# jiaxi98/cnf_ot

Hardware: AMD Instinct MI355X
Metric: MC samples/sec through flow fwd+log|detJ| at dim=2, batch=65536 (higher is better)
Workload: dtype f32; 1 GPU; configs[1]: OT free dim=2, batch=65536, sample_and_log_prob (RQS fwd + log|detJ|), L=2 H=16 M=2 K=5, params N(0,0.20^2) seed 42; ONE STEP = one evaluator-shaped pass of 10000 time-slices x 65536 samples (cnf_ot/utils.py:311-340), each slice its own condition t, one cnf_sample_logprob call per rank; batch=65536, dim=2, parallelism=slice-shard x1 (contiguous blocks of the step's slices; no collective)

## Files before the change

cnf_ot_amd/_capi.py:

```python
import ctypes
import os

_HERE = os.path.dirname(os.path.abspath(__file__))
LIB_PATH = os.path.join(_HERE, "lib", "libcnf_ot_amd.so")

CNF_OK = 0
CNF_ERR_INVALID = -22
CNF_ERR_UNSUPPORTED = -95
CNF_ERR_NOMEM = -12
CNF_ERR_HIP = -5


class CnfConfig(ctypes.Structure):
  _fields_ = [
    ("dim", ctypes.c_int32), ("num_layers", ctypes.c_int32),
    ("hidden_size", ctypes.c_int32), ("mlp_num_layers", ctypes.c_int32),
    ("num_bins", ctypes.c_int32),
    ("range_min", ctypes.c_float), ("range_max", ctypes.c_float),
    ("min_bin_size", ctypes.c_float), ("min_knot_slope", ctypes.c_float),
    ("periodized", ctypes.c_int32),
  ]


class CnfFieldGrid(ctypes.Structure):
# ... 57 lines not shown

KDE_MAX_BW = 4


class CnfKdeSpec(ctypes.Structure):
  _fields_ = [("n_bw", ctypes.c_int32), ("loo", ctypes.c_int32), ("bw", ctypes.c_float * KDE_MAX_BW)]


TERM_KINETIC, TERM_KINETIC_SCORE, TERM_FLOW_MATCHING, TERM_POTENTIAL, TERM_REVERSE_KL, TERM_NEG_LOGPROB = range(6)
TERM_DENSITY_L2, TERM_DENSITY_L2_DATA = 6, 7
POTENTIALS = {"quadratic": 0, "double_well": 1, "obstacle": 2}
DRIFTS = {"ou": 0, "gradient": 1, "smile": 1, "nongradient": 2, "lorenz": 3}

_P = ctypes.c_void_p
_I64 = ctypes.c_int64
_U64 = ctypes.c_uint64
_CFG = ctypes.POINTER(CnfConfig)
SYMBOLS = {
  "cnf_config_default": (None, [_CFG, ctypes.c_int32]),
  "cnf_param_count": (_I64, [_CFG]),
  "cnf_model_create": (ctypes.c_int, [_CFG, ctypes.POINTER(_P)]),
  "cnf_model_destroy": (None, [_P]),
  "cnf_model_set_params": (ctypes.c_int, [_P, _P, _P]),
  "cnf_model_reserve": (ctypes.c_int, [_P, _P, _I64]),
  "cnf_model_reserved": (_I64, [_P, _P]),
  "cnf_model_table_bytes": (_I64, [_P]),
  "cnf_model_has_tables": (ctypes.c_int, [_P]),
  "cnf_model_term_on_tables": (ctypes.c_int, [_P, _I64, _I64, ctypes.c_int]),
  "cnf_model_last_path": (ctypes.c_int, [_P]),
  "cnf_model_set_precise": (ctypes.c_int, [_P, ctypes.c_int]),
  "cnf_forward_logdet": (ctypes.c_int, [_P, _P, _P, _I64, _P, _P, _I64, _P]),
  "cnf_inverse_logdet": (ctypes.c_int, [_P, _P, _P, _I64, _P, _P, _I64, _P]),
  "cnf_log_prob": (ctypes.c_int, [_P, _P, _P, _I64, _P, _I64, _P]),
  "cnf_sample_logprob": (ctypes.c_int, [_P, _P, _P, _I64, _P, _P, _I64, _P]),
  "cnf_sample_logprob_seeded": (ctypes.c_int, [_P, _U64, _I64, _I64, _P, _I64, _P, _P, _I64, _P]),
  "cnf_forward_logdet_f64": (ctypes.c_int, [_P, _P, _P, _I64, _P, _P, _I64, _P]),
  "cnf_inverse_logdet_f64": (ctypes.c_int, [_P, _P, _P, _I64, _P, _P, _I64, _P]),
  "cnf_log_prob_f64": (ctypes.c_int, [_P, _P, _P, _I64, _P, _I64, _P]),
  "cnf_sample_logprob_f64": (ctypes.c_int, [_P, _P, _P, _I64, _P, _P, _I64, _P]),
  "cnf_fill_normal": (ctypes.c_int, [_U64, _U64, _I64, _P, _P]),
  "cnf_fill_normal_threefry": (ctypes.c_int, [ctypes.c_uint32, ctypes.c_uint32, _U64, _U64, _I64, _P, _P, _P]),
  "cnf_loss_terms": (ctypes.c_int, [_P, ctypes.POINTER(CnfLossSpec), _P, ctypes.c_int, _P, _I64, _I64, _P, _P]),
  "cnf_loss_terms_seeded": (ctypes.c_int, [_P, ctypes.POINTER(CnfLossSpec), _U64, _I64, _I64, _P, _I64, _I64, _P, _P]),
  "cnf_grad_supported": (ctypes.c_int, [_CFG]),
  "cnf_grad_enable": (ctypes.c_int, [_P, _I64]),
  "cnf_loss_terms_grad": (ctypes.c_int, [_P, ctypes.POINTER(CnfLossSpec), _P, ctypes.c_int, _P, _I64, _I64,
                                         ctypes.c_float, _P, _P, _P, _P]),
  "cnf_loss_terms_grad_multi": (ctypes.c_int, [_P, ctypes.c_int32, _P, _P, _P, _P, _P, _P, _P, _P, _P, _P, _P]),
  "cnf_input_vjp": (ctypes.c_int, [_P, ctypes.c_int, _P, _P, _I64, _P, _P, _P, _I64, _P]),
  "cnf_pass_vjp": (ctypes.c_int, [_P, ctypes.c_int, _P, _P, _I64, _P, _P, _P, _P, _P, _I64, _P]),
  "cnf_neg_logprob_vjp": (ctypes.c_int, [_P, _P, _P, _I64, ctypes.c_float, _P, _P, _P, _I64, _P]),
  "cnf_kinetic_potential_vjp": (ctypes.c_int, [_P, _P, _I64, _P, ctypes.c_int32, ctypes.c_float, ctypes.c_float, ctypes.c_int32,
                                               ctypes.c_float, ctypes.c_float, _P, _P, _P, _P, _P, _P]),
  "cnf_logprob_fd": (ctypes.c_int, [_P, _P, _P, _I64, ctypes.c_float, _P, _I64, _P]),
  "cnf_score": (ctypes.c_int, [_P, _P, ctypes.c_int32, _P, _I64, _I64, _P, _P, _P]),
  "cnf_logprob_fd_vjp": (ctypes.c_int, [_P, _P, _P, _I64, ctypes.c_float, _P, _P, _P, _P, _I64, _P]),
  "cnf_score_fd_vjp": (ctypes.c_int, [_P, _P, _P, _I64, ctypes.c_float, ctypes.c_float, ctypes.c_float, ctypes.c_int32,
                                      ctypes.c_float, ctypes.c_float, _P, _P, _P, _P, _I64, _P]),
  "cnf_score_residual": (ctypes.c_int, [_P, _P, _I64, _I64, ctypes.c_int32, ctypes.c_float, ctypes.c_float,
                                        ctypes.c_int32, ctypes.c_float, ctypes.c_float, _P, _P, _P, _P]),
  "cnf_score_residual_force": (ctypes.c_int, [_P, _P, _P, ctypes.c_float, _I64, _I64, ctypes.c_int32, ctypes.c_float,
                                              ctypes.c_float, ctypes.c_int32, ctypes.c_float, ctypes.c_float, _P, _P, _P, _P,
                                              _P]),
  "cnf_term_residual": (ctypes.c_int, [ctypes.c_int32, _P, _P, _I64, _I64, ctypes.c_int32, ctypes.c_int32, ctypes.c_float,
                                       ctypes.c_float, _P, _P, _P, _P]),
  "cnf_rkl_residual": (ctypes.c_int, [_P, _P, _I64, ctypes.c_int32, ctypes.c_float, ctypes.c_float, ctypes.c_float,
                                      ctypes.c_float, _P, _P, _P, _P]),
  "cnf_adam_step": (ctypes.c_int, [_P, _P, _P, _P, _I64, ctypes.c_float, ctypes.c_float, ctypes.c_float,
                                   ctypes.c_float, _I64, _P]),
  "cnf_step_begin": (ctypes.c_int, [_P, _P]),
  "cnf_fill_normal_dev": (ctypes.c_int, [_P, _U64, _I64, _P, _P]),
  "cnf_fill_uniform_dev": (ctypes.c_int, [_P, _U64, _I64, ctypes.c_float, _P, _P]),
  "cnf_mixture_source_dev": (ctypes.c_int, [_P, _U64, _I64, _P, _P, _P, _P]),
  "cnf_adam_step_dev": (ctypes.c_int, [_P, _P, _P, _P, _I64, ctypes.c_float, ctypes.c_float, ctypes.c_float,
                                       ctypes.c_float, _P, _P]),
  "cnf_weighted_sum": (ctypes.c_int, [_P, _P, _I64, _P, _P]),
  "cnf_hopf_cole_workspace": (ctypes.c_int, [ctypes.c_double, ctypes.c_double, ctypes.c_double, _I64, _I64,
                                              ctypes.POINTER(_I64)]),
  "cnf_hopf_cole_2d": (ctypes.c_int, [ctypes.c_int32, ctypes.c_float] + [ctypes.c_double] * 6
                       + [_P, _I64, _P, _I64, _P, _P, _P, _P, _P, _P, _P, _I64, _P]),
  "cnf_hopf_cole_path_workspace": (ctypes.c_int, [ctypes.c_double, ctypes.c_double, ctypes.c_double, _I64, _I64,
                                                   ctypes.POINTER(_I64)]),
  "cnf_hopf_cole_path_2d": (ctypes.c_int, [ctypes.c_int32, ctypes.c_float] + [ctypes.c_double] * 6
                            + [ctypes.POINTER(ctypes.c_double), _I64, _P, _I64, _P, _I64, _P, _P, _P, _P, _P, _P, _P,
                               _I64, _P]),
  "cnf_eulerian_fields": (ctypes.c_int, [_P, ctypes.POINTER(CnfFieldGrid), _P, _I64, _P, _I64, ctypes.c_float, ctypes.c_float,
                                        _P, _P, _P, _P, _P]),
  "cnf_eulerian_fields_f64": (ctypes.c_int, [_P, ctypes.POINTER(CnfFieldGrid), _P, _I64, _P, _I64, ctypes.c_double,
                                            ctypes.c_double, _P, _P, _P, _P, _P]),
  "cnf_trajectories": (ctypes.c_int, [_P, _P, _I64, ctypes.c_float, _P, _I64, ctypes.c_float, _P, _P, _P]),
  "cnf_trajectories_f64": (ctypes.c_int, [_P, _P, _I64, ctypes.c_double, _P, _I64, ctypes.c_double, _P, _P, _P]),
  "cnf_fp_particles_workspace": (ctypes.c_int, [_I64, ctypes.c_int32, ctypes.c_int32, ctypes.POINTER(_I64)]),
  "cnf_fp_particles": (ctypes.c_int, [ctypes.c_int32, ctypes.c_int32, ctypes.c_float, ctypes.c_double, ctypes.c_double,
                                      _I64, ctypes.c_double, _U64, _I64, _I64, _P, ctypes.POINTER(_I64), ctypes.c_int32,
                                      ctypes.POINTER(CnfFieldGrid), _P, _P, _P, _P, _I64, _P]),
  "cnf_point_stats": (ctypes.c_int, [_P, _I64, ctypes.c_int32, ctypes.c_int32, ctypes.POINTER(CnfFieldGrid), _P, _P, _P,
                                     _I64, _P]),
  "cnf_importance_workspace": (ctypes.c_int, [_I64, _I64, ctypes.c_int32, ctypes.POINTER(_I64)]),
  "cnf_importance_stats": (ctypes.c_int, [_P, ctypes.POINTER(CnfTargetSpec), _P, ctypes.c_int, _P, _I64, _I64, _P, _P, _I64,
                                          _P]),
  "cnf_importance_stats_seeded": (ctypes.c_int, [_P, ctypes.POINTER(CnfTargetSpec), _U64, _I64, _I64, _P, _I64, _I64, _P, _P,
                                                 _I64, _P]),
  "cnf_mmd_workspace": (ctypes.c_int, [ctypes.c_int32, _I64, _I64, ctypes.c_int32, ctypes.c_int32, ctypes.POINTER(_I64)]),
  "cnf_mmd_splits": (ctypes.c_int, [ctypes.c_int32, _I64, _I64, ctypes.c_int32]),
  "cnf_mmd2": (ctypes.c_int, [ctypes.POINTER(CnfMmdSpec), ctypes.c_int32, _P, _I64, _P, _I64, ctypes.c_int32, _P, _P, _P,
                              _I64, _P]),
  "cnf_sinkhorn_workspace": (ctypes.c_int, [ctypes.c_int32, _I64, _I64, ctypes.c_int32, ctypes.POINTER(_I64)]),
  "cnf_sinkhorn_splits": (ctypes.c_int, [ctypes.c_int32, _I64, _I64, ctypes.c_int32]),
  "cnf_sinkhorn": (ctypes.c_int, [ctypes.c_int32, _P, _I64, _P, _I64, ctypes.c_int32, ctypes.POINTER(ctypes.c_double),
                                  ctypes.c_int32, _P, _P, _P, _P, _P, _I64, _P]),
  "cnf_sliced_workspace": (ctypes.c_int, [ctypes.c_int32, _I64, _I64, ctypes.c_int32, ctypes.c_int32, ctypes.c_int32,
                                          ctypes.POINTER(_I64)]),
  "cnf_sliced_tile": (ctypes.c_int, []),
  "cnf_sliced_w2": (ctypes.c_int, [ctypes.c_int32, _P, _I64, _P, _I64, ctypes.c_int32, _P, ctypes.c_int32, ctypes.c_int32, _P,
                                   _P, _P, _I64, _P]),
  "cnf_knn_workspace": (ctypes.c_int, [ctypes.c_int32, _I64, _I64, ctypes.c_int32, ctypes.c_int32, ctypes.POINTER(_I64)]),
  "cnf_knn_splits": (ctypes.c_int, [ctypes.c_int32, _I64, _I64, ctypes.c_int32]),
  "cnf_knn": (ctypes.c_int, [ctypes.c_int32, _P, _I64, _P, _I64, ctypes.c_int32, ctypes.c_int32, _P, _P, _P, _P, _P, _P, _I64,
                             _P]),
  "cnf_interaction_workspace": (ctypes.c_int, [ctypes.c_int32, _I64, _I64, ctypes.c_int32, ctypes.c_int32,
                                               ctypes.POINTER(_I64)]),
  "cnf_interaction_splits": (ctypes.c_int, [ctypes.c_int32, _I64, _I64, ctypes.c_int32]),
  "cnf_interaction": (ctypes.c_int, [ctypes.POINTER(CnfInteractionSpec), ctypes.c_int32, _P, _I64, _P, _I64, ctypes.c_int32,
                                     _P, _P, _P, _P, _I64, _P]),
  "cnf_interaction_vjp_workspace": (ctypes.c_int, [ctypes.c_int32, _I64, ctypes.c_int32, ctypes.POINTER(_I64)]),
  "cnf_interaction_vjp": (ctypes.c_int, [ctypes.POINTER(CnfInteractionSpec), ctypes.c_int32, _P, _P, _I64, ctypes.c_int32, _P,
                                         _P, _I64, _P]),
  "cnf_stein_workspace": (ctypes.c_int, [ctypes.c_int32, _I64, ctypes.c_int32, ctypes.c_int32, ctypes.POINTER(_I64)]),
  "cnf_stein_splits": (ctypes.c_int, [ctypes.c_int32, _I64, ctypes.c_int32]),
  "cnf_stein": (ctypes.c_int, [ctypes.POINTER(CnfSteinSpec), ctypes.c_int32, _P, _P, _I64, ctypes.c_int32, _P, _P, _P, _P,
                               _P, _I64, _P]),
  "cnf_kde_workspace": (ctypes.c_int, [ctypes.c_int32, _I64, _I64, ctypes.c_int32, ctypes.c_int32, ctypes.c_int32,
                                       ctypes.POINTER(_I64)]),
  "cnf_kde_splits": (ctypes.c_int, [ctypes.c_int32, _I64, _I64, ctypes.c_int32]),
  "cnf_kde": (ctypes.c_int, [ctypes.POINTER(CnfKdeSpec), ctypes.c_int32, _P, _I64, _P, _I64, ctypes.c_int32, _P, _P, _P, _P,
                             _I64, _P]),
  "cnf_mv_particles_workspace": (ctypes.c_int, [ctypes.c_int32, _I64, ctypes.c_int32, ctypes.c_int32, ctypes.POINTER(_I64)]),
  "cnf_mv_particles": (ctypes.c_int, [ctypes.POINTER(CnfInteractionSpec), ctypes.c_double, ctypes.c_int32, ctypes.c_int32,
                                      ctypes.c_float, ctypes.c_double, ctypes.c_double, _I64, ctypes.c_double, _U64, _I64,
                                      ctypes.c_int32, _I64, _P, ctypes.POINTER(_I64), ctypes.c_int32,
                                      ctypes.POINTER(CnfFieldGrid), _P, _P, _P, _P, _P, _I64, _P]),
  "cnf_strerror": (ctypes.c_char_p, [ctypes.c_int]),
  "cnf_build_arch": (ctypes.c_char_p, []),
  "cnf_config_supported": (ctypes.c_int, [_CFG]),
}
_INTERNAL = {
  "cnf_model_set_fast_math": (ctypes.c_int, [_P, ctypes.c_int]),
  "cnf_model_set_samples_per_lane": (ctypes.c_int, [_P, ctypes.c_int]),
  "cnf_model_set_mfma": (ctypes.c_int, [_P, ctypes.c_int]),
  "cnf_model_set_pwl": (ctypes.c_int, [_P, ctypes.c_int]),
  "cnf_model_set_dpar": (ctypes.c_int, [_P, ctypes.c_int]),
  "cnf_model_set_pwl_builder": (ctypes.c_int, [_P, ctypes.c_int]),
  "cnf_model_last_pwl_builder": (ctypes.c_int, [_P]),
  "cnf_internal_build_tables_into": (ctypes.c_int, [_P, _P, _P, ctypes.c_float, _I64, _P]),
  "cnf_model_set_profiling": (ctypes.c_int, [_P, ctypes.c_int]),
  "cnf_model_read_profile": (ctypes.c_int, [_P, ctypes.POINTER(ctypes.c_double), ctypes.POINTER(ctypes.c_double),
                                            ctypes.POINTER(_I64), ctypes.POINTER(_I64)]),
}
PATH_NAMES = {0: "none", 1: "mlp1", 2: "mlp2", 3: "mfma", 4: "tables", 5: "loss_mlp", 6: "loss_tables", 7: "f64", 8: "detect", 9: "dpar", 10: "fields",
              11: "score", 12: "importance"}

_lib = None


class CnfError(RuntimeError):
  def __init__(self, code, where):
    self.code = code
    msg = lib().cnf_strerror(code).decode() if _lib is not None else str(code)
    super().__init__(f"{where}: {msg} ({code})")


def lib():
  global _lib
  if _lib is not None:
    return _lib
  if not os.path.exists(LIB_PATH):
    raise ImportError(
      f"{LIB_PATH} is missing: the cnf_ot_amd product path is hand-written HIP "
      "for gfx950 and has no CPU fallback. Build it with "
      "`python -m cnf_ot_amd.build` (needs hipcc).")
  handle = ctypes.CDLL(LIB_PATH)
  for table in (SYMBOLS, _INTERNAL):
    for name, (res, args) in table.items():
      fn = getattr(handle, name)
      fn.restype = res
      fn.argtypes = args
  _lib = handle
  return _lib


def check(code, where):
  if code != CNF_OK:
    raise CnfError(code, where)
```

cnf_ot_amd/build.py:

```python
import os
import shutil
import subprocess
import sys
from concurrent.futures import ThreadPoolExecutor

HERE = os.path.dirname(os.path.abspath(__file__))
SRC_DIR = os.path.join(HERE, "csrc")
LIB_DIR = os.path.join(HERE, "lib")
LIB_PATH = os.path.join(LIB_DIR, "libcnf_ot_amd.so")
OBJ_DIR = os.path.join(LIB_DIR, "obj")
SOURCES = ["cnf_flow.hip", "cnf_grad.hip", "cnf_grad_pwl.hip", "cnf_importance.hip", "cnf_mmd.hip", "cnf_knn.hip", "cnf_interaction.hip", "cnf_interaction_vjp.hip", "cnf_stein.hip", "cnf_kde.hip", "cnf_hopf_cole.hip", "cnf_fp_particles.hip",
           "cnf_mv_particles.hip", "cnf_sinkhorn.hip", "cnf_sliced.hip", "cnf_step.hip", "cnf_model.hip", "cnf_rng.hip"]
HEADERS = ["cnf_device.h", "cnf_terms.h", "cnf_common.h", "cnf_host.h", "cnf_flow_tile.h", "cnf_backward.h", "cnf_pwl.h",
           "cnf_pwl_build.h", "cnf_fp_stats.h", "cnf_pairs.h", "cnf_interaction_pairs.h", os.path.join("..", "..", "include", "cnf_ot_amd.h")]
VARIANT_PATH = os.path.join(LIB_DIR, "BUILD_VARIANT")
ARCH = "gfx950"


def _hipcc():
  for cand in (os.environ.get("HIPCC"), shutil.which("hipcc"), "/opt/rocm/bin/hipcc"):
    if cand and os.path.exists(cand):
      return cand
  raise RuntimeError("hipcc not found (need ROCm's hipcc to build the gfx950 kernels)")


def _variant() -> str:
  try:
    with open(VARIANT_PATH) as f:
      return f.read().strip()
  except OSError:
    return ""


def is_stale(minimal: bool = False) -> bool:
  if not os.path.exists(LIB_PATH):
    return True
  if not minimal and _variant() != "full":
    return True
  t = os.path.getmtime(LIB_PATH)
  deps = [os.path.join(SRC_DIR, f) for f in SOURCES + HEADERS]
  return any(os.path.getmtime(d) > t for d in deps if os.path.exists(d))


def _jobs() -> int:
  try:
    n = int(os.environ.get("MAX_JOBS", ""))
  except ValueError:
    n = 16
  return max(1, min(n, len(SOURCES), 16))


def build(force: bool = False, minimal: bool = False, verbose: bool = False) -> str:
  if not force and not is_stale(minimal):
    return LIB_PATH
  os.makedirs(OBJ_DIR, exist_ok=True)
  hipcc = _hipcc()
  flags = ["-O3", f"--offload-arch={ARCH}", "-std=c++17", "-fPIC", "-Wall", "-Wno-unused-function"]
  if minimal:
    flags.append("-DCNF_MINIMAL_CONFIGS")
  flags += os.environ.get("CNF_EXTRA_FLAGS", "").split()
  flags_path = os.path.join(OBJ_DIR, "FLAGS")
  try:
    with open(flags_path) as f:
      same_flags = f.read() == " ".join(flags)
  except OSError:
    same_flags = False
  newest_header = max(os.path.getmtime(os.path.join(SRC_DIR, h)) for h in HEADERS)

  def compile_one(name):
    src, obj = os.path.join(SRC_DIR, name), os.path.join(OBJ_DIR, os.path.splitext(name)[0] + ".o")
    if not force and same_flags and os.path.exists(obj) and os.path.getmtime(obj) > max(os.path.getmtime(src), newest_header):
      return obj
    cmd = [hipcc, *flags, "-c", src, "-o", obj]
    if verbose:
      print(" ".join(cmd), flush=True)
    res = subprocess.run(cmd, capture_output=True, text=True)
    if res.returncode != 0:
      raise RuntimeError(f"hipcc failed on {name}:\n" + res.stdout + res.stderr)
    return obj

  if os.path.exists(flags_path):
    os.remove(flags_path)
  with ThreadPoolExecutor(max_workers=_jobs()) as pool:
    objs = list(pool.map(compile_one, SOURCES))
  with open(flags_path, "w") as f:
    f.write(" ".join(flags))
  tmp = LIB_PATH + ".tmp"
  cmd = [hipcc, f"--offload-arch={ARCH}", "-fPIC", "-shared", *objs, "-o", tmp]
  if verbose:
    print(" ".join(cmd), flush=True)
  res = subprocess.run(cmd, capture_output=True, text=True)
  if res.returncode != 0:
    raise RuntimeError("hipcc failed to link:\n" + res.stdout + res.stderr)
  os.replace(tmp, LIB_PATH)
  with open(VARIANT_PATH, "w") as f:
    f.write("minimal\n" if minimal else "full\n")
  return LIB_PATH


if __name__ == "__main__":
  path = build(force="--force" in sys.argv, minimal="--minimal" in sys.argv, verbose=True)
  print("built", path)
```

cnf_ot_amd/csrc/cnf_common.h:

```cpp
#pragma once
#include <mutex>
#include <map>
#include <tuple>
#include <type_traits>
#include <unordered_map>
#include <vector>

#include "cnf_device.h"
#include "cnf_terms.h"
#include "../../include/cnf_ot_amd.h"

namespace cnf {

constexpr int TILE = 256;

struct ModelArgs {
  const float* prep;
  const float* wq;
  int64_t per_layer;
  int64_t per_layer_q;
  int32_t D, L, M;
  SplineConsts sc;
  SplineConstsT<double> scd;
  const double* tabd;
  const double* e2tab;
};

template <class R> __device__ __forceinline__ const SplineConstsT<R>& sc_of(const ModelArgs& a);
template <> __device__ __forceinline__ const SplineConstsT<float>& sc_of<float>(const ModelArgs& a) { return a.sc; }
template <> __device__ __forceinline__ const SplineConstsT<double>& sc_of<double>(const ModelArgs& a) { return a.scd; }
template <class R> __device__ __forceinline__ const R* table_of(const ModelArgs& a);
template <> __device__ __forceinline__ const float* table_of<float>(const ModelArgs& a) { return a.prep; }
template <> __device__ __forceinline__ const double* table_of<double>(const ModelArgs& a) { return a.tabd; }

}

struct CnfModel {
  CnfConfig cfg;
  cnf::SplineConsts sc;
  cnf::SplineConstsT<double> scd;
  int64_t tabd_off;
  int64_t e2_off;
  int precise;
  float* prep;
  int64_t n_params;
  int64_t per_layer;
  int device;
  int num_cus;
  int fast_math;
  int force_spl;
  int use_mfma;
  uint32_t div_magic;
  int64_t per_layer_q;
  int64_t mfma_off;
  int params_set;
  float* grad_slabs;
  int64_t grad_max_blocks;
  int use_pwl;
  int use_dpar;
  int pwl_builder;
  int last_pwl_builder;
  float* pwl_stats;
  struct PwlWorkspace { float* tables; int64_t sets; uint32_t epoch; std::vector<float*> retired; };
  std::mutex pwl_mu;
  std::unordered_map<void*, PwlWorkspace> pwl_ws;
  hipEvent_t prep_event;
  void* prep_stream;
  int last_path;
  struct ProfRec { hipEvent_t e0, e1, e2; int64_t samples; int path; };
  int profiling;
  std::vector<ProfRec> prof;
};

enum CnfPath {
  CNF_PATH_NONE = 0,
  CNF_PATH_MLP1 = 1,
  CNF_PATH_MLP2 = 2,
  CNF_PATH_MFMA = 3,
  CNF_PATH_TABLES = 4,
  CNF_PATH_LOSS_MLP = 5,
  CNF_PATH_LOSS_TABLES = 6,
  CNF_PATH_F64 = 7,
  CNF_PATH_DPAR = 9,
  CNF_PATH_DETECT = 8,
  CNF_PATH_FIELDS = 10,
  CNF_PATH_SCORE = 11,
  CNF_PATH_IMPORTANCE = 12,
};

static inline bool pwl_network(const CnfConfig& g) {
  return g.dim == 2 && g.hidden_size == 16 && g.num_bins == 5 && g.mlp_num_layers == 2 && !g.periodized;
}
static inline bool pwl_backward_network(const CnfConfig& g) { return pwl_network(g) && g.num_layers <= 4; }
static inline bool pwl_config_ok(const CnfModel* m) { return m->use_pwl && m->fast_math && pwl_network(m->cfg); }
static inline bool pwl_backward_ok(const CnfModel* m) {
  return pwl_config_ok(m) && pwl_backward_network(m->cfg) && m->pwl_stats != nullptr;
}
constexpr int64_t PWL_MIN_SLICE = 8192, PWL_MIN_POINTS = 262144;
static inline bool pwl_term_on_tables(const CnfModel* m, int64_t slice_len, int64_t n_points, bool with_grad) {
  if (with_grad ? !pwl_backward_ok(m) : !pwl_config_ok(m)) return false;
  return m->use_pwl != 1 || (slice_len >= PWL_MIN_SLICE && n_points >= PWL_MIN_POINTS);
}

#ifdef CNF_MINIMAL_CONFIGS
#define CNF_KERNEL_CONFIGS(X) X(16, 5)
#else
#define CNF_KERNEL_CONFIGS(X) \
  X(8, 5) X(16, 4) X(16, 5) X(16, 8) X(16, 10) X(32, 5) X(32, 8) X(64, 5)
#endif

template <class F>
static inline int with_shape(const CnfConfig& cfg, F&& f) {
#define X(HH, KK)                                      \
  if (cfg.hidden_size == HH && cfg.num_bins == KK)     \
    return f(std::integral_constant<int, HH>{}, std::integral_constant<int, KK>{});
  CNF_KERNEL_CONFIGS(X)
#undef X
  return CNF_ERR_UNSUPPORTED;
}
static inline bool shape_compiled(const CnfConfig& cfg) {
  return with_shape(cfg, [](auto, auto) { return CNF_OK; }) == CNF_OK;
}

template <class K>
static inline bool ensure_lds(K kernel, size_t bytes) {
  if (bytes > 160 * 1024) return false;
  if (bytes <= 64 * 1024) return true;
  static std::mutex mu;
  static std::map<std::pair<const void*, int>, bool> done;
  int dev = 0;
  if (hipGetDevice(&dev) != hipSuccess) return false;
  std::lock_guard<std::mutex> lock(mu);
  const auto key = std::make_pair((const void*)kernel, dev);
  auto it = done.find(key);
  if (it != done.end()) return it->second;
  const bool ok = hipFuncSetAttribute((const void*)kernel, hipFuncAttributeMaxDynamicSharedMemorySize, 160 * 1024) == hipSuccess;
  done[key] = ok;
  return ok;
}

struct ProfScope {
  CnfModel* m; hipStream_t s; CnfModel::ProfRec r; bool on;
  ProfScope(CnfModel* m_, hipStream_t s_, bool with_build, int64_t samples, int path) : m(m_), s(s_), on(false) {
    r.e0 = r.e1 = r.e2 = nullptr; r.samples = samples; r.path = path;
    if (!m->profiling || samples < 0 || m->prof.size() >= 4096) return;
    if (hipEventCreate(&r.e1) != hipSuccess || hipEventCreate(&r.e2) != hipSuccess) return;
    if (with_build) { if (hipEventCreate(&r.e0) != hipSuccess) return; (void)hipEventRecord(r.e0, s); }
    else (void)hipEventRecord(r.e1, s);
    on = true;
  }
  void built() { if (on && r.e0) (void)hipEventRecord(r.e1, s); }
  void done() { if (on) { (void)hipEventRecord(r.e2, s); m->prof.push_back(r); on = false; } }
};

template <class K, class A>
static int launch(CnfModel* m, K kernel, int64_t grid, int threads, size_t lds, hipStream_t stream, const A& a, int path,
                  bool gated = false, int64_t prof_samples = -1) {
  if (!gated) m->last_path = path;
  if (!ensure_lds(kernel, lds)) return CNF_ERR_UNSUPPORTED;
  ProfScope ps(m, stream, false, prof_samples, path);
  hipLaunchKernelGGL(kernel, dim3((unsigned)grid), dim3(threads), lds, stream, a);
  ps.done();
  return hipGetLastError() == hipSuccess ? CNF_OK : CNF_ERR_HIP;
}

template <class K, class... A>
static int launch_plain(K kernel, int64_t grid, int threads, size_t lds, hipStream_t stream, const A&... a) {
  hipLaunchKernelGGL(kernel, dim3((unsigned)grid), dim3(threads), lds, stream, a...);
  return hipGetLastError() == hipSuccess ? CNF_OK : CNF_ERR_HIP;
}

template <class K>
static inline int resident_blocks_per_cu(K kernel, int threads, size_t lds) {
  static std::mutex mu;
  static std::map<std::tuple<const void*, int, size_t, int>, int> cache;
  int dev = 0;
  if (hipGetDevice(&dev) != hipSuccess) return 1;
  std::lock_guard<std::mutex> lock(mu);
  const auto key = std::make_tuple((const void*)kernel, threads, lds, dev);
  auto it = cache.find(key);
  if (it != cache.end()) return it->second;
  int n = 0;
  if (hipOccupancyMaxActiveBlocksPerMultiprocessor(&n, (const void*)kernel, threads, lds) != hipSuccess || n < 1) n = 1;
  hipFuncAttributes fa;
  if (hipFuncGetAttributes(&fa, (const void*)kernel) == hipSuccess) {
    const size_t per_wg = ((lds + fa.sharedSizeBytes + 511) / 512) * 512;
    if (per_wg > 0) { const int by_lds = (int)((160 * 1024) / per_wg); if (by_lds >= 1 && by_lds < n) n = by_lds; }
    const int regs = ((fa.numRegs > 0 ? fa.numRegs : 1) + 7) / 8 * 8;
    int waves_per_simd = 512 / regs; if (waves_per_simd > 8) waves_per_simd = 8;
    const int by_regs = waves_per_simd * 4 / ((threads + 63) / 64);
    if (by_regs >= 1 && by_regs < n) n = by_regs;
  }
  cache[key] = n;
  return n;
}

// ... 60 lines not shown
```

cnf_ot_amd/csrc/cnf_device.h:

```cpp
#pragma once

#include <hip/hip_runtime.h>
#include <stdint.h>
#include <type_traits>

namespace cnf {

typedef float v2f __attribute__((ext_vector_type(2)));
typedef int v2i __attribute__((ext_vector_type(2)));

typedef const float __attribute__((address_space(4)))* uniform_ptr;

__device__ __forceinline__ uniform_ptr as_uniform(const float* p) { return (uniform_ptr)p; }

__device__ __forceinline__ uniform_ptr launder(uniform_ptr p) {
  asm volatile("" : "+s"(p));
  return p;
}

enum TabField {
  F_X0 = 0, F_Y0, F_BW, F_BH, F_IBW, F_IBH, F_S, F_ST, F_D0, F_D1, F_L2S,
  F_XK,
  F_YK,
  F_TAIL,
// ... 111 lines not shown
  static __device__ __forceinline__ v2f div(v2f a, v2f b) { return v2f{a.x / b.x, a.y / b.y}; }
  static __device__ __forceinline__ v2f sqrt(v2f x) { return v2f{sqrtf(x.x), sqrtf(x.y)}; }
};

constexpr float LOG2E = 1.44269502162933349609375f;
constexpr float LN2 = 0.693147182464599609375f;

template <> struct Math<true> {
  static __device__ __forceinline__ float exp(float x) { return __builtin_amdgcn_exp2f(x * LOG2E); }
  static __device__ __forceinline__ float log(float x) { return __builtin_amdgcn_logf(x) * LN2; }
  static __device__ __forceinline__ float rcp(float x) { return __builtin_amdgcn_rcpf(x); }
  static __device__ __forceinline__ float div(float a, float b) {
    const float r = __builtin_amdgcn_rcpf(b), q = a * r;
    return fmaf(fmaf(-b, q, a), r, q);
  }
  static __device__ __forceinline__ float sqrt(float x) { return __builtin_amdgcn_sqrtf(x); }
  static __device__ __forceinline__ v2f exp(v2f x) {
    const v2f t = x * LOG2E;
    return v2f{__builtin_amdgcn_exp2f(t.x), __builtin_amdgcn_exp2f(t.y)};
  }
  static __device__ __forceinline__ float exp2(float x) { return __builtin_amdgcn_exp2f(x); }
  static __device__ __forceinline__ v2f exp2(v2f x) { return v2f{__builtin_amdgcn_exp2f(x.x), __builtin_amdgcn_exp2f(x.y)}; }
  static __device__ __forceinline__ v2f log(v2f x) {
    return v2f{__builtin_amdgcn_logf(x.x), __builtin_amdgcn_logf(x.y)} * LN2;
  }
  static __device__ __forceinline__ v2f rcp(v2f x) {
    return v2f{__builtin_amdgcn_rcpf(x.x), __builtin_amdgcn_rcpf(x.y)};
  }
  static __device__ __forceinline__ v2f div(v2f a, v2f b) {
    const v2f r = rcp(b), q = a * r;
    return vfma(vfma(-b, q, a), r, q);
  }
  static __device__ __forceinline__ v2f sqrt(v2f x) {
    return v2f{__builtin_amdgcn_sqrtf(x.x), __builtin_amdgcn_sqrtf(x.y)};
  }
};

__device__ __forceinline__ v2f mul_clip01(v2f a, v2f b) {
  v2f z;
  asm("s_nop 0\n\tv_pk_mul_f32 %0, %1, %2 clamp" : "=v"(z) : "v"(a), "v"(b));
  return z;
}
__device__ __forceinline__ float mul_clip01(float a, float b) { return clip01(a * b); }
__device__ __forceinline__ double mul_clip01(double a, double b) { return clip01(a * b); }

template <bool FAST, class T, bool OFFSET_ADDED = false>
__device__ __forceinline__ T knot_slope(T t, const SplineConstsT<typename Lanes<T>::real> sc) {
  const T v = OFFSET_ADDED ? t : t + sc.sp_offset;
  const T av = vabs(v);
  const T e = Math<FAST>::exp(-av);
  typedef typename Lanes<T>::real R;
  if constexpr (std::is_same<T, double>::value) {
    return vrelu(v) + ::log1p(e) + sc.min_slope;
  } else {
    const T l_log = Math<FAST>::log(e + 1.0f);
    const T l_ser = vfma(e * -0.5f, e, e);
    const T l = vsel(vlt(e, (R)1e-4f), l_ser, l_log);
    return vfma(v + av, splat<T>(0.5f), l) + sc.min_slope;
  }
}

template <bool INV, bool FAST, class T, bool L2S_GIVEN = true, bool ARG = false, bool NEWTON = true, bool PRE = false>
__device__ __forceinline__ void rqs_bin_eval(T v, T x0, T y0, T bw, T bh, T ibw, T s, T st,
                                             T d0, T d1, T l2s, T& out, T& ld, T d0bh = T{}, T s2 = T{}) {
  using M = Math<FAST>;
  static_assert(!PRE || (INV && !NEWTON), "prepared products: the sampling direction's root");
  static_assert(NEWTON || INV, "the root without its Newton step: the inverse only");
  T z;
  [[maybe_unused]] T two_s;
  if (INV) {
    const T dy = vclamp(v - y0, bh);
    if constexpr (NEWTON) {
      const T c = -s * dy;
      const T b = vfma(-st, dy, d0 * bh);
      const T a = vfma(s, bh, -b);
      const T disc = vfma(b, b, a * c * -4.0f);
      z = clip01(M::div(c * -2.0f, b + M::sqrt(disc)));
    } else {
      two_s = PRE ? s2 : s * 2.0f;
      const T c2 = two_s * dy;
      const T b = vfma(-st, dy, PRE ? d0bh : d0 * bh);
      const T a = vfma(s, bh, -b);
      const T disc = vfma(b, b, a * (c2 + c2));
      z = mul_clip01(c2, M::rcp(b + M::sqrt(disc)));
    }
    out = vfma(bw, z, x0);
  } else {
    z = clip01((v - x0) * ibw);
  }
  const T sq_z = z * z;
  const T z1mz = z - sq_z;
  const T omz = 1.0f - z;
  const T den = vfma(st, z1mz, s);
  const T iden = M::rcp(den);
  if (!INV) out = vfma(bh * vfma(s, sq_z, d0 * z1mz), iden, y0);
  const T num2 = vfma(d1, sq_z, vfma(NEWTON ? s * 2.0f : two_s, z1mz, d0 * omz * omz));
  if constexpr (ARG) {
    static_assert(!L2S_GIVEN, "the argument form folds s^2 in");
    const T q = s * iden;
    ld = num2 * q * q;
  } else {
    T ldf;
    if (L2S_GIVEN) {
      ldf = l2s + M::log(num2 * iden * iden);
    } else {
      const T q = s * iden;
      ldf = M::log(num2 * q * q);
    }
    ld = INV ? -ldf : ldf;
  }
}

template <int K, class R> __device__ __forceinline__ int bin_of(const R* pos, R v) {
  int k = 0;
#pragma unroll
  for (int j = 1; j < K; ++j) k += (v >= pos[j]) ? 1 : 0;
  return k;
}
template <int K> __device__ __forceinline__ v2i bin_of_pairs(const float* kb, v2f v) {
  const v2f big = v2f{1.152921504606846976e18f, 1.152921504606846976e18f};
  v2f c = v2f{0.0f, 0.0f};
#pragma unroll
  for (int j = 1; j < K; ++j) {
    const v2f nk = *reinterpret_cast<const v2f*>(kb + 2 * j);
    v2f m;
    asm("v_pk_fma_f32 %0, %1, %2, %3 clamp" : "=v"(m) : "v"(v), "v"(big), "v"(nk));
    c = j == 1 ? m : c + m;
  }
  return v2i{(int)c.x, (int)c.y};
}
template <int K, class R> __device__ __forceinline__ R gather(const R* tab, int f, int k) {
  return tab[tab_off(f, K) + k];
}
template <int K> __device__ __forceinline__ v2f gather(const float* tab, int f, v2i k) {
  return v2f{tab[tab_off(f, K) + k.x], tab[tab_off(f, K) + k.y]};
}

template <class T> struct BinRow {
  const typename Lanes<T>::real* p;
  __device__ __forceinline__ BinRow(const typename Lanes<T>::real* tab, int k) : p(tab + k) {}
  template <int K> __device__ __forceinline__ T get(int f) const { return p[tab_off(f, K)]; }
};
template <> struct BinRow<v2f> {
  typedef const volatile float __attribute__((address_space(3))) * lds_ptr;
  lds_ptr px, py;
  __device__ __forceinline__ BinRow(const float* tab, v2i k) {
    lds_ptr t = (lds_ptr)(uintptr_t)(uint32_t)(uintptr_t)tab;
    px = t + k.x;
    py = t + k.y;
  }
  template <int K> __device__ __forceinline__ v2f get(int f) const { return v2f{px[tab_off(f, K)], py[tab_off(f, K)]}; }
};

template <int K, bool INV, bool FAST, class T, bool ARG = false, bool LEAN = false>
__device__ __forceinline__ void table_spline(const typename Lanes<T>::real* tab, T v,
                                             const SplineConstsT<typename Lanes<T>::real> sc, T& out, T& ld,
                                             bool tails = true) {
  typedef typename Lanes<T>::real R;
  typename Lanes<T>::index k;
  if constexpr (std::is_same<T, v2f>::value) k = bin_of_pairs<K>(tab + tab_off(INV ? F_YKB : F_XKB, K), v);
  else k = bin_of<K>(tab + tab_off(INV ? F_YK : F_XK, K), v);
  const BinRow<T> row(tab, k);
  const T bw = INV ? row.template get<K>(F_BW) : splat<T>(0.0f);
  const T ibw = INV ? splat<T>(0.0f) : row.template get<K>(F_IBW);
  if constexpr (ARG && LEAN && INV)
    rqs_bin_eval<INV, FAST, T, false, true, false, true>(v, row.template get<K>(F_X0), row.template get<K>(F_Y0), bw,
                                            row.template get<K>(F_BH), ibw,
                                            row.template get<K>(F_S), row.template get<K>(F_ST), row.template get<K>(F_D0),
                                            row.template get<K>(F_D1), splat<T>(0.0f), out, ld,
                                            row.template get<K>(F_D0BH), row.template get<K>(F_2S));
  else if constexpr (ARG)
    rqs_bin_eval<INV, FAST, T, false, true, !LEAN>(v, row.template get<K>(F_X0), row.template get<K>(F_Y0), bw,
                                            row.template get<K>(F_BH), ibw,
                                            row.template get<K>(F_S), row.template get<K>(F_ST), row.template get<K>(F_D0),
                                            row.template get<K>(F_D1), splat<T>(0.0f), out, ld);
  else
    rqs_bin_eval<INV, FAST, T, true, false, !LEAN>(v, row.template get<K>(F_X0), row.template get<K>(F_Y0), bw,
                               row.template get<K>(F_BH), ibw,
                               row.template get<K>(F_S), row.template get<K>(F_ST), row.template get<K>(F_D0),
                               row.template get<K>(F_D1), row.template get<K>(F_L2S), out, ld);
  if (LEAN ? tails : maybe_outside(v, sc.lo, sc.hi)) {
    const auto below = vle(v, sc.lo);
    const auto above = vge(v, sc.hi);
    const R* tl = tab + tab_off(F_TAIL, K);
    const T lo_out = INV ? vfma(v - sc.lo, splat<T>(tl[T_INV_DLO]), splat<T>(sc.lo))
                         : vfma(v - sc.lo, splat<T>(tl[T_DLO]), splat<T>(sc.lo));
    const T hi_out = INV ? vfma(v - sc.hi, splat<T>(tl[T_INV_DHI]), splat<T>(sc.hi))
                         : vfma(v - sc.hi, splat<T>(tl[T_DHI]), splat<T>(sc.hi));
    out = vsel(below, lo_out, out);
    ld = vsel(below, ARG ? splat<T>(tl[T_DLO]) : splat<T>(INV ? -tl[T_LOG_DLO] : tl[T_LOG_DLO]), ld);
    out = vsel(above, hi_out, out);
    ld = vsel(above, ARG ? splat<T>(tl[T_DHI]) : splat<T>(INV ? -tl[T_LOG_DHI] : tl[T_LOG_DHI]), ld);
  }
}

__device__ __forceinline__ v2f step_mask(v2f d, v2f big) {
  v2f m;
  asm("v_pk_mul_f32 %0, %1, %2 clamp" : "=v"(m) : "v"(d), "v"(big));
  return m;
}

template <int K, bool INV, bool FAST, bool SHIFT_FREE>
__device__ __forceinline__ void cond_spline_masked(const v2f (&th)[3 * K + 1], v2f v,
                                                   const SplineConsts sc, v2f& out, v2f& ld) {
  using M = Math<FAST>;
  typedef v2f T;
  T ew[K], eh[K];
  T aw, ah;
  if constexpr (SHIFT_FREE) {
#pragma unroll
    for (int k = 0; k < K; ++k) { ew[k] = M::exp2(th[k]); eh[k] = M::exp2(th[K + k]); }
    T sw = ew[0] + ew[1], sh = eh[0] + eh[1];
#pragma unroll
    for (int k = 2; k < K; ++k) { sw += ew[k]; sh += eh[k]; }
    const T r = M::rcp(sw * sh) * sc.span_eff;
    aw = r * sh; ah = r * sw;
  } else {
    T mw = th[0], mh = th[K];
#pragma unroll
    for (int k = 1; k < K; ++k) { mw = vmax(mw, th[k]); mh = vmax(mh, th[K + k]); }
#pragma unroll
    for (int k = 0; k < K; ++k) { ew[k] = M::exp2(th[k] - mw); eh[k] = M::exp2(th[K + k] - mh); }
    T sw = ew[0], sh = eh[0];
#pragma unroll
    for (int k = 1; k < K; ++k) { sw += ew[k]; sh += eh[k]; }
    aw = M::rcp(sw) * sc.span_eff; ah = M::rcp(sh) * sc.span_eff;
  }
  const T big = splat<T>(1.152921504606846976e18f);
  T px = splat<T>(sc.lo), py = splat<T>(sc.lo);
  T wp = vfma(ew[0], aw, splat<T>(sc.min_bin)), hp = vfma(eh[0], ah, splat<T>(sc.min_bin));
  T x0 = px, y0 = py;
  T mprev = splat<T>(1.0f), bw = splat<T>(0.0f), bh = splat<T>(0.0f), t0 = splat<T>(0.0f), t1 = splat<T>(0.0f);
#pragma unroll
  for (int k = 1; k < K; ++k) {
    px += wp;
    py += hp;
    const T m = step_mask(v - (INV ? py : px), big);
    const T o = mprev - m;
    bw = k == 1 ? o * wp : vfma(o, wp, bw);
    bh = k == 1 ? o * hp : vfma(o, hp, bh);
    t0 = k == 1 ? o * th[2 * K] : vfma(o, th[2 * K + k - 1], t0);
    t1 = k == 1 ? o * th[2 * K + 1] : vfma(o, th[2 * K + k], t1);
    x0 = vfma(m, wp, x0);
    y0 = vfma(m, hp, y0);
    if (k == K - 1) { wp = sc.hi - px; hp = sc.hi - py; }
    else { wp = vfma(ew[k], aw, splat<T>(sc.min_bin)); hp = vfma(eh[k], ah, splat<T>(sc.min_bin)); }
    mprev = m;
  }
  bw = vfma(mprev, wp, bw);
  bh = vfma(mprev, hp, bh);
  t0 = vfma(mprev, th[3 * K - 1], t0);
  t1 = vfma(mprev, th[3 * K], t1);
  T d0, d1;
  if constexpr (SHIFT_FREE) {
    const T l0 = v2f{__builtin_amdgcn_logf(M::exp2(t0).x + 1.0f), __builtin_amdgcn_logf(M::exp2(t0).y + 1.0f)};
    const T l1 = v2f{__builtin_amdgcn_logf(M::exp2(t1).x + 1.0f), __builtin_amdgcn_logf(M::exp2(t1).y + 1.0f)};
    d0 = vfma(l0, splat<T>(LN2), splat<T>(sc.min_slope));
    d1 = vfma(l1, splat<T>(LN2), splat<T>(sc.min_slope));
  } else {
    T n0 = t0 * LN2, n1 = t1 * LN2;
    asm volatile("" : "+v"(n0), "+v"(n1));
    d0 = knot_slope<FAST, T, true>(n0, sc);
    d1 = knot_slope<FAST, T, true>(n1, sc);
  }
  const T ibw = M::rcp(bw);
  const T s = bh * ibw;
  const T st = d1 + d0 - s * 2.0f;
  rqs_bin_eval<INV, FAST, T, false>(v, x0, y0, bw, bh, ibw, s, st, d0, d1, s, out, ld);
  if (maybe_outside(v, sc.lo, sc.hi)) {
    const auto below = vle(v, sc.lo);
    const auto above = vge(v, sc.hi);
    const T lo_out = INV ? M::div(v - sc.lo, d0) + sc.lo : vfma(v - sc.lo, d0, splat<T>(sc.lo));
    const T hi_out = INV ? M::div(v - sc.hi, d1) + sc.hi : vfma(v - sc.hi, d1, splat<T>(sc.hi));
    const T ld0 = M::log(d0), ld1 = M::log(d1);
    out = vsel(below, lo_out, out);
    ld = vsel(below, INV ? -ld0 : ld0, ld);
    out = vsel(above, hi_out, out);
    ld = vsel(above, INV ? -ld1 : ld1, ld);
  }
}

template <int K, bool INV, bool FAST, bool SHIFT_FREE, bool ARG = false, bool LEAN = false, class SlopeFetch>
__device__ __forceinline__ void cond_spline_rows(const v2f (&qa)[K], const v2f (&qb)[K], SlopeFetch&& slopes, v2f v,
                                                 const SplineConsts sc, v2f& out, v2f& ld, bool tails = true) {
  using M = Math<FAST>;
  typedef v2f T;
  auto la = [&](int j) { return qa[j >> 1][j & 1]; };
  auto lb = [&](int j) { return qb[j >> 1][j & 1]; };
  constexpr bool UNNORM = LEAN && SHIFT_FREE && INV;
  T ew[K], eh[K];
  T aw, ah;
  [[maybe_unused]] T ch[K + 1];
  if constexpr (SHIFT_FREE) {
#pragma unroll
    for (int k = 0; k < K; ++k) {
      ew[k] = v2f{__builtin_amdgcn_exp2f(la(k)), __builtin_amdgcn_exp2f(lb(k))};
      eh[k] = v2f{__builtin_amdgcn_exp2f(la(K + k)), __builtin_amdgcn_exp2f(lb(K + k))};
    }
    T sw = ew[0] + ew[1], sh = eh[0] + eh[1];
    if constexpr (UNNORM) { ch[1] = eh[0]; ch[2] = sh; }
#pragma unroll
    for (int k = 2; k < K; ++k) {
      sw += ew[k]; sh += eh[k];
      if constexpr (UNNORM) ch[k + 1] = sh;
    }
    const T r = M::rcp(sw * sh) * sc.span_eff;
    aw = r * sh; ah = r * sw;
  } else {
    float mwa = la(0), mwb = lb(0), mha = la(K), mhb = lb(K);
#pragma unroll
    for (int k = 1; k < K; ++k) {
      mwa = fmaxf(mwa, la(k)); mwb = fmaxf(mwb, lb(k));
      mha = fmaxf(mha, la(K + k)); mhb = fmaxf(mhb, lb(K + k));
    }
#pragma unroll
    for (int k = 0; k < K; ++k) {
      ew[k] = v2f{__builtin_amdgcn_exp2f(la(k) - mwa), __builtin_amdgcn_exp2f(lb(k) - mwb)};
      eh[k] = v2f{__builtin_amdgcn_exp2f(la(K + k) - mha), __builtin_amdgcn_exp2f(lb(K + k) - mhb)};
    }
    T sw = ew[0], sh = eh[0];
#pragma unroll
    for (int k = 1; k < K; ++k) { sw += ew[k]; sh += eh[k]; }
    aw = M::rcp(sw) * sc.span_eff; ah = M::rcp(sh) * sc.span_eff;
  }
  const T big = splat<T>(1.152921504606846976e18f);
  T x0, y0, bw, bh, kf;
  if constexpr (UNNORM) {
    const T t = ch[K] * (1.0f / sc.span_eff);
    T m[K];
#pragma unroll
    for (int k = 1; k < K; ++k) m[k] = step_mask(vfma(v - (sc.lo + (float)k * sc.min_bin), t, -ch[k]), big);
    T xs = m[1] * ew[0], ys = m[1] * eh[0];
    T ws = ew[0] - xs, hs = eh[0] - ys;
    kf = m[1];
#pragma unroll
    for (int k = 1; k < K; ++k) {
      const T o = k == K - 1 ? m[k] : m[k] - m[k + 1];
      ws = vfma(o, ew[k], ws);
      hs = vfma(o, eh[k], hs);
      if (k > 1) { xs = vfma(m[k], ew[k - 1], xs); ys = vfma(m[k], eh[k - 1], ys); kf += m[k]; }
    }
    const T base = vfma(kf, splat<T>(sc.min_bin), splat<T>(sc.lo));
    x0 = vfma(xs, aw, base);
    y0 = vfma(ys, ah, base);
    bw = vfma(ws, aw, splat<T>(sc.min_bin));
    bh = vfma(hs, ah, splat<T>(sc.min_bin));
// ... 607 lines not shown
```

cnf_ot_amd/csrc/cnf_flow.hip:

```cpp
#include "cnf_flow_tile.h"
#include "cnf_host.h"
#include "cnf_pwl_build.h"

#include <math.h>
#include <new>
#include <stdlib.h>
#include <string.h>

namespace cnf {

__global__ void circular_slopes_kernel(const float* __restrict__ params, float* __restrict__ prep, int K, int H,
                                       int D, int L, int M, int64_t per_layer) {
  const int P = 3 * K + 1;
  const int hdr = hdr_floats(K);
  const int l = blockIdx.x / (D - 1), d = 1 + blockIdx.x % (D - 1);
  int64_t o = (int64_t)l * per_layer;
  for (int dd = 1; dd < d; ++dd) o += cond_floats_p(dd, H, M, P, true);
  o += cond_floats_p(d, H, M, P, true) - ((int64_t)H * P + P);
  for (int r = threadIdx.x; r <= H; r += blockDim.x)
    prep[hdr + o + (int64_t)r * P + 3 * K] = params[P + o + (int64_t)r * P + 2 * K];
}

__global__ void prepare_kernel(const float* __restrict__ params, float* __restrict__ prep,
                               int K, int64_t n_params, double lo, double hi, double min_bin,
                               double min_slope, int D, int L, int M, int64_t per_layer,
                               int64_t per_layer_q, int64_t mfma_off, int64_t tabd_off, int H, int periodic) {
  const int P = 3 * K + 1;
  const int hdr = hdr_floats(K);
  constexpr int MAXK = 64;
  if (blockIdx.x != gridDim.x - 1) {
    const int nb = gridDim.x - 1;
    for (int64_t i = blockIdx.x * (int64_t)blockDim.x + threadIdx.x; i < n_params - P; i += (int64_t)nb * blockDim.x)
      prep[hdr + i] = params[P + i];
    if (mfma_off > 0) {
      const int nc = L * (D - 1);
      for (int ci = blockIdx.x; ci < nc; ci += nb) {
        const int l = ci / (D - 1), d = 1 + ci % (D - 1);
        int64_t so = P + l * per_layer, qo = mfma_off + l * per_layer_q;
        for (int dd = 1; dd < d; ++dd) { so += cond_floats(dd, 16, M, 16); qo += cond_floats_mfma(dd, M); }
        const float* src = params + so;
        float* dst = prep + qo;
        const int nf = (1 + d) + 1 + 2 * M;
        for (int idx = threadIdx.x; idx < nf * 64; idx += blockDim.x) {
          const int f = idx >> 6, lane = idx & 63, g = lane >> 4, i = lane & 15;
          float o[4];
          if (f <= d) {
            for (int t = 0; t < 4; ++t) o[t] = src[f * 16 + 4 * g + t];
          } else if (f == d + 1) {
            for (int t = 0; t < 4; ++t) o[t] = src[(1 + d) * 16 + 4 * g + t];
          } else {
            const int m = (f - (d + 2)) >> 1;
            const float* Wm = src + (1 + d) * 16 + 16 + m * (256 + 16);
            if (((f - (d + 2)) & 1) == 0) { for (int t = 0; t < 4; ++t) o[t] = Wm[(4 * g + t) * 16 + i]; }
            else { for (int t = 0; t < 4; ++t) o[t] = Wm[256 + 4 * g + t]; }
          }
          for (int t = 0; t < 4; ++t) dst[(f * 64 + lane) * 4 + t] = o[t];
        }
      }
    }
    return;
  }

  __shared__ double ex[2][MAXK], dl[MAXK + 1], mxs[2];
  if (threadIdx.x < 2) {
    const float* u = params + threadIdx.x * K;
    double mx = u[0];
    for (int k = 1; k < K; ++k) mx = fmax(mx, (double)u[k]);
    mxs[threadIdx.x] = mx;
  }
  __syncthreads();
  const double offset = log(exp(1.0 - min_slope) - 1.0);
  for (int idx = threadIdx.x; idx < 3 * K + 1; idx += blockDim.x) {
    if (idx < 2 * K) {
      const int part = idx / K, k = idx - part * K;
      ex[part][k] = exp((double)params[part * K + k] - mxs[part]);
    } else {
      const int k = idx - 2 * K;
      const double v = (double)params[2 * K + (periodic && k == K ? 0 : k)] + offset;
      dl[k] = fmax(v, 0.0) + log1p(exp(-fabs(v))) + min_slope;
    }
  }
  __syncthreads();
  __shared__ double xk[MAXK + 1], yk[MAXK + 1];
  double* td = reinterpret_cast<double*>(prep + tabd_off);
  for (int i = threadIdx.x; i < hdr; i += blockDim.x) { prep[i] = 0.0f; td[i] = 0.0; }
  const double total = (hi - lo) - K * min_bin;
  if (threadIdx.x < 2) {
    const int part = threadIdx.x;
    double* pos = part == 0 ? xk : yk;
    double sum = 0;
    for (int k = 0; k < K; ++k) sum += ex[part][k];
    double run = 0;
    pos[0] = lo;
    for (int k = 0; k < K - 1; ++k) {
      run += ex[part][k] / sum * total + min_bin;
      pos[k + 1] = lo + run;
    }
    pos[K] = hi;
  }
  __syncthreads();
  for (int k = threadIdx.x; k < K; k += blockDim.x) {
    const double bw = xk[k + 1] - xk[k], bh = yk[k + 1] - yk[k], s = bh / bw;
    td[tab_off(F_X0, K) + k] = xk[k];            td[tab_off(F_Y0, K) + k] = yk[k];
    td[tab_off(F_BW, K) + k] = bw;               td[tab_off(F_BH, K) + k] = bh;
    td[tab_off(F_IBW, K) + k] = 1.0 / bw;        td[tab_off(F_IBH, K) + k] = 1.0 / bh;
    td[tab_off(F_S, K) + k] = s;                 td[tab_off(F_ST, K) + k] = dl[k + 1] + dl[k] - 2.0 * s;
    td[tab_off(F_D0, K) + k] = dl[k];            td[tab_off(F_D1, K) + k] = dl[k + 1];
    td[tab_off(F_L2S, K) + k] = 2.0 * log(s);
    prep[tab_off(F_X0, K) + k] = (float)xk[k];
    prep[tab_off(F_Y0, K) + k] = (float)yk[k];
    prep[tab_off(F_BW, K) + k] = (float)bw;
    prep[tab_off(F_BH, K) + k] = (float)bh;
    prep[tab_off(F_IBW, K) + k] = (float)(1.0 / bw);
    prep[tab_off(F_IBH, K) + k] = (float)(1.0 / bh);
    prep[tab_off(F_S, K) + k] = (float)s;
    prep[tab_off(F_ST, K) + k] = (float)(dl[k + 1] + dl[k] - 2.0 * s);
    prep[tab_off(F_D0, K) + k] = (float)dl[k];
    prep[tab_off(F_D1, K) + k] = (float)dl[k + 1];
    prep[tab_off(F_L2S, K) + k] = (float)(2.0 * log(s));
    td[tab_off(F_D0BH, K) + k] = dl[k] * bh;     td[tab_off(F_2S, K) + k] = 2.0 * s;
    prep[tab_off(F_D0BH, K) + k] = (float)(dl[k] * bh);
    prep[tab_off(F_2S, K) + k] = 2.0f * (float)s;
  }
  for (int k = threadIdx.x; k <= K; k += blockDim.x) {
    const float big = 1.152921504606846976e18f;
    if (2 * k + 1 < 2 * tab_stride(K)) {
      prep[tab_off(F_XKB, K) + 2 * k] = prep[tab_off(F_XKB, K) + 2 * k + 1] = -(float)xk[k] * big;
      prep[tab_off(F_YKB, K) + 2 * k] = prep[tab_off(F_YKB, K) + 2 * k + 1] = -(float)yk[k] * big;
    }
    prep[tab_off(F_XK, K) + k] = (float)xk[k];
    prep[tab_off(F_YK, K) + k] = (float)yk[k];
    td[tab_off(F_XK, K) + k] = xk[k];
    td[tab_off(F_YK, K) + k] = yk[k];
  }
  if (threadIdx.x != 64) return;
  double* tld = td + tab_off(F_TAIL, K);
  tld[T_DLO] = dl[0];            tld[T_DHI] = dl[K];
  tld[T_LOG_DLO] = log(dl[0]);   tld[T_LOG_DHI] = log(dl[K]);
  tld[T_INV_DLO] = 1.0 / dl[0];  tld[T_INV_DHI] = 1.0 / dl[K];
  float* tl = prep + tab_off(F_TAIL, K);
  tl[T_DLO] = (float)dl[0];             tl[T_DHI] = (float)dl[K];
  tl[T_LOG_DLO] = (float)log(dl[0]);    tl[T_LOG_DHI] = (float)log(dl[K]);
  tl[T_INV_DLO] = (float)(1.0 / dl[0]); tl[T_INV_DHI] = (float)(1.0 / dl[K]);
}

template <int H, int K, bool TO_BASE, bool FAST, class T, bool MFMA = false, bool PRECISE = false, bool PERIODIC = false, int DFIX = 0>
__global__ __launch_bounds__(TILE, 2) void flow_kernel(const FlowArgsT<typename Lanes<T>::real> a) {
  typedef typename Lanes<T>::real R;
  extern __shared__ __attribute__((aligned(16))) float lds_raw[];
  R* lds = reinterpret_cast<R*>(lds_raw);
  constexpr int HDR = hdr_floats(K);
  constexpr int SPL = Lanes<T>::N;
  constexpr int TS = TILE * SPL;
  const int DD = DFIX ? DFIX : a.m.D;
  const uint32_t dmagic = DFIX == 2 ? 0x80000000u : (uint32_t)a.div_magic;
  R* tab = lds;
  R* U = lds + HDR;
  R* O = U + DD * TS;
  if (gate_closed(a)) return;
  for (int i = threadIdx.x; i < HDR; i += TILE) tab[i] = table_of<R>(a.m)[i];
  [[maybe_unused]] double* e2tab = nullptr;
  [[maybe_unused]] double* tabd = nullptr;
  [[maybe_unused]] R* LO = nullptr;
  if constexpr (PRECISE) {
    LO = O + DD * TS;
    e2tab = reinterpret_cast<double*>(LO + DD * TS);
    tabd = e2tab + EXP2_N;
    for (int i = threadIdx.x; i < EXP2_N; i += TILE) e2tab[i] = a.m.e2tab[i];
    for (int i = threadIdx.x; i < HDR; i += TILE) tabd[i] = a.m.tabd[i];
  }

  const int64_t n_tiles = (a.B + TS - 1) / TS;
  for (int64_t tile = blockIdx.x; tile < n_tiles; tile += gridDim.x) {
    const int64_t tile_start = tile * TS;
    const int64_t i = tile_start + SPL * threadIdx.x;
    __syncthreads();
    if (TO_BASE && !PRECISE && a.fd2) tile_load_fd<R>(a, U, DD, dmagic, TS, tile_start);
    else if (a.in) tile_load<R>(a.in, U, DD, dmagic, TS, tile_start, a.B);
    else tile_noise_flow(a, U, DD, dmagic, TS, tile_start, TILE);
    const T c = load_cond<T>(a, tile_start, i);
    __syncthreads();

    T base = splat<T>(0.0f);
    if (!TO_BASE && a.aux_mode == AUX_LOGPROB && a.aux) base = base_logprob<T>(lds_col<T>(U + SPL * threadIdx.x, TS), DD);
    BaseAcc<T> bacc;
    [[maybe_unused]] T poison = splat<T>(0.0f);
    if constexpr (TO_BASE) {
      for (int d = 0; d < DD; ++d) { const T v = lds_get<T>(U + SPL * threadIdx.x, d, TS); poison += v - v; }
    }
    const T acc = flow_pass<H, K, TO_BASE, FAST, T, MFMA, PRECISE, PERIODIC, DFIX>(a.m, tab, U, O, c, e2tab, tabd, LO, &bacc);
    if (a.aux) {
      T r = acc;
      if (a.aux_mode == AUX_LOGPROB) {
        if constexpr (PRECISE) r = bacc.log_prob(acc, DD);
        else r = TO_BASE ? base_logprob<T>(lds_col<T>(U + SPL * threadIdx.x, TS), DD) + acc : base - acc;
      }
      if constexpr (TO_BASE) r += poison;
      if (TO_BASE && !PRECISE && a.fd2) store_fd(a, i, r);
      else store_aux(a.aux, i, a.B, r);
    }
    if (a.out) {
      if constexpr (TO_BASE) {
        for (int d = 0; d < DD; ++d) lds_put(U + SPL * threadIdx.x, d, TS, lds_get<T>(U + SPL * threadIdx.x, d, TS) + poison);
      }
      __syncthreads();
      tile_store<R>(a.out, U, DD, dmagic, TS, tile_start, a.B);
    }
  }
}


template <int H, int K, bool FAST, class T>
__global__ __launch_bounds__(1024) void flow_dpar_kernel(const FlowArgs a) {
  extern __shared__ __attribute__((aligned(16))) float lds[];
  constexpr int HDR = hdr_floats(K), P = 3 * K + 1, SPL = Lanes<T>::N, TS = 64 * SPL;
  const int D = a.m.D, L = a.m.L, NT = blockDim.x, NW = NT >> 6;
  const int wave = __builtin_amdgcn_readfirstlane(threadIdx.x >> 6), lane = threadIdx.x & 63;
  float* tab = lds;
  float* U = lds + HDR;
  float* O = U + D * TS;
  float* LD = O + D * TS;
  if (gate_closed(a)) return;
  for (int i = threadIdx.x; i < HDR; i += NT) tab[i] = a.m.prep[i];
  const SplineConsts& sc = a.m.sc;
  uniform_ptr weights = as_uniform(a.m.prep + HDR);
  const int64_t cpart = cond_floats(0, H, a.m.M, P) - H;

  const int64_t n_tiles = (a.B + TS - 1) / TS;
  for (int64_t tile = blockIdx.x; tile < n_tiles; tile += gridDim.x) {
    const int64_t tile_start = tile * TS;
    const int64_t i = tile_start + SPL * lane;
    __syncthreads();
    if (a.in) tile_load_n<float>(a.in, U, D, a.div_magic, TS, tile_start, a.B, NT);
    else tile_noise_flow(a, U, D, a.div_magic, TS, tile_start, NT);
    const T c = load_cond<T>(a, tile_start, i);
    __syncthreads();
    T base = splat<T>(0.0f);
    if (wave == 0 && a.aux_mode == AUX_LOGPROB && a.aux) base = base_logprob<T>(lds_col<T>(U + SPL * lane, TS), D);
    T acc = splat<T>(0.0f);
    for (int l = 0; l < L; ++l) {
      const bool odd = l & 1;
      const int first_idx = odd ? D - 1 : 0, idx_step = odd ? -1 : 1;
      const float* cu = U + SPL * lane;
      float* co = O + SPL * lane;
      T o, ld;
      if (wave == 0) {
        table_spline<K, true, FAST, T>(tab, lds_get<T>(cu, first_idx, TS), sc, o, ld);
        lds_put(co, first_idx, TS, o);
        acc += ld;
      }
      for (int d = 1 + wave; d < D; d += NW) {
        const int64_t off = l * a.m.per_layer + (int64_t)H * ((d - 1) + (int64_t)d * (d - 1) / 2) + (d - 1) * cpart;
        T th[P];
        conditioner<H, P, T>(weights + off, d, a.m.M, c, cu, first_idx, idx_step, TS, th);
        const int idx = first_idx + d * idx_step;
        cond_spline<K, true, FAST, T>(th, lds_get<T>(cu, idx, TS), sc, o, ld);
        lds_put(co, idx, TS, o);
        acc += ld;
      }
      __syncthreads();
      float* t = U; U = O; O = t;
    }
    if (a.aux) lds_put(LD + wave * TS + SPL * lane, 0, TS, acc);
    __syncthreads();
    if (a.aux && wave == 0) {
      T tot = splat<T>(0.0f);
      for (int w = 0; w < NW; ++w) tot += lds_get<T>(LD + w * TS + SPL * lane, 0, TS);
      store_aux(a.aux, i, a.B, a.aux_mode == AUX_LOGPROB ? base - tot : tot);
    }
    if (a.out) tile_store_n<float>(a.out, U, D, a.div_magic, TS, tile_start, a.B, NT);
  }
}

struct PwlArgs {
  ModelArgs m;
  const float* in;
  float* out;
  float* aux;
  const float* tables;
  int64_t B, slice_len;
  int32_t n_slices, tiles_per_slice, aux_mode;
  const uint32_t* gate;
  uint32_t gate_epoch;
  int32_t gate_want;
  uint64_t seed;
  int64_t first_sample, slice_stride;
  int32_t in_shared;
};

__global__ void cond_uniform_kernel(const float* __restrict__ c, int64_t B, uint32_t* flag, uint32_t epoch) {
  const uint32_t c0 = __float_as_uint(c[0]);
  bool diff = false;
  for (int64_t i = blockIdx.x * (int64_t)blockDim.x + threadIdx.x; i < B; i += (int64_t)gridDim.x * blockDim.x)
    diff |= __float_as_uint(c[i]) != c0;
  if (__syncthreads_or(diff) && threadIdx.x == 0) *flag = epoch;
}

constexpr int PWL_WAIT_VM0 = 0x0F70;

template <int K, bool TO_BASE, bool FAST, bool PRECISE = false, int LROWS = PWL_LROWS, int LFIX = 0, bool SEEDED = false>
__global__ __launch_bounds__(PWL_MAX_THREADS) void flow_pwl_kernel(const PwlArgs a) {
  const int PWL_THREADS = blockDim.x, PWL_TS = 2 * PWL_THREADS;
  extern __shared__ __attribute__((aligned(16))) float lds_raw[];
  constexpr int HDR = (hdr_floats(K) + 3) & ~3;
  float* tab = lds_raw;
  float* tbl = lds_raw + HDR;
  const int tid = threadIdx.x;
  const int L = LFIX ? LFIX : a.m.L;
  if (gate_closed(a)) return;
  for (int i = tid; i < hdr_floats(K); i += PWL_THREADS) tab[i] = table_of<float>(a.m)[i];
  const SplineConsts sc = sc_scalars(sc_of<float>(a.m));
  [[maybe_unused]] double* e2tab = nullptr;
  [[maybe_unused]] double* tabd = nullptr;
  if constexpr (PRECISE) {
    e2tab = reinterpret_cast<double*>(tbl + L * pwl_ltbl(LROWS));
    tabd = e2tab + EXP2_N;
    for (int i = tid; i < EXP2_N; i += PWL_THREADS) e2tab[i] = a.m.e2tab[i];
    for (int i = tid; i < hdr_floats(K); i += PWL_THREADS) tabd[i] = a.m.tabd[i];
  }

  const int total = a.n_slices * a.tiles_per_slice;
  const int per_block = (total + gridDim.x - 1) / gridDim.x;
  const int t0 = blockIdx.x * per_block;
  const int t1 = t0 + per_block < total ? t0 + per_block : total;
  int cur = -1;
  const bool big = a.slice_len >= ((int64_t)1 << 30);
  struct Tile { int slice; int ti; int valid; int left; int64_t g0; int64_t st0; int64_t gin; };
  auto tile_at = [&](int slice, int ti) {
    Tile t;
    t.slice = slice;
    t.ti = ti;
    const int64_t s0 = (int64_t)t.slice * a.slice_len;
    const int64_t len = a.B - s0 < a.slice_len ? a.B - s0 : a.slice_len;
    const int64_t jt = (int64_t)ti * PWL_TS;
    const int64_t left = len - jt;
    t.valid = left >= PWL_TS ? PWL_TS : (left > 0 ? (int)left : 0);
    t.left = big ? 0 : (int)(left < -(int64_t)PWL_TS ? -(int64_t)PWL_TS : left);
    t.g0 = s0 + jt;
    t.gin = a.in_shared ? jt : t.g0;
    t.st0 = a.first_sample + (int64_t)t.slice * a.slice_stride + jt;
    return t;
  };
  auto tile_of = [&](int tile) { const int sl = tile / a.tiles_per_slice; return tile_at(sl, tile - sl * a.tiles_per_slice); };
  auto tile_next = [&](const Tile& t) {
    if (t.ti + 1 >= a.tiles_per_slice) return tile_at(t.slice + 1, 0);
    if (big) return tile_at(t.slice, t.ti + 1);
    Tile n = t;
    n.ti = t.ti + 1;
    n.left = t.left - PWL_TS;
    n.valid = n.left >= PWL_TS ? PWL_TS : (n.left > 0 ? n.left : 0);
    n.g0 = t.g0 + PWL_TS; n.gin = t.gin + PWL_TS; n.st0 = t.st0 + PWL_TS;
    return n;
  };
  const uint32_t lane2 = 2u * (uint32_t)tid;
  const bool lp = a.aux_mode == AUX_LOGPROB;
  const int omode = (a.aux ? 1 : 0) | (a.out ? 2 : 0) | (lp ? 4 : 0);
  auto tile_points = [&](const Tile& t) {
    f4 x = {0.f, 0.f, 0.f, 0.f};
    if (SEEDED && !a.in) {
      const uint64_t e0 = (uint64_t)(t.st0 + lane2) * 2u;
      if ((int)lane2 < t.valid) {
        if ((e0 & 3) == 0) {
          float z[4];
          philox_normals4(a.seed, e0 >> 2, z);
#pragma unroll
          for (int q = 0; q < 4; ++q) x[q] = z[q];
        } else {
#pragma unroll
          for (int q = 0; q < 4; ++q) x[q] = normal_at(a.seed, e0 + q);
        }
        if ((int)lane2 + 1 >= t.valid) { x[2] = 0.f; x[3] = 0.f; }
      }
      return x;
    }
    const float* p = a.in + 2 * t.gin;
    if (t.valid == PWL_TS) return *reinterpret_cast<const f4*>(p + 2u * lane2);
    if ((int)lane2 + 1 < t.valid) x = *reinterpret_cast<const f4*>(p + 2u * lane2);
    else if ((int)lane2 < t.valid) { x[0] = p[2u * lane2]; x[1] = p[2u * lane2 + 1]; }
    __builtin_amdgcn_s_waitcnt(PWL_WAIT_VM0);
    return x;
  };
  [[maybe_unused]] f4 xn = {0.f, 0.f, 0.f, 0.f};
  Tile tn{};
  if (t0 < t1) { tn = tile_of(t0); xn = tile_points(tn); }
  f4 x = xn;
  __builtin_amdgcn_s_waitcnt(PWL_WAIT_VM0);
  for (int tile = t0; tile < t1; ++tile) {
    const Tile tl = tn;
    const int slice = tl.slice;
    if (slice != cur) {
      __syncthreads();
      pwl_stage<LROWS>(tbl, a.tables + (int64_t)slice * L * PWL_TBL, L, tid, PWL_THREADS);
      cur = slice;
      __syncthreads();
    }
    const bool full = tl.valid == PWL_TS;
    if (tile + 1 < t1) { tn = tile_next(tl); xn = tile_points(tn); }
    __builtin_amdgcn_sched_barrier(0);
    v2f u0 = {x[0], x[2]}, u1 = {x[1], x[3]};
    [[maybe_unused]] v2f poison = splat<v2f>(0.0f);
    if constexpr (TO_BASE) poison = (u0 - u0) + (u1 - u1);

    v2f base = splat<v2f>(0.0f);
    if (!TO_BASE && lp && a.aux) base = (u0 * u0 + u1 * u1) * -0.5f - (float)(2 * HALF_LOG_2PI);
    if (!TO_BASE) asm volatile("" : "+v"(base));
    BaseAcc<v2f> bacc;
    const v2f acc = flow2_tables<K, TO_BASE, FAST, PRECISE, true, LROWS, LFIX, true>(tab, tbl, a.tables + (int64_t)slice * L * PWL_TBL, L, sc,
                                                            u0, u1, &a.m.scd, e2tab, tabd, &bacc);
    asm volatile("" : "+v"(xn));
    __builtin_amdgcn_sched_barrier(0);
    auto emit = [&](bool has_aux, bool is_lp, bool has_out, bool whole) {
      const bool v0 = (int)lane2 < tl.valid, v1 = (int)lane2 + 1 < tl.valid;
      if (has_aux) {
        v2f r = acc;
        if constexpr (PRECISE) { if (is_lp) r = bacc.log_prob(acc, 2); }
        else if (is_lp)
          r = TO_BASE ? (u0 * u0 + u1 * u1) * -0.5f - (float)(2 * HALF_LOG_2PI) + acc : base - acc;
        if constexpr (TO_BASE) r += poison;
        float* q = a.aux + tl.g0;
        if (whole || v1) *reinterpret_cast<v2f*>(q + lane2) = r;
        else if (v0) q[lane2] = r.x;
      }
      if (has_out) {
        float* q = a.out + 2 * tl.g0;
        if constexpr (TO_BASE) { u0 += poison; u1 += poison; }
        if (whole || v1) *reinterpret_cast<f4*>(q + 2u * lane2) = f4{u0.x, u1.x, u0.y, u1.y};
        else if (v0) { q[2u * lane2] = u0.x; q[2u * lane2 + 1] = u1.x; }
      }
    };
    if (full && omode == 7) emit(true, true, true, true);
    else emit(a.aux != nullptr, lp, a.out != nullptr, full);
    x = xn;
  }
}

struct LossArgs {
  ModelArgs m;
  CnfLossSpec spec;
  const float* pts;
  const float* t;
  double* sums;
  int64_t B;
  int64_t n_slices;
  int64_t pts_slice_stride;
  uint32_t div_magic;
  uint64_t seed;
  int64_t first_sample;
  DensityMix mix;
};

template <class T>
__device__ __forceinline__ void copy_cols(float* dst, const float* src, int D, int TS) {
  for (int d = 0; d < D; ++d) lds_put(dst, d, TS, lds_get<T>(src, d, TS));
}

__device__ __forceinline__ float mask_tail(float v, int64_t i, int64_t B) { return i < B ? v : 0.0f; }
__device__ __forceinline__ float mask_tail(v2f v, int64_t i, int64_t B) {
  return (i < B ? v.x : 0.0f) + (i + 1 < B ? v.y : 0.0f);
}

template <int H, int K, bool FAST, class T>
__global__ __launch_bounds__(TILE, 2) void loss_kernel(const LossArgs a) {
  extern __shared__ __attribute__((aligned(16))) float lds[];
  constexpr int HDR = hdr_floats(K);
  constexpr int SPL = Lanes<T>::N;
  constexpr int TS = TILE * SPL;
  using M = Math<FAST>;
  const int D = a.m.D;
  float* tab = lds;
  float* Nn = lds + HDR;
  float* U = Nn + D * TS;
  float* O = U + D * TS;
  float* V = O + D * TS;
  float* R = V + D * TS;
  for (int i = threadIdx.x; i < HDR; i += TILE) tab[i] = a.m.prep[i];
  const int col = SPL * threadIdx.x;
  const int kind = a.spec.kind;

  const int64_t tiles_per_slice = (a.B + TS - 1) / TS;
  const int64_t n_tiles = tiles_per_slice * a.n_slices;
  SliceSum ssum;
  for (int64_t tile = blockIdx.x; tile < n_tiles; tile += gridDim.x) {
    const int64_t slice = tile / tiles_per_slice;
    const int64_t tile_start = (tile - slice * tiles_per_slice) * TS;
    const int64_t i = tile_start + col;
    __syncthreads();
    if (a.pts)
      tile_load<float>(a.pts + slice * a.pts_slice_stride * D, Nn, D, a.div_magic, TS, tile_start, a.B);
    else
      tile_noise(a.seed, (uint64_t)(a.first_sample + slice * a.pts_slice_stride + tile_start) * (uint64_t)D, Nn, D,
                 a.div_magic, TS, a.B - tile_start);
    const float t = a.t[slice];
    __syncthreads();

    T acc = splat<T>(0.0f);
    const float dt = a.spec.dt;
    const bool kin = kind <= CNF_TERM_FLOW_MATCHING;
    const bool data = kind == CNF_TERM_NEG_LOGPROB || kind == CNF_TERM_DENSITY_L2_DATA;
    const int n_fwd = data ? 0 : (kind == CNF_TERM_KINETIC ? 2 : (kin ? 3 : 1));
    T fldj = splat<T>(0.0f);
    for (int p = 0; p < n_fwd; ++p) {
      const float c = !kin ? t : (p == 0 ? t - 0.5f * dt : (p == 1 ? t + 0.5f * dt : t));
      copy_cols<T>(U + col, Nn + col, D, TS);
      fldj = flow_pass<H, K, false, FAST, T>(a.m, tab, U, O, splat<T>(c));
      if (kin) {
        if (p == 0) copy_cols<T>(V + col, U + col, D, TS);
        else if (p == 1) {
          const float inv_dt = 1.0f / dt;
          for (int d = 0; d < D; ++d)
            lds_put(V + col, d, TS, (lds_get<T>(U + col, d, TS) - lds_get<T>(V + col, d, TS)) * inv_dt);
        } else copy_cols<T>(R + col, U + col, D, TS);
      }
    }
    if (kind == CNF_TERM_KINETIC) {
      acc = sq_norm<T>(lds_col<T>(V + col, TS), D);
    } else if (kind == CNF_TERM_POTENTIAL) {
      acc = potential<FAST, T>(lds_col<T>(U + col, TS), D, a.spec.subtype, a.spec.a).v;
    } else if (kind == CNF_TERM_REVERSE_KL) {
      const T lp = base_logprob<T>(lds_col<T>(Nn + col, TS), D) - fldj;
      acc = lp - rkl_mixture<FAST, T>(lds_col<T>(U + col, TS), D, t, a.spec.T, a.spec.beta).logmix;
    } else if (kind == CNF_TERM_DENSITY_L2) {
      const T lp = base_logprob<T>(lds_col<T>(Nn + col, TS), D) - fldj;
      acc = density_l2_residual<FAST, T>(lp, density_mixture<FAST, T>(lds_col<T>(U + col, TS), D, t, a.mix));
    }
    const bool neg = data;
    const int n_tb = neg ? 1 : ((kind == CNF_TERM_KINETIC_SCORE || kind == CNF_TERM_FLOW_MATCHING) ? 2 * D : 0);
    const float dx = a.spec.dx;
    T lp0 = splat<T>(0.0f);
    for (int e = 0; e < n_tb; ++e) {
      const int d = e >> 1, sgn = e & 1;
      copy_cols<T>(U + col, (neg ? Nn : R) + col, D, TS);
      if (!neg) lds_put(U + col, d, TS, lds_get<T>(R + col, d, TS) + (sgn == 0 ? 0.5f * dx : -0.5f * dx));
      if (kind == CNF_TERM_DENSITY_L2_DATA)
        lds_put(V + col, 0, TS, density_mixture<FAST, T>(lds_col<T>(Nn + col, TS), D, t, a.mix));
      const T ildj = flow_pass<H, K, true, FAST, T>(a.m, tab, U, O, splat<T>(t));
      const T lp = base_logprob<T>(lds_col<T>(U + col, TS), D) + ildj;
      if (kind == CNF_TERM_DENSITY_L2_DATA) acc = density_l2_residual<FAST, T>(lp, lds_get<T>(V + col, 0, TS));
      else if (neg) acc = -lp;
      else if (sgn == 0) lp0 = lp;
      else {
        const T dr = drift_field<T>(lds_col<T>(R + col, TS), d, kind == CNF_TERM_FLOW_MATCHING ? a.spec.subtype : -1, a.spec.a);
        const T u = score_residual(lds_get<T>(V + col, d, TS), (lp0 - lp) * (1.0f / dx), a.spec.coef, dr);
        acc = vfma(u, u, acc);
      }
    }
    float part = mask_tail(acc, i, a.B);
#pragma unroll
    for (int off = 32; off > 0; off >>= 1) part += __shfl_xor(part, off, 64);
    ssum.add(a.sums, slice, part);
  }
  ssum.flush(a.sums);
}


template <class R> struct FieldArgsT {
  ModelArgs m;
  const R* pts;
  const R* t;
  const R* fixed;
  const R* sec;
  R* rho;
// ... 116 lines not shown
          field_copy<T>(U + col, P + col, D);
          lds_put(U + col, d, TS, lds_get<T>(P + col, d, TS) + (sgn == 0 ? half_dx : -half_dx));
          const T ps = field_poison<T>(U + col, D);
          const T ildj = flow_pass<H, K, true, FAST, T>(a.m, tab, U, O, ts);
          const T lp = base_logprob<T>(lds_col<T>(U + col, TS), D) + ildj;
          if (sgn == 0) lp0 = lp;
          else lds_put(V + col, d, TS, (lp0 - lp) * inv_dx + ps);
        }
        __syncthreads();
        tile_store<R>(a.score + s * a.N * D, V, D, a.div_magic, TS, tile_start, a.N);
        __syncthreads();
      }
    }
  }
}


struct LossPwlArgs {
  ModelArgs m;
  CnfLossSpec spec;
  const float* pts;
  const float* t;
  double* sums;
  const float* tables;
  int64_t B, n_slices, pts_slice_stride;
  uint64_t seed;
  int64_t first_sample;
  int32_t n_sets, tiles_per_slice;
  DensityMix mix;
};

template <int K, bool FAST>
__global__ __launch_bounds__(PWL_MAX_THREADS) void loss_pwl_kernel(const LossPwlArgs a) {
  using M = Math<FAST>;
  typedef v2f T;
  const int NT = blockDim.x, TS = 2 * NT;
  extern __shared__ __attribute__((aligned(16))) float lds_raw[];
  constexpr int HDR = (hdr_floats(K) + 3) & ~3;
  const int tid = threadIdx.x;
  const int L = a.m.L;
  float* tab = lds_raw;
  float* tbl = lds_raw + HDR;
  float* R = tbl + a.n_sets * L * PWL_LTBL;
  for (int i = tid; i < hdr_floats(K); i += NT) tab[i] = table_of<float>(a.m)[i];
  const SplineConsts sc = sc_scalars(sc_of<float>(a.m));
  const int kind = a.spec.kind;
  const bool kin = kind <= CNF_TERM_FLOW_MATCHING;
  const float dt = a.spec.dt, dx = a.spec.dx;
  const int64_t set_stride = a.n_slices * L * (int64_t)PWL_TBL;
  const int col = 2 * tid;

  const int total = (int)a.n_slices * a.tiles_per_slice;
  const int per_block = (total + gridDim.x - 1) / gridDim.x;
  const int t0 = blockIdx.x * per_block;
  const int t1 = t0 + per_block < total ? t0 + per_block : total;
  int cur = -1;
  SliceSum ssum;
  for (int tile = t0; tile < t1; ++tile) {
    const int slice = tile / a.tiles_per_slice;
    __syncthreads();
    if (slice != cur) {
      for (int s = 0; s < a.n_sets; ++s)
        pwl_stage(tbl + s * L * PWL_LTBL, a.tables + s * set_stride + (int64_t)slice * L * PWL_TBL, L, tid, NT);
      cur = slice;
      __syncthreads();
    }
    const float* gslice = a.tables + (int64_t)slice * L * PWL_TBL;
    const int64_t j = (int64_t)(tile - slice * a.tiles_per_slice) * TS + col;
    const bool v0 = j < a.B, v1 = j + 1 < a.B;
    const float t = a.t[slice];
    f4 x = {0.f, 0.f, 0.f, 0.f};
    const int64_t g = slice * a.pts_slice_stride + j;
    if (a.pts) {
      const float* src = a.pts + 2 * g;
      if (v1 && (reinterpret_cast<uintptr_t>(src) & 15) == 0) x = *reinterpret_cast<const f4*>(src);
      else { if (v0) { x[0] = src[0]; x[1] = src[1]; } if (v1) { x[2] = src[2]; x[3] = src[3]; } }
    } else {
      const uint64_t e0 = (uint64_t)(a.first_sample + g) * 2u;
      if ((e0 & 3) == 0) {
        float z[4];
        philox_normals4(a.seed, e0 >> 2, z);
#pragma unroll
        for (int q = 0; q < 4; ++q) x[q] = z[q];
      } else {
#pragma unroll
        for (int q = 0; q < 4; ++q) x[q] = normal_at(a.seed, e0 + q);
      }
      if (!v0) { x[0] = 0.f; x[1] = 0.f; }
      if (!v1) { x[2] = 0.f; x[3] = 0.f; }
    }
    const T n0 = {x[0], x[2]}, n1 = {x[1], x[3]};
    auto n = [&](int q) { return q == 0 ? n0 : n1; };

    T acc = splat<T>(0.0f);
    const bool data = kind == CNF_TERM_NEG_LOGPROB || kind == CNF_TERM_DENSITY_L2_DATA;
    const int n_fwd = data ? 0 : (kind == CNF_TERM_KINETIC ? 2 : (kin ? 3 : 1));
    T fldj = splat<T>(0.0f);
    T y0 = n0, y1 = n1, va = splat<T>(0.0f), vb = splat<T>(0.0f);
    auto y = [&](int q) { return q == 0 ? y0 : y1; };
    for (int p = 0; p < n_fwd; ++p) {
      y0 = n0; y1 = n1;
      fldj = flow2_tables<K, false, FAST, false, true>(tab, tbl + p * L * PWL_LTBL, gslice + p * set_stride, L, sc, y0, y1);
      if (kin) {
        if (p == 0) { va = y0; vb = y1; }
        else if (p == 1) { const float inv_dt = 1.0f / dt; va = (y0 - va) * inv_dt; vb = (y1 - vb) * inv_dt; }
      }
    }
    const int tset = kin ? 2 : 0;
    if (kind == CNF_TERM_KINETIC) {
      acc = vfma(va, va, vb * vb);
    } else if (kind == CNF_TERM_POTENTIAL) {
      acc = potential<FAST, T>(y, 2, a.spec.subtype, a.spec.a).v;
    } else if (kind == CNF_TERM_REVERSE_KL) {
      acc = base_logprob<T>(n, 2) - fldj - rkl_mixture<FAST, T>(y, 2, t, a.spec.T, a.spec.beta).logmix;
    } else if (kind == CNF_TERM_DENSITY_L2) {
      acc = density_l2_residual<FAST, T>(base_logprob<T>(n, 2) - fldj,
                                         density_mixture<FAST, T>(y, 2, t, a.mix));
    }
    const bool neg = data;
    const int n_tb = neg ? 1 : ((kind == CNF_TERM_KINETIC_SCORE || kind == CNF_TERM_FLOW_MATCHING) ? 4 : 0);
    if (kind == CNF_TERM_FLOW_MATCHING) { lds_put(R + col, 0, TS, y0); lds_put(R + col, 1, TS, y1); }
    T lp0 = splat<T>(0.0f);
    for (int e = 0; e < n_tb; ++e) {
      const int d = e >> 1, sgn = e & 1;
      T u0 = neg ? n0 : y0, u1 = neg ? n1 : y1;
      if (!neg) {
        const float h = sgn == 0 ? 0.5f * dx : -0.5f * dx;
        if (d == 0) u0 = u0 + h; else u1 = u1 + h;
      }
      if (kind == CNF_TERM_DENSITY_L2_DATA) lds_put(R + col, 0, TS, density_mixture<FAST, T>(n, 2, t, a.mix));
      const T ildj = flow2_tables<K, true, FAST, false, true>(tab, tbl + tset * L * PWL_LTBL, gslice + tset * set_stride, L, sc, u0, u1);
      const T lp = base_logprob<T>([&](int q) { return q == 0 ? u0 : u1; }, 2) + ildj;
      if (kind == CNF_TERM_DENSITY_L2_DATA) acc = density_l2_residual<FAST, T>(lp, lds_get<T>(R + col, 0, TS));
      else if (neg) acc = -lp;
      else if (sgn == 0) lp0 = lp;
      else {
        const T dr = drift_field<T>(lds_col<T>(R + col, TS), d, kind == CNF_TERM_FLOW_MATCHING ? a.spec.subtype : -1, a.spec.a);
        const T u = score_residual(d == 0 ? va : vb, (lp0 - lp) * (1.0f / dx), a.spec.coef, dr);
        acc = vfma(u, u, acc);
      }
    }
    float part = (v0 ? acc.x : 0.0f) + (v1 ? acc.y : 0.0f);
#pragma unroll
    for (int off = 32; off > 0; off >>= 1) part += __shfl_xor(part, off, 64);
    ssum.add(a.sums, slice, part);
  }
  ssum.flush(a.sums);
}

}

using namespace cnf;

extern "C" int cnf_model_set_params(CnfModel* m, const float* params, void* stream) {
  if (!m || !params) return CNF_ERR_INVALID;
  const int K = m->cfg.num_bins;
  const int64_t n_w = m->n_params - (3 * K + 1);
  int blocks = (int)((n_w + 255) / 256);
  if (blocks < 1) blocks = 1;
  if (blocks > 256) blocks = 256;
  blocks += 1;
  hipLaunchKernelGGL(prepare_kernel, dim3(blocks), dim3(256), 0, (hipStream_t)stream, params, m->prep, K,
                     m->n_params, (double)m->cfg.range_min, (double)m->cfg.range_max,
                     (double)m->cfg.min_bin_size, (double)m->cfg.min_knot_slope, m->cfg.dim,
                     m->cfg.num_layers, m->cfg.mlp_num_layers, m->per_layer, m->per_layer_q, m->mfma_off,
                     m->tabd_off, m->cfg.hidden_size, m->cfg.periodized);
  if (m->cfg.periodized && m->cfg.dim > 1)
    hipLaunchKernelGGL(circular_slopes_kernel, dim3((unsigned)(m->cfg.num_layers * (m->cfg.dim - 1))), dim3(64), 0,
                       (hipStream_t)stream, params, m->prep, K, m->cfg.hidden_size, m->cfg.dim, m->cfg.num_layers,
                       m->cfg.mlp_num_layers, m->per_layer);
  if (hipGetLastError() != hipSuccess) return CNF_ERR_HIP;
  hipStreamCaptureStatus cap = hipStreamCaptureStatusNone;
  if (hipStreamIsCapturing((hipStream_t)stream, &cap) != hipSuccess) cap = hipStreamCaptureStatusNone;
  if (cap == hipStreamCaptureStatusNone && hipEventRecord(m->prep_event, (hipStream_t)stream) != hipSuccess) return CNF_ERR_HIP;
  m->prep_stream = stream;
  m->params_set = 1;
  return CNF_OK;
}


constexpr int CNF_MFMA_SMALL_WAVES = 4;

static int samples_per_lane(const CnfModel* m, int64_t B) {
  if (m->force_spl == 1 || m->force_spl == 2) return m->force_spl;
  if (m->use_mfma == 2 && m->mfma_off > 0 && m->cfg.hidden_size == 16 && m->cfg.num_bins == 5 &&
      B <= (int64_t)m->num_cus * 4 * 64 * CNF_MFMA_SMALL_WAVES) return 1;
  return (m->fast_math && B >= (int64_t)m->num_cus * 4 * 64 * 2) ? 2 : 1;
}

typedef void (*FlowKernel)(const FlowArgs);

static int launch_flow_dpar(CnfModel* m, const FlowArgs& a, hipStream_t stream) {
  const int D = m->cfg.dim;
  if (D < 3 || !m->fast_math || m->use_mfma == 1 || !m->use_dpar || m->cfg.periodized) return CNF_ERR_UNSUPPORTED;
  if (m->use_dpar == 1 && a.B > (int64_t)m->num_cus * 512) return CNF_ERR_UNSUPPORTED;
  int nw = D - 1;
  if (nw > 16) nw = 16;
  const int spl = (m->force_spl == 1 || m->force_spl == 2) ? m->force_spl : (a.B >= (int64_t)m->num_cus * 128 ? 2 : 1);
  const int64_t ts = 64 * spl;
  const size_t lds = (size_t)(hdr_floats(m->cfg.num_bins) + (2 * D + nw) * ts) * sizeof(float);
  if (lds > 64 * 1024) return CNF_ERR_UNSUPPORTED;
  int64_t grid = (a.B + ts - 1) / ts;
  const int64_t cap = (int64_t)m->num_cus * 8;
  if (grid > cap) grid = cap;
  return with_shape(m->cfg, [&](auto h, auto k) -> int {
    constexpr int H = decltype(h)::value, K = decltype(k)::value;
    const FlowKernel kern = spl == 2 ? flow_dpar_kernel<H, K, true, v2f> : flow_dpar_kernel<H, K, true, float>;
    return launch(m, kern, grid, 64 * nw, lds, stream, a, CNF_PATH_DPAR, a.gate != nullptr, a.B);
  });
}

static size_t precise_lds_bytes(int K) { return sizeof(double) * (size_t)(cnf::EXP2_N + hdr_floats(K)); }

template <int H, int K, bool TO_BASE, bool PRECISE = false>
static FlowKernel flow_kernel_of(bool precise, bool fast, int spl) {
  if constexpr (TO_BASE && !PRECISE)
    if (precise) return flow_kernel_of<H, K, true, true>(true, fast, spl);
  if (!fast) return flow_kernel<H, K, TO_BASE, false, float, false, PRECISE>;
  return spl == 2 ? flow_kernel<H, K, TO_BASE, true, v2f, false, PRECISE>
                  : flow_kernel<H, K, TO_BASE, true, float, false, PRECISE>;
}
template <bool TO_BASE, bool PRECISE = false>
static FlowKernel flow_mfma_kernel_of(bool precise, int spl, bool d2) {
  if constexpr (TO_BASE && !PRECISE)
    if (precise) return flow_mfma_kernel_of<true, true>(true, spl, d2);
  if (spl == 2) return flow_kernel<16, 5, TO_BASE, true, v2f, true, PRECISE>;
  return d2 ? flow_kernel<16, 5, TO_BASE, true, float, true, PRECISE, false, 2>
            : flow_kernel<16, 5, TO_BASE, true, float, true, PRECISE>;
}

template <bool TO_BASE>
static int launch_flow(CnfModel* m, const FlowArgs& a, int spl, hipStream_t stream) {
  const int64_t ts = (int64_t)TILE * spl;
  const int64_t n_tiles = (a.B + ts - 1) / ts;
  int64_t grid = n_tiles;
  const int64_t cap = (int64_t)m->num_cus * 8;
  if (grid > cap) grid = cap;
  const bool gated = a.gate != nullptr;
  if (m->cfg.periodized) {
    if (!m->fast_math) return CNF_ERR_UNSUPPORTED;
    const int64_t tiles1 = (a.B + TILE - 1) / TILE;
    const int64_t grid1 = tiles1 < cap ? tiles1 : cap;
    const size_t lds1 = (size_t)(hdr_floats(m->cfg.num_bins) + 2 * a.m.D * TILE) * sizeof(float);
    return with_shape(m->cfg, [&](auto h, auto k) -> int {
      constexpr int H = decltype(h)::value, K = decltype(k)::value;
      return launch(m, flow_kernel<H, K, TO_BASE, true, float, false, false, true>, grid1, TILE, lds1, stream, a,
                    CNF_PATH_MLP1, gated);
    });
  }
  const bool precise = TO_BASE && m->precise;
  const size_t lds = (size_t)(hdr_floats(m->cfg.num_bins) + 2 * a.m.D * ts) * sizeof(float) +
                     (precise ? precise_lds_bytes(m->cfg.num_bins) + sizeof(float) * a.m.D * ts : 0);
  const bool small = a.B <= (int64_t)m->num_cus * 4 * 64 * CNF_MFMA_SMALL_WAVES;
  if (m->fast_math && (m->use_mfma == 1 || (m->use_mfma == 2 && small)) && m->mfma_off > 0 &&
      m->cfg.hidden_size == 16 && m->cfg.num_bins == 5)
    return launch(m, flow_mfma_kernel_of<TO_BASE>(precise, spl, m->cfg.dim == 2 && spl == 1), grid, TILE, lds, stream, a,
                  CNF_PATH_MFMA, gated, a.B);
  return with_shape(m->cfg, [&](auto h, auto k) -> int {
    constexpr int H = decltype(h)::value, K = decltype(k)::value;
    return launch(m, flow_kernel_of<H, K, TO_BASE>(precise, m->fast_math != 0, spl), grid, TILE, lds, stream, a,
                  spl == 2 ? CNF_PATH_MLP2 : CNF_PATH_MLP1, gated, a.B);
  });
}

struct SlicePlan { int64_t tps, chunk; float* tables; };

static int slice_plan(CnfModel* m, hipStream_t stream, int64_t slice_len, int64_t n_slices, int64_t tile,
                      int sets_per_slice, SlicePlan* p) {
  const int64_t PWL_MAX_SLICES = 2048;
  p->tps = (slice_len + tile - 1) / tile;
  const int64_t total = n_slices * p->tps;
  if (total > (1 << 30)) return CNF_ERR_UNSUPPORTED;
  if (m->use_pwl == 1 && (total < 2 * (int64_t)m->num_cus || slice_len < 4 * tile)) return CNF_ERR_UNSUPPORTED;
  p->chunk = n_slices < PWL_MAX_SLICES ? n_slices : PWL_MAX_SLICES;
  int64_t sets = 0;
  pwl_workspace(m, stream, &p->tables, &sets);
  if (sets / sets_per_slice < p->chunk) p->chunk = sets / sets_per_slice;
  if (p->chunk < 1) return CNF_ERR_UNSUPPORTED;
  if (m->use_pwl == 1 && p->chunk < n_slices && p->chunk * p->tps < (int64_t)m->num_cus) return CNF_ERR_UNSUPPORTED;
  return CNF_OK;
}

constexpr int64_t PWL_LEAN_MIN_TABLES = 2048;
static void build_tables(CnfModel* m, hipStream_t stream, const float* c, float offset, int64_t ns, float* tables) {
  const int L = m->cfg.num_layers;
  const float* w = m->prep + cnf::hdr_floats(5);
  const bool lean = m->pwl_builder == 0 ? ns * L >= PWL_LEAN_MIN_TABLES : m->pwl_builder != 1;
  m->last_pwl_builder = lean ? 2 : 1;
  const dim3 grid((unsigned)(ns * L));
  if (!lean)
    hipLaunchKernelGGL(cnf::pwl_build_kernel, grid, dim3(512), 0, stream, w, m->per_layer, c, offset, L,
                       m->scd.sp_offset, tables);
  else
    hipLaunchKernelGGL(cnf::pwl_build_lean_kernel<64>, grid, dim3(64), 0, stream, w, m->per_layer, c, offset, L,
                       m->scd.sp_offset, tables);
}

typedef void (*PwlKernel)(const cnf::PwlArgs);

template <bool TO_BASE, bool PRECISE, bool SEEDED>
static PwlKernel flow_pwl_kernel_of(bool full, bool l2) {
  constexpr int ALL = cnf::PWL_NPIECE, WIN = cnf::PWL_LROWS;
  if (l2) return cnf::flow_pwl_kernel<5, TO_BASE, true, PRECISE, ALL, 2, SEEDED>;
  return full ? cnf::flow_pwl_kernel<5, TO_BASE, true, PRECISE, ALL, 0, SEEDED>
              : cnf::flow_pwl_kernel<5, TO_BASE, true, PRECISE, WIN, 0, SEEDED>;
}
static PwlKernel flow_pwl_kernel_of(bool to_base, bool precise, bool seeded, bool full, bool l2) {
  if (precise) return flow_pwl_kernel_of<true, true, false>(full, l2);
  if (to_base) return flow_pwl_kernel_of<true, false, false>(full, l2);
  return seeded ? flow_pwl_kernel_of<false, false, true>(full, l2) : flow_pwl_kernel_of<false, false, false>(full, l2);
}

struct NoiseSrc { uint64_t seed; int64_t first_sample, slice_stride; };

static int run_flow_pwl(CnfModel* m, bool to_base, const float* in, const float* c, int64_t c_block,
                        float* out, float* aux, int aux_mode, int64_t B, hipStream_t stream,
                        bool detect = false, const uint32_t** gate = nullptr, uint32_t* gate_epoch = nullptr,
                        const NoiseSrc* noise = nullptr, const float* built = nullptr, bool in_shared = false) {
  if (!pwl_config_ok(m)) return CNF_ERR_UNSUPPORTED;
  const int L = m->cfg.num_layers;
  const bool precise = to_base && m->precise;
  auto lds_for = [&](int lrows) {
    return (size_t)(((cnf::hdr_floats(5) + 3) & ~3) + L * cnf::pwl_ltbl(lrows)) * sizeof(float) +
           (precise ? precise_lds_bytes(5) : 0);
  };
  const bool full = lds_for(cnf::PWL_NPIECE) <= 160 * 1024;
  size_t lds = lds_for(full ? cnf::PWL_NPIECE : cnf::PWL_LROWS);
  if (lds > 160 * 1024) return CNF_ERR_UNSUPPORTED;
  const int64_t slice_len = c_block < B ? c_block : B;
  const int64_t n_slices = (B + slice_len - 1) / slice_len;
  if (n_slices > 1 && (slice_len & 1)) return CNF_ERR_UNSUPPORTED;
  if ((reinterpret_cast<uintptr_t>(in) & 15) || (reinterpret_cast<uintptr_t>(out) & 15) ||
      (reinterpret_cast<uintptr_t>(aux) & 7))
    return CNF_ERR_UNSUPPORTED;
  const int pwl_threads = cnf::PWL_MAX_THREADS;
  const size_t pwl_min_lds = 82 * 1024;
  SlicePlan plan;
  if (slice_plan(m, stream, slice_len, n_slices, 2 * pwl_threads, 1, &plan) != CNF_OK) return CNF_ERR_UNSUPPORTED;
  const int64_t tps = plan.tps, chunk = plan.chunk;
  float* tables = plan.tables;
  if (built && (chunk < n_slices || built != tables)) return CNF_ERR_UNSUPPORTED;
  if (pwl_min_lds > lds) lds = pwl_min_lds;
  const PwlKernel kern = flow_pwl_kernel_of(to_base, precise, noise != nullptr, full, full && L == 2);
  if (!ensure_lds(kern, lds)) return CNF_ERR_UNSUPPORTED;
  uint32_t* flag = nullptr;
  uint32_t epoch = 0;
  if (detect) {
    int64_t sets = 0;
    pwl_workspace(m, stream, &tables, &sets, &flag, &epoch);
    int64_t g = (B + 4095) / 4096;
    if (g > 4 * (int64_t)m->num_cus) g = 4 * (int64_t)m->num_cus;
    hipLaunchKernelGGL(cnf::cond_uniform_kernel, dim3((unsigned)g), dim3(256), 0, stream, c, B, flag, epoch);
    *gate = flag; *gate_epoch = epoch;
  }
  m->last_path = detect ? CNF_PATH_DETECT : CNF_PATH_TABLES;
  for (int64_t s0 = 0; s0 < n_slices; s0 += chunk) {
    const int64_t ns = n_slices - s0 < chunk ? n_slices - s0 : chunk;
    const int64_t first = s0 * slice_len;
    ProfScope ps(m, stream, true, (B - first) < ns * slice_len ? (B - first) : ns * slice_len, CNF_PATH_TABLES);
    if (!built) build_tables(m, stream, c + s0, 0.0f, ns, tables);
    ps.built();
    cnf::PwlArgs a;
    a.m = model_args(m);
    a.in_shared = in_shared ? 1 : 0;
    a.in = in ? in + (in_shared ? 0 : first * 2) : nullptr; a.out = out ? out + first * 2 : nullptr; a.aux = aux ? aux + first : nullptr;
    a.seed = noise ? noise->seed : 0; a.slice_stride = noise ? noise->slice_stride : 0;
    a.first_sample = noise ? noise->first_sample + s0 * noise->slice_stride : 0;
    a.tables = tables;
    a.B = (B - first) < ns * slice_len ? (B - first) : ns * slice_len;
    a.slice_len = slice_len;
    a.n_slices = (int32_t)ns; a.tiles_per_slice = (int32_t)tps; a.aux_mode = aux_mode;
    a.gate = flag; a.gate_epoch = epoch; a.gate_want = 0;
    const int64_t tiles = ns * tps;
    const int64_t want = (int64_t)m->num_cus;
    const int64_t grid = tiles < want ? tiles : want;
    hipLaunchKernelGGL(kern, dim3((unsigned)grid), dim3(pwl_threads), lds, stream, a);
    ps.done();
  }
  return hipGetLastError() == hipSuccess ? CNF_OK : CNF_ERR_HIP;
}

int cnf_internal_flow_shared(CnfModel* m, hipStream_t stream, const float* in, const float* c, int64_t slice_len,
                             int64_t n_slices, const float* tables, float* out) {
  return run_flow_pwl(m, false, in, c, slice_len, out, nullptr, 0, n_slices * slice_len, stream, false, nullptr, nullptr,
                      nullptr, tables, true);
}

int cnf_internal_build_tables(CnfModel* m, hipStream_t stream, const float* c, int64_t n, float** tables) {
  if (!pwl_config_ok(m) || n < 1) return CNF_ERR_UNSUPPORTED;
  int64_t sets = 0;
  pwl_workspace(m, stream, tables, &sets);
  if (sets < n) return CNF_ERR_UNSUPPORTED;
  build_tables(m, stream, c, 0.0f, n, *tables);
  return hipGetLastError() == hipSuccess ? CNF_OK : CNF_ERR_HIP;
}

extern "C" int cnf_internal_build_tables_into(CnfModel* m, void* stream, const float* c, float c_offset, int64_t n,
                                              float* out) {
  if (!m || !c || !out || n < 1 || n * m->cfg.num_layers > (1 << 30)) return CNF_ERR_INVALID;
  if (!m->params_set) return CNF_ERR_INVALID;
  if (!pwl_network(m->cfg) || (reinterpret_cast<uintptr_t>(out) & 15)) return CNF_ERR_UNSUPPORTED;
  if (wait_for_params(m, (hipStream_t)stream) != CNF_OK) return CNF_ERR_HIP;
  build_tables(m, (hipStream_t)stream, c, c_offset, n, out);
  return hipGetLastError() == hipSuccess ? CNF_OK : CNF_ERR_HIP;
}

template <class R>
static FlowArgsT<R> flow_args(const CnfModel* m, const R* in, const R* c, int64_t c_block, R* out, R* aux, int aux_mode,
                              int64_t B, int64_t tile_samples) {
  FlowArgsT<R> a;
  a.m = model_args(m);
  a.in = in; a.c = c; a.out = out; a.aux = aux;
  a.B = B; a.c_block = c_block; a.aux_mode = aux_mode; a.div_magic = m->div_magic;
  if (c_block >= B) a.c_mode = C_SINGLE;
  else if (c_block == 1) a.c_mode = C_PER_SAMPLE;
  else if (c_block % tile_samples == 0) a.c_mode = C_TILE_UNIFORM;
  else a.c_mode = C_GENERIC;
  a.gate = nullptr; a.gate_epoch = 0; a.gate_want = 0;
  a.fd2 = 0; a.fd_h = 0; a.fd_inv_dx = 0;
  a.seed = 0; a.first_sample = 0; a.slice_stride = 0;
  return a;
}

static int run_flow(CnfModel* m, bool to_base, const float* in, const float* c, int64_t c_block,
                    float* out, float* aux, int aux_mode, int64_t B, void* stream, const NoiseSrc* noise = nullptr) {
  if (!m || (!in && !noise) || (in && noise) || !c || B < 0 || c_block < 1) return CNF_ERR_INVALID;
  if (noise && (to_base || noise->first_sample < 0 || noise->slice_stride < 0)) return CNF_ERR_INVALID;
  if (noise && c_block == 1 && B > 1 && noise->slice_stride != 1) return CNF_ERR_INVALID;
  if (!out && !aux) return CNF_ERR_INVALID;
  if (!m->params_set) return CNF_ERR_INVALID;
  if (B == 0) return CNF_OK;
  if (wait_for_params(m, (hipStream_t)stream) != CNF_OK) return CNF_ERR_HIP;
  const uint32_t* gate = nullptr;
  uint32_t gate_epoch = 0;
  if (c_block == 1 && B > 1) {
    const int r = run_flow_pwl(m, to_base, in, c, B, out, aux, aux_mode, B, (hipStream_t)stream, true, &gate, &gate_epoch, noise);
    if (r != CNF_OK && r != CNF_ERR_UNSUPPORTED) return r;
  } else {
    const int r = run_flow_pwl(m, to_base, in, c, c_block, out, aux, aux_mode, B, (hipStream_t)stream, false, nullptr, nullptr, noise);
    if (r != CNF_ERR_UNSUPPORTED) return r;
  }
  int spl = m->fast_math ? samples_per_lane(m, B) : 1;
  if (spl == 2 && (size_t)(hdr_floats(m->cfg.num_bins) + 3 * m->cfg.dim * TILE * 2) * sizeof(float) +
                      precise_lds_bytes(m->cfg.num_bins) > 160 * 1024) spl = 1;
  FlowArgs a = flow_args<float>(m, in, c, c_block, out, aux, aux_mode, B, TILE * spl);
  a.gate = gate; a.gate_epoch = gate_epoch; a.gate_want = 1;
  if (noise) { a.seed = noise->seed; a.first_sample = noise->first_sample; a.slice_stride = noise->slice_stride; }
  if (!to_base) {
    const int r = launch_flow_dpar(m, a, (hipStream_t)stream);
    if (r != CNF_ERR_UNSUPPORTED) return r;
  }
  return to_base ? launch_flow<true>(m, a, spl, (hipStream_t)stream)
                 : launch_flow<false>(m, a, spl, (hipStream_t)stream);
}

extern "C" int cnf_forward_logdet(CnfModel* m, const float* x, const float* c, int64_t c_block,
                                  float* y, float* logdet, int64_t B, void* stream) {
  return run_flow(m, false, x, c, c_block, y, logdet, AUX_LOGDET, B, stream);
}

extern "C" int cnf_inverse_logdet(CnfModel* m, const float* y, const float* c, int64_t c_block,
                                  float* x, float* logdet, int64_t B, void* stream) {
  return run_flow(m, true, y, c, c_block, x, logdet, AUX_LOGDET, B, stream);
}

extern "C" int cnf_log_prob(CnfModel* m, const float* value, const float* c, int64_t c_block,
                            float* logp, int64_t B, void* stream) {
  if (!logp) return CNF_ERR_INVALID;
  return run_flow(m, true, value, c, c_block, nullptr, logp, AUX_LOGPROB, B, stream);
}

extern "C" int cnf_sample_logprob(CnfModel* m, const float* noise, const float* c, int64_t c_block,
                                  float* y, float* logp, int64_t B, void* stream) {
  if (!y) return CNF_ERR_INVALID;
  return run_flow(m, false, noise, c, c_block, y, logp, AUX_LOGPROB, B, stream);
}

extern "C" int cnf_sample_logprob_seeded(CnfModel* m, uint64_t seed, int64_t first_sample, int64_t slice_stride,
                                         const float* c, int64_t c_block, float* y, float* logp, int64_t B,
                                         void* stream) {
  if (!y) return CNF_ERR_INVALID;
  const NoiseSrc noise{seed, first_sample, slice_stride};
  return run_flow(m, false, nullptr, c, c_block, y, logp, AUX_LOGPROB, B, stream, &noise);
}

extern "C" int cnf_logprob_fd(CnfModel* m, const float* pts, const float* c, int64_t c_block, float dx,
                              float* score, int64_t B, void* stream) {
  if (!m || !pts || !c || !score || B < 0 || c_block < 1 || !(dx > 0.f)) return CNF_ERR_INVALID;
  if (!m->params_set) return CNF_ERR_INVALID;
  if (B == 0) return CNF_OK;
  const int D = m->cfg.dim;
  if (B * 2 * D >= ((int64_t)1 << 40)) return CNF_ERR_INVALID;
  if (wait_for_params(m, (hipStream_t)stream) != CNF_OK) return CNF_ERR_HIP;
  const int64_t n_eval = B * 2 * D;
  int spl = m->fast_math ? samples_per_lane(m, n_eval) : 1;
  if (spl == 2 && (size_t)(hdr_floats(m->cfg.num_bins) + 2 * D * TILE * 2) * sizeof(float) > 160 * 1024) spl = 1;
  FlowArgs a = flow_args<float>(m, pts, c, c_block, nullptr, score, AUX_LOGPROB, n_eval, TILE * spl);
  a.fd2 = 2 * D; a.fd_h = 0.5f * dx; a.fd_inv_dx = 1.0f / dx;
  a.c_mode = c_block >= B ? C_SINGLE : C_GENERIC;
  const int precise = m->precise;
  m->precise = 0;
  const int r = launch_flow<true>(m, a, spl, (hipStream_t)stream);
  m->precise = precise;
  return r;
}


static int loss_terms_pwl(CnfModel* m, const CnfLossSpec* spec, const float* pts, int64_t slice_stride,
                          uint64_t seed, int64_t first_sample, const float* t, int64_t n_slices, int64_t B,
                          double* sums, hipStream_t stream) {
  if (!pwl_config_ok(m)) return CNF_ERR_UNSUPPORTED;
  const int L = m->cfg.num_layers;
  const int kind = spec->kind;
  const bool kin = kind <= CNF_TERM_FLOW_MATCHING;
  const int n_sets = kind == CNF_TERM_KINETIC ? 2 : (kin ? 3 : 1);
  const int threads = cnf::PWL_MAX_THREADS;
  const int64_t ts = 2 * threads;
  const size_t lds = (size_t)(((cnf::hdr_floats(5) + 3) & ~3) + n_sets * L * cnf::PWL_LTBL + 2 * ts) * sizeof(float);
  if (lds > 160 * 1024) return CNF_ERR_UNSUPPORTED;
  SlicePlan plan;
  if (slice_plan(m, stream, B, n_slices, ts, n_sets, &plan) != CNF_OK) return CNF_ERR_UNSUPPORTED;
// ... 219 lines not shown
```

cnf_ot_amd/csrc/cnf_flow_tile.h:

```cpp
#pragma once
#include "cnf_common.h"
#include "cnf_pwl.h"

namespace cnf {

enum CMode { C_SINGLE = 0, C_PER_SAMPLE = 1, C_TILE_UNIFORM = 2, C_GENERIC = 3 };
enum AuxMode { AUX_LOGDET = 0, AUX_LOGPROB = 1 };


template <class R> struct FlowArgsT {
  ModelArgs m;
  const R* in;
  const R* c;
  R* out;
  R* aux;
  int64_t B;
  int64_t c_block;
  int32_t c_mode, aux_mode;
  int32_t div_magic;
  const uint32_t* gate;
  uint32_t gate_epoch;
  int32_t gate_want;
  int32_t fd2;
  R fd_h, fd_inv_dx;
  uint64_t seed;
  int64_t first_sample, slice_stride;
};
typedef FlowArgsT<float> FlowArgs;
typedef FlowArgsT<double> FlowArgsD;

template <class A> __device__ __forceinline__ bool gate_closed(const A& a) {
  return a.gate && ((*a.gate == a.gate_epoch) ? 1 : 0) != a.gate_want;
}

template <class R>
__device__ __forceinline__ void tile_load(const R* __restrict__ g, R* U, int D, uint32_t magic, int TS,
                                          int64_t tile_start, int64_t B) {
  const int64_t base = tile_start * D;
  const int n_el = (int)(B - tile_start < TS ? B - tile_start : TS) * D;
  for (int e = threadIdx.x; e < TS * D; e += TILE) {
    const int s = magic ? (int)__umulhi((uint32_t)e, magic) : e, d = e - s * D;
    U[d * TS + s] = e < n_el ? g[base + e] : (R)0;
  }
}

__device__ __forceinline__ void tile_noise(uint64_t seed, uint64_t first_element, float* U, int D, uint32_t magic,
                                           int TS, int64_t n_valid_samples, int nthreads = TILE) {
  const int n_el = (int)(n_valid_samples < TS ? n_valid_samples : TS) * D;
  const uint64_t blk0 = first_element >> 2;
  const int n_blk = (int)(((first_element + (uint64_t)(TS * D) - 1) >> 2) - blk0) + 1;
  for (int q = threadIdx.x; q < n_blk; q += nthreads) {
    const uint64_t blk = blk0 + (uint64_t)q;
    float z[4];
    philox_normals4(seed, blk, z);
#pragma unroll
    for (int r = 0; r < 4; ++r) {
      const int64_t e = (int64_t)((blk << 2) + r) - (int64_t)first_element;
      if (e >= 0 && e < TS * D) {
        const int s = magic ? (int)__umulhi((uint32_t)e, magic) : (int)e, d = (int)e - s * D;
        U[d * TS + s] = e < n_el ? z[r] : 0.0f;
      }
    }
  }
}

__device__ __forceinline__ float normal_at(uint64_t seed, uint64_t e) {
  float z[4];
  philox_normals4(seed, e >> 2, z);
  return z[e & 3];
}

__device__ __forceinline__ void tile_noise_flow(const FlowArgsT<float>& a, float* U, int D, uint32_t magic, int TS,
                                                int64_t tile_start, int nthreads) {
  const int64_t left = a.B - tile_start;
  const int64_t last = tile_start + (left < TS ? left : TS) - 1;
  const bool one = a.c_block >= a.B;
  const int64_t s0 = one ? 0 : tile_start / a.c_block, s1 = one ? 0 : last / a.c_block;
  if (s0 == s1 || a.slice_stride == a.c_block) {
    const int64_t st = a.first_sample + s0 * a.slice_stride + (tile_start - s0 * a.c_block);
    tile_noise(a.seed, (uint64_t)st * (uint64_t)D, U, D, magic, TS, left, nthreads);
    return;
  }
  const int n_el = (int)(left < TS ? left : TS) * D;
  for (int e = threadIdx.x; e < TS * D; e += nthreads) {
    const int s = magic ? (int)__umulhi((uint32_t)e, magic) : e, d = e - s * D;
    float v = 0.0f;
    if (e < n_el) {
      const int64_t i = tile_start + s, sl = i / a.c_block;
      const int64_t st = a.first_sample + sl * a.slice_stride + (i - sl * a.c_block);
      v = normal_at(a.seed, (uint64_t)st * (uint64_t)D + (uint64_t)d);
    }
    U[d * TS + s] = v;
  }
}
__device__ __forceinline__ void tile_noise_flow(const FlowArgsT<double>&, double*, int, uint32_t, int, int64_t, int) {}

template <class R>
__device__ __forceinline__ void tile_store(R* __restrict__ g, const R* U, int D, uint32_t magic, int TS,
                                           int64_t tile_start, int64_t B) {
  const int64_t base = tile_start * D;
  const int n_el = (int)(B - tile_start < TS ? B - tile_start : TS) * D;
  for (int e = threadIdx.x; e < TS * D; e += TILE) {
    const int s = magic ? (int)__umulhi((uint32_t)e, magic) : e, d = e - s * D;
    if (e < n_el) g[base + e] = U[d * TS + s];
  }
}

template <class R>
__device__ __forceinline__ R load_cond1(const FlowArgsT<R>& a, int64_t tile_start, int64_t i) {
  if (a.fd2) {
    if (a.c_mode == C_SINGLE) return a.c[0];
    return i < a.B ? a.c[(i / a.fd2) / a.c_block] : (R)0;
  }
  switch (a.c_mode) {
    case C_SINGLE: return a.c[0];
    case C_PER_SAMPLE: return i < a.B ? a.c[i] : (R)0;
    case C_TILE_UNIFORM: return a.c[tile_start / a.c_block];
    default: return i < a.B ? a.c[i / a.c_block] : (R)0;
  }
}
template <class T> __device__ __forceinline__ T load_cond(const FlowArgsT<typename Lanes<T>::real>& a, int64_t tile_start, int64_t i);
template <> __device__ __forceinline__ float load_cond<float>(const FlowArgs& a, int64_t ts, int64_t i) {
  return load_cond1(a, ts, i);
}
template <> __device__ __forceinline__ double load_cond<double>(const FlowArgsD& a, int64_t ts, int64_t i) {
  return load_cond1(a, ts, i);
}
template <> __device__ __forceinline__ v2f load_cond<v2f>(const FlowArgs& a, int64_t ts, int64_t i) {
  if (a.c_mode == C_SINGLE || a.c_mode == C_TILE_UNIFORM) return splat<v2f>(load_cond1(a, ts, i));
  return v2f{load_cond1(a, ts, i), load_cond1(a, ts, i + 1)};
}

template <class R>
__device__ __forceinline__ void tile_load_fd(const FlowArgsT<R>& a, R* U, int D, uint32_t magic, int TS, int64_t tile_start) {
  const int n_el = (int)(a.B - tile_start < TS ? a.B - tile_start : TS) * D;
  for (int e = threadIdx.x; e < TS * D; e += TILE) {
    const int s = magic ? (int)__umulhi((uint32_t)e, magic) : e, d = e - s * D;
    R v = (R)0;
    if (e < n_el) {
      const int64_t j = tile_start + s, i = j / a.fd2;
      const int k = (int)(j - i * a.fd2);
      v = a.in[i * D + d];
      if ((k >> 1) == d) v += (k & 1) ? -a.fd_h : a.fd_h;
    }
    U[d * TS + s] = v;
  }
}
__device__ __forceinline__ void store_fd(const FlowArgs& a, int64_t j, v2f lp) {
  if (j + 1 < a.B) a.aux[j >> 1] = (lp.x - lp.y) * a.fd_inv_dx;
}
__device__ __forceinline__ void store_fd(const FlowArgs& a, int64_t j, float lp) {
  const float other = __shfl_xor(lp, 1, 64);
  if (!(j & 1) && j + 1 < a.B) a.aux[j >> 1] = (lp - other) * a.fd_inv_dx;
}
__device__ __forceinline__ void store_fd(const FlowArgsD&, int64_t, double) {}

__device__ __forceinline__ float hsum(float v) { return v; }
__device__ __forceinline__ v2f hsum(v2f v) { return v; }

template <int H, int K, bool TO_BASE, bool FAST, class T, bool MFMA = false, bool PRECISE = false, bool PERIODIC = false, int DFIX = 0>
__device__ __forceinline__ T flow_pass(const ModelArgs& a, const typename Lanes<T>::real* tab,
                                       typename Lanes<T>::real*& U, typename Lanes<T>::real*& O, T c,
                                       const double* e2tab = nullptr, const double* tabd = nullptr,
                                       typename Lanes<T>::real* LO = nullptr, BaseAcc<T>* bacc = nullptr) {
  typedef typename Lanes<T>::real R;
  static_assert(!PRECISE || (TO_BASE && !std::is_same<T, double>::value), "precise path: data -> base, fp32 kernels");
  const SplineConstsT<R>& sc = sc_of<R>(a);
  static_assert(!MFMA || (H == 16 && K == 5), "the MFMA conditioner is built for H = 16, P = 16");
  static_assert(!PERIODIC || (!MFMA && !PRECISE), "periodized: the scalar-weight conditioner, plain positions");
  constexpr int P = 3 * K + 1;
  constexpr bool INV = !TO_BASE;
  constexpr int SPL = Lanes<T>::N;
  constexpr int TS = TILE * SPL;
  uniform_ptr weights = as_uniform(a.prep + hdr_floats(K));
  const int D = DFIX ? DFIX : a.D;
  T acc = splat<T>(0.0f);
  for (int step = 0; step < a.L; ++step) {
    const int l = TO_BASE ? a.L - 1 - step : step;
    const bool odd = l & 1;
    const int first_idx = odd ? D - 1 : 0, idx_step = odd ? -1 : 1;
    R* cu = U + SPL * threadIdx.x;
    R* co = O + SPL * threadIdx.x;
    T o, ld, olo;
    const bool last = step == a.L - 1;
    [[maybe_unused]] R* clo = nullptr;
    if constexpr (PRECISE) {
      clo = LO + SPL * threadIdx.x;
      const T vlo = step == 0 ? splat<T>(0.0f) : lds_get<T>(clo, first_idx, TS);
      table_spline_precise<K, FAST>(tab, tabd, lds_get<T>(cu, first_idx, TS), vlo, sc, o, ld, olo);
      lds_put(clo, first_idx, TS, olo);
      if (last) bacc->add(o, olo);
    } else {
      table_spline<K, INV, FAST, T>(tab, lds_get<T>(cu, first_idx, TS), sc, o, ld);
    }
    lds_put(co, first_idx, TS, o);
    acc += ld;
    uniform_ptr w = weights + l * a.per_layer;
    const float* wq = a.wq + l * a.per_layer_q;
    for (int d = 1; d < D; ++d) {
      const int i = first_idx + d * idx_step;
      T th[P];
      if constexpr (MFMA && !std::is_same<T, double>::value) {
        conditioner_mfma<T>(reinterpret_cast<const f4*>(wq), d, a.M, c, TO_BASE ? co : cu, first_idx, idx_step, TS, th,
                            D >= 3 ? w : nullptr);
        wq += cond_floats_mfma(d, a.M);
        w += cond_floats(d, H, a.M, P);
      } else {
        conditioner<H, P, T, PERIODIC>(w, d, a.M, c, TO_BASE ? co : cu, first_idx, idx_step, TS, th);
        w += cond_floats_p(d, H, a.M, P, PERIODIC);
      }
      if constexpr (PRECISE) {
        const T vlo = step == 0 ? splat<T>(0.0f) : lds_get<T>(clo, i, TS);
        cond_spline_precise<K, FAST, false>(th, lds_get<T>(cu, i, TS), vlo, sc, a.scd, e2tab, o, ld, olo);
        lds_put(clo, i, TS, olo);
        if (last) bacc->add(o, olo);
      } else {
        cond_spline<K, INV, FAST, T>(th, lds_get<T>(cu, i, TS), sc, o, ld);
      }
      lds_put(co, i, TS, o);
      acc += ld;
    }
    R* t = U; U = O; O = t;
  }
  return acc;
}

__device__ __forceinline__ void store_aux(float* aux, int64_t i, int64_t B, float r) {
  if (i < B) aux[i] = r;
}
__device__ __forceinline__ void store_aux(double* aux, int64_t i, int64_t B, double r) {
  if (i < B) aux[i] = r;
}
__device__ __forceinline__ void store_aux(float* aux, int64_t i, int64_t B, v2f r) {
  if (i + 1 < B && ((reinterpret_cast<uintptr_t>(aux + i) & 7) == 0)) *reinterpret_cast<v2f*>(aux + i) = r;
  else { if (i < B) aux[i] = r.x; if (i + 1 < B) aux[i + 1] = r.y; }
}

template <class R>
__device__ __forceinline__ void tile_load_n(const R* __restrict__ g, R* U, int D, uint32_t magic, int TS,
                                            int64_t tile_start, int64_t B, int nthreads) {
  const int64_t base = tile_start * D;
  const int n_el = (int)(B - tile_start < TS ? B - tile_start : TS) * D;
  for (int e = threadIdx.x; e < TS * D; e += nthreads) {
    const int s = magic ? (int)__umulhi((uint32_t)e, magic) : e, d = e - s * D;
    U[d * TS + s] = e < n_el ? g[base + e] : (R)0;
  }
}
template <class R>
__device__ __forceinline__ void tile_store_n(R* __restrict__ g, const R* U, int D, uint32_t magic, int TS,
                                             int64_t tile_start, int64_t B, int nthreads) {
  const int64_t base = tile_start * D;
  const int n_el = (int)(B - tile_start < TS ? B - tile_start : TS) * D;
  for (int e = threadIdx.x; e < n_el; e += nthreads) {
    const int s = magic ? (int)__umulhi((uint32_t)e, magic) : e, d = e - s * D;
    g[base + e] = U[d * TS + s];
  }
}

constexpr int PWL_MAX_THREADS = 1024;

template <int K, bool TO_BASE, bool FAST, bool PRECISE = false, bool SHIFT_FREE_OK = false, int LROWS = PWL_LROWS, int LFIX = 0,
          bool LEAN_OK = false>
__device__ __forceinline__ v2f flow2_tables(const float* tab, const float* tbl, const float* __restrict__ gtbl,
                                            int L, const SplineConsts sc, v2f& u0, v2f& u1,
                                            const PreciseConsts* pc = nullptr, const double* e2tab = nullptr,
                                            const double* tabd = nullptr, BaseAcc<v2f>* bacc = nullptr) {
  constexpr bool INV = !TO_BASE;
  constexpr bool LEAN = LEAN_OK && INV && FAST;
  static_assert(!PRECISE || TO_BASE, "precise path: data -> base");
  v2f acc = splat<v2f>(0.0f);
  [[maybe_unused]] v2f lo0 = splat<v2f>(0.0f), lo1 = lo0;
  if (LFIX) L = LFIX;
#pragma unroll
  for (int step = 0; step < (LFIX ? LFIX : L); ++step) {
    const int l = TO_BASE ? L - 1 - step : step;
    const bool odd = l & 1;
    const v2f uf = odd ? u1 : u0, uo = odd ? u0 : u1;
    v2f of, oo, ld, olo_f, olo_o;
    bool general;
    const float* tl = tbl + l * pwl_ltbl(LROWS);
    const float* gl = gtbl + (int64_t)l * PWL_TBL;
    if constexpr (PRECISE) {
      table_spline_precise<K, FAST>(tab, tabd, uf, odd ? lo1 : lo0, sc, of, ld, olo_f);
      if (step == L - 1) bacc->add(of, olo_f);
      acc += ld;
      v2f th[PWL_P];
      pwl_eval<LROWS>(tl, gl, of, th, general);
      cond_spline_precise<K, FAST, true>(th, uo, odd ? lo0 : lo1, sc, *pc, e2tab, oo, ld, olo_o);
      if (step == L - 1) bacc->add(oo, olo_o);
      lo0 = odd ? olo_o : olo_f;
      lo1 = odd ? olo_f : olo_o;
    } else {
      PwlRows rr;
      v2f qa[K], qb[K];
      if (!TO_BASE) {
        pwl_find<LROWS>(tl, uf, rr, general);
        rr.dua = pwl_logit_pairs<LROWS>(rr.ra, gl, rr.pa, uf.x, qa);
        rr.dub = pwl_logit_pairs<LROWS>(rr.rb, gl, rr.pb, uf.y, qb);
      }
      constexpr bool LOGPROD = LEAN;
      bool tails = true;
      if constexpr (LEAN) tails = __builtin_amdgcn_ballot_w64(maybe_outside(uf, uo, sc.lo, sc.hi)) != 0;
      v2f larg = splat<v2f>(1.0f);
      if constexpr (LOGPROD) {
        table_spline<K, INV, FAST, v2f, true, LEAN>(tab, uf, sc, of, larg, tails);
      } else {
        table_spline<K, INV, FAST, v2f, false, LEAN>(tab, uf, sc, of, ld, tails);
        acc += ld;
      }
      if (TO_BASE) {
        pwl_find<LROWS>(tl, of, rr, general);
        rr.dua = pwl_logit_pairs<LROWS>(rr.ra, gl, rr.pa, of.x, qa);
        rr.dub = pwl_logit_pairs<LROWS>(rr.rb, gl, rr.pb, of.y, qb);
      }
      auto slopes = [&](int ka, int kb, v2f& ta, v2f& tb) {
        ta = pwl_slope_pair<LROWS>(rr.ra, gl, rr.pa, ka, rr.dua);
        tb = pwl_slope_pair<LROWS>(rr.rb, gl, rr.pb, kb, rr.dub);
      };
      if (!SHIFT_FREE_OK || __builtin_amdgcn_ballot_w64(general) != 0)
      {
        cond_spline_rows<K, INV, FAST, false, false, LEAN>(qa, qb, slopes, uo, sc, oo, ld, tails);
        if constexpr (LOGPROD) { const v2f lg = Math<FAST>::log(larg); ld += INV ? -lg : lg; }
      } else {
        cond_spline_rows<K, INV, FAST, true, LOGPROD, LEAN>(qa, qb, slopes, uo, sc, oo, ld, tails);
        if constexpr (LOGPROD) { const v2f lg = Math<FAST>::log(larg * ld); ld = INV ? -lg : lg; }
      }
    }
    acc += ld;
    u0 = odd ? oo : of;
    u1 = odd ? of : oo;
  }
  return acc;
}

}
```

cnf_ot_amd/csrc/cnf_host.h:

```cpp
#pragma once
#include "cnf_common.h"

void pwl_workspace(CnfModel* m, hipStream_t stream, float** tables, int64_t* sets, uint32_t** flag = nullptr,
                   uint32_t* epoch = nullptr);

int grad_finish(const CnfModel* m, int64_t n_slabs, const float* params, float* grad, uint32_t* amax, hipStream_t stream);

size_t pwl_stats_bytes(int L);
int pass_vjp_pwl(CnfModel* m, int to_base, const float* pts, const float* c, int64_t c_block, const float* ybar,
                 const float* ldbar, float* xbar, float* grad, const float* params, int64_t B, hipStream_t stream,
                 float seed_coef = 0.0f, double* seed_sums = nullptr, const float* built = nullptr);

int term_residual_launch(int32_t kind, const float* r, const float* aux, int64_t n, int64_t count, int32_t D,
                         int32_t subtype, float p0, float loss_coef, double* sums, float* rbar, float* auxbar,
                         uint32_t* amax, hipStream_t stream);

int cnf_internal_build_tables(CnfModel* m, hipStream_t stream, const float* c, int64_t n, float** tables);
int cnf_internal_flow_shared(CnfModel* m, hipStream_t stream, const float* in, const float* c, int64_t slice_len,
                             int64_t n_slices, const float* tables, float* out);






struct IaPairLayout {
  int32_t P;
  int64_t force_off;
  double cv, cf;
};
int interaction_pairs(const CnfInteractionSpec* spec, int32_t S, const float* x, int64_t N, const float* q, int64_t Q,
                      int32_t D, bool force, void* workspace, int64_t workspace_bytes, hipStream_t stream,
                      IaPairLayout* lay);
```

cnf_ot_amd/csrc/cnf_model.hip:

```cpp
#include "cnf_host.h"
#include "cnf_pwl.h"

#include <math.h>
#include <new>
#include <stdlib.h>
#include <string.h>

using namespace cnf;

static int config_valid(const CnfConfig* c) {
  if (!c) return 0;
  if (c->dim < 1 || c->dim > 64) return 0;
  if (c->num_layers < 1 || c->num_layers > 64) return 0;
  if (c->hidden_size < 1 || c->mlp_num_layers < 1 || c->mlp_num_layers > 16) return 0;
  if (c->num_bins < 1 || c->num_bins > 64) return 0;
  if (!(c->range_min < c->range_max)) return 0;
  if (!(c->min_bin_size > 0.f) || !(c->min_knot_slope > 0.f) || !(c->min_knot_slope < 1.f)) return 0;
  if (c->num_bins * c->min_bin_size > c->range_max - c->range_min) return 0;
  if (c->periodized != 0 && c->periodized != 1) return 0;
  return 1;
}

extern "C" int cnf_config_supported(const CnfConfig* c) {
  return config_valid(c) && shape_compiled(*c) ? 1 : 0;
}

extern "C" void cnf_config_default(CnfConfig* c, int32_t dim) {
  if (!c) return;
  c->dim = dim; c->num_layers = 2; c->hidden_size = 16; c->mlp_num_layers = 2; c->num_bins = 5;
  c->range_min = -10.f; c->range_max = 10.f; c->min_bin_size = 1e-4f; c->min_knot_slope = 1e-4f;
  c->periodized = 0;
}

extern "C" int64_t cnf_param_count(const CnfConfig* c) {
  if (!config_valid(c)) return CNF_ERR_INVALID;
  const int P = 3 * c->num_bins + 1;
  int64_t n = P;
  for (int d = 1; d < c->dim; ++d)
    n += (int64_t)c->num_layers * cond_floats_p(d, c->hidden_size, c->mlp_num_layers, P, c->periodized != 0);
  return n;
}

extern "C" const char* cnf_strerror(int code) {
  switch (code) {
    case CNF_OK: return "ok";
    case CNF_ERR_INVALID: return "invalid argument";
    case CNF_ERR_UNSUPPORTED: return "no kernel compiled for this (hidden_size, num_bins)";
    case CNF_ERR_NOMEM: return "out of memory";
    case CNF_ERR_HIP: return "HIP runtime error";
    default: return "unknown error";
  }
}

extern "C" const char* cnf_build_arch(void) { return "gfx950"; }

extern "C" int cnf_model_create(const CnfConfig* cfg, CnfModel** out) {
  if (!out) return CNF_ERR_INVALID;
  *out = nullptr;
  if (!config_valid(cfg)) return CNF_ERR_INVALID;
  if (!cnf_config_supported(cfg)) return CNF_ERR_UNSUPPORTED;
  CnfModel* m = new (std::nothrow) CnfModel();
  if (!m) return CNF_ERR_NOMEM;
  m->cfg = *cfg;
  const int K = cfg->num_bins, P = 3 * K + 1;
  m->n_params = cnf_param_count(cfg);
  m->per_layer = 0;
  for (int d = 1; d < cfg->dim; ++d)
    m->per_layer += cond_floats_p(d, cfg->hidden_size, cfg->mlp_num_layers, P, cfg->periodized != 0);
  m->sc.lo = cfg->range_min; m->sc.hi = cfg->range_max;
  m->sc.min_bin = cfg->min_bin_size; m->sc.min_slope = cfg->min_knot_slope;
  m->sc.span_eff = (float)(((double)cfg->range_max - (double)cfg->range_min) - (double)K * (double)cfg->min_bin_size);
  m->sc.sp_offset = (float)log(exp(1.0 - (double)cfg->min_knot_slope) - 1.0);
  m->fast_math = 1;
  if (hipGetDevice(&m->device) != hipSuccess) { delete m; return CNF_ERR_HIP; }
  hipDeviceProp_t prop;
  if (hipGetDeviceProperties(&prop, m->device) != hipSuccess) { delete m; return CNF_ERR_HIP; }
  m->num_cus = prop.multiProcessorCount;
  m->use_mfma = 2;
  m->use_pwl = 1;
  m->use_dpar = 1;
  m->div_magic = cfg->dim == 1 ? 0u : (uint32_t)((((uint64_t)1 << 32) + (uint64_t)cfg->dim - 1) / (uint64_t)cfg->dim);
  m->per_layer_q = 0; m->mfma_off = 0;
  size_t q_floats = 0;
  if (cfg->hidden_size == 16 && P == 16 && cfg->dim > 1 && !cfg->periodized) {
    for (int d = 1; d < cfg->dim; ++d) m->per_layer_q += cond_floats_mfma(d, cfg->mlp_num_layers);
    m->mfma_off = (hdr_floats(K) + (m->n_params - P) + 3) & ~(int64_t)3;
    q_floats = (size_t)m->per_layer_q * cfg->num_layers;
  }
  m->tabd_off = (hdr_floats(K) + (m->n_params - P) + 4 + (int64_t)q_floats + 1) & ~(int64_t)1;
  m->e2_off = m->tabd_off + 2 * hdr_floats(K);
  m->precise = 1;
  const size_t bytes = (size_t)(m->e2_off + 2 * cnf::EXP2_N) * sizeof(float) + 64;
  m->scd.lo = (double)cfg->range_min; m->scd.hi = (double)cfg->range_max;
  m->scd.min_bin = (double)cfg->min_bin_size; m->scd.min_slope = (double)cfg->min_knot_slope;
  m->scd.span_eff = (m->scd.hi - m->scd.lo) - (double)K * m->scd.min_bin;
  m->scd.sp_offset = log(exp(1.0 - m->scd.min_slope) - 1.0);
  if (hipMalloc((void**)&m->prep, bytes) != hipSuccess) { delete m; return CNF_ERR_NOMEM; }
  {
    double e2[cnf::EXP2_N];
    for (int i = 0; i < cnf::EXP2_N; ++i) e2[i] = exp2(-(double)i / (double)cnf::EXP2_STEPS);
    if (hipMemcpy(m->prep + m->e2_off, e2, sizeof(e2), hipMemcpyHostToDevice) != hipSuccess) {
      (void)hipFree(m->prep); delete m; return CNF_ERR_HIP;
    }
  }
  if (hipEventCreateWithFlags(&m->prep_event, hipEventDisableTiming) != hipSuccess) {
    (void)hipFree(m->prep); delete m; return CNF_ERR_HIP;
  }
  *out = m;
  return CNF_OK;
}

static void prof_clear(CnfModel* m) {
  for (auto& r : m->prof) {
    if (r.e0) (void)hipEventDestroy(r.e0);
    if (r.e1) (void)hipEventDestroy(r.e1);
    if (r.e2) (void)hipEventDestroy(r.e2);
  }
  m->prof.clear();
}

extern "C" void cnf_model_destroy(CnfModel* m) {
  if (!m) return;
  if (m->prep) (void)hipFree(m->prep);
  if (m->grad_slabs) (void)hipFree(m->grad_slabs);
  if (m->pwl_stats) (void)hipFree(m->pwl_stats);
  for (auto& kv : m->pwl_ws) {
    if (kv.second.tables) (void)hipFree(kv.second.tables);
    for (float* p : kv.second.retired) (void)hipFree(p);
  }
  if (m->prep_event) (void)hipEventDestroy(m->prep_event);
  prof_clear(m);
  delete m;
}

extern "C" int cnf_model_last_path(const CnfModel* m) { return m ? m->last_path : CNF_ERR_INVALID; }

extern "C" int cnf_model_set_profiling(CnfModel* m, int on) {
  if (!m) return CNF_ERR_INVALID;
  m->profiling = on ? 1 : 0;
  if (!on) prof_clear(m);
  return CNF_OK;
}

extern "C" int cnf_model_read_profile(CnfModel* m, double* flow_ms, double* build_ms, int64_t* launches,
                                      int64_t* samples) {
  if (!m) return CNF_ERR_INVALID;
  double f = 0.0, b = 0.0;
  int64_t n = 0, smp = 0;
  for (auto& r : m->prof) {
    if (hipEventSynchronize(r.e2) != hipSuccess) return CNF_ERR_HIP;
    float ms = 0.f;
    if (r.e0) { if (hipEventElapsedTime(&ms, r.e0, r.e1) != hipSuccess) return CNF_ERR_HIP; b += ms; }
    if (hipEventElapsedTime(&ms, r.e1, r.e2) != hipSuccess) return CNF_ERR_HIP;
    f += ms; ++n; smp += r.samples;
  }
  prof_clear(m);
  if (flow_ms) *flow_ms = f;
  if (build_ms) *build_ms = b;
  if (launches) *launches = n;
  if (samples) *samples = smp;
  return CNF_OK;
}

extern "C" int cnf_model_set_fast_math(CnfModel* m, int on) {
  if (!m) return CNF_ERR_INVALID;
  m->fast_math = on ? 1 : 0;
  return CNF_OK;
}

extern "C" int cnf_model_set_mfma(CnfModel* m, int mode) {
  if (!m || mode < 0 || mode > 2) return CNF_ERR_INVALID;
  m->use_mfma = mode;
  return CNF_OK;
}

extern "C" int cnf_model_set_pwl(CnfModel* m, int mode) {
  if (!m || mode < 0 || mode > 2) return CNF_ERR_INVALID;
  m->use_pwl = mode;
  return CNF_OK;
}

extern "C" int cnf_model_set_pwl_builder(CnfModel* m, int mode) {
  if (!m || mode < 0 || mode > 2) return CNF_ERR_INVALID;
  m->pwl_builder = mode;
  return CNF_OK;
}

extern "C" int cnf_model_last_pwl_builder(const CnfModel* m) { return m ? m->last_pwl_builder : CNF_ERR_INVALID; }

extern "C" int cnf_model_set_precise(CnfModel* m, int on) {
  if (!m) return CNF_ERR_INVALID;
  m->precise = on ? 1 : 0;
  return CNF_OK;
}

extern "C" int cnf_model_set_dpar(CnfModel* m, int mode) {
  if (!m || mode < 0 || mode > 2) return CNF_ERR_INVALID;
  m->use_dpar = mode;
  return CNF_OK;
}

extern "C" int cnf_model_set_samples_per_lane(CnfModel* m, int spl) {
  if (!m || spl < 0 || spl > 2) return CNF_ERR_INVALID;
  m->force_spl = spl;
  return CNF_OK;
}


void pwl_workspace(CnfModel* m, hipStream_t stream, float** tables, int64_t* sets, uint32_t** flag, uint32_t* epoch) {
  std::lock_guard<std::mutex> lock(m->pwl_mu);
  auto it = m->pwl_ws.find((void*)stream);
  if (it == m->pwl_ws.end()) { *tables = nullptr; *sets = 0; return; }
  *tables = it->second.tables; *sets = it->second.sets;
  if (flag) { *flag = reinterpret_cast<uint32_t*>(it->second.tables + it->second.sets * m->cfg.num_layers * (int64_t)cnf::PWL_TBL);
              *epoch = ++it->second.epoch; }
}

extern "C" int64_t cnf_model_table_bytes(const CnfModel* m) {
  return m ? (int64_t)sizeof(float) * m->cfg.num_layers * cnf::PWL_TBL : 0;
}

extern "C" int cnf_model_reserve(CnfModel* m, void* stream, int64_t n_sets) {
  if (!m || n_sets < 0) return CNF_ERR_INVALID;
  std::lock_guard<std::mutex> lock(m->pwl_mu);
  CnfModel::PwlWorkspace& ws = m->pwl_ws[stream];
  if (ws.sets >= n_sets && n_sets > 0) return CNF_OK;
  if (ws.tables && n_sets > 0) {
    ws.retired.push_back(ws.tables);
    ws.tables = nullptr; ws.sets = 0;
  }
  if (n_sets == 0) {
    if (hipStreamSynchronize((hipStream_t)stream) != hipSuccess) return CNF_ERR_HIP;
    if (ws.tables) (void)hipFree(ws.tables);
    for (float* p : ws.retired) (void)hipFree(p);
    m->pwl_ws.erase(stream);
    return CNF_OK;
  }
  if (hipMalloc((void**)&ws.tables, (size_t)cnf_model_table_bytes(m) * (size_t)n_sets + 64) != hipSuccess) {
    ws.tables = nullptr; ws.sets = 0;
    return CNF_ERR_NOMEM;
  }
  if (hipMemset(reinterpret_cast<char*>(ws.tables) + (size_t)cnf_model_table_bytes(m) * (size_t)n_sets, 0, 64) != hipSuccess) {
    (void)hipFree(ws.tables); ws.tables = nullptr; ws.sets = 0;
    return CNF_ERR_HIP;
  }
  ws.sets = n_sets; ws.epoch = 0;
  return CNF_OK;
}

extern "C" int64_t cnf_model_reserved(CnfModel* m, void* stream) {
  if (!m) return CNF_ERR_INVALID;
  float* t; int64_t sets;
  pwl_workspace(m, (hipStream_t)stream, &t, &sets);
  return sets;
}

static_assert(cnf::PWL_H == 16, "pwl_network (cnf_common.h) states the tables' network");

extern "C" int cnf_model_has_tables(const CnfModel* m) { return m && pwl_network(m->cfg) ? 1 : 0; }

extern "C" int cnf_model_term_on_tables(const CnfModel* m, int64_t slice_len, int64_t n_points, int with_grad) {
  return m && pwl_term_on_tables(m, slice_len, n_points, with_grad != 0) ? 1 : 0;
}
```

cnf_ot_amd/flows.py:

```python
import math
from collections import namedtuple
from typing import Optional, Sequence, Tuple, Union

import numpy as np
import torch

from . import _capi
from .params import FlowConfig, Params, flatten

Flow = namedtuple("Flow", [
  "log_prob", "sample", "sample_and_log_prob", "forward", "inverse",
  "forward_jac", "inverse_jac", "gauge_potential",
])

_MASK64 = (1 << 64) - 1

_WRITE_EPOCH = {}


def mark_updated(flat: torch.Tensor) -> None:
  _WRITE_EPOCH[flat.data_ptr()] = _WRITE_EPOCH.get(flat.data_ptr(), 0) + 1


def _c_config(cfg: FlowConfig) -> _capi.CnfConfig:
# ... 23 lines not shown

  def __exit__(self, *exc):
    if self.ctx is not None:
      self.ctx.__exit__(*exc)
      self.ctx = None
    return False


def seed_to_u64(seed) -> Tuple[int, int]:
  offset = 0
  if isinstance(seed, tuple) and len(seed) == 2 and not torch.is_tensor(seed[0]):
    seed, offset = seed
  if torch.is_tensor(seed) or isinstance(seed, np.ndarray):
    words = [int(v) for v in np.asarray(seed.cpu() if torch.is_tensor(seed) else seed).reshape(-1)]
    if len(words) == 1:
      seed = words[0]
    elif len(words) == 2:
      seed = ((words[0] & 0xFFFFFFFF) << 32) | (words[1] & 0xFFFFFFFF)
    else:
      raise ValueError("seed array must have 1 or 2 words")
  return int(seed) & _MASK64, int(offset)


_MULTI_TYPES = {}


class DeviceRng:

  SLOTS = 32

  def __init__(self, device):
    self.device = torch.device(device)
    self.state = torch.zeros(2, dtype=torch.int64, device=self.device)
    self._pin = torch.zeros(self.SLOTS, dtype=torch.int64).pin_memory()
    self._done = [None] * self.SLOTS
    self._n = 0

  def set_key(self, rng) -> "DeviceRng":
    seed, off = seed_to_u64(rng)
    seed = (seed + 0x9E3779B97F4A7C15 * off) & _MASK64
    k = self._n % self.SLOTS
    self._n += 1
    if self._done[k] is not None:
      self._done[k].synchronize()
    else:
      self._done[k] = torch.cuda.Event()
    self._pin[k] = seed - (1 << 64) if seed >= (1 << 63) else seed
    self.state[1:2].copy_(self._pin[k:k + 1], non_blocking=True)
    self._done[k].record(torch.cuda.current_stream(self.device))
    return self

  @property
  def ptr(self) -> int:
    return self.state.data_ptr()


class FlowEngine:

  def __init__(self, cfg: FlowConfig, device: Union[str, torch.device, int] = "cuda"):
    self.lib = _capi.lib()
    self.cfg = cfg
    self.device = torch.device(device)
    if self.device.type != "cuda":
      raise ValueError("cnf_ot_amd runs on MI355X only: pass a cuda (ROCm) device")
    if self.device.index is None:
      self.device = torch.device("cuda", torch.cuda.current_device())
    ccfg = _c_config(cfg)
    handle = _capi.ctypes.c_void_p()
    with _OnDevice(self.device):
      _capi.check(self.lib.cnf_model_create(_capi.ctypes.byref(ccfg), _capi.ctypes.byref(handle)),
                  "cnf_model_create")
    self._h = handle
    self._flat = None
    self._flat_key = None
    self._reserved = {}
    self._pwl_mode = 1
    self._precise = True
    self._tables_ok = bool(self.lib.cnf_model_has_tables(self._h))
    self._grad_enabled = False

  def __del__(self):
    h = getattr(self, "_h", None)
    if h:
      try:
        self.lib.cnf_model_destroy(h)
      except Exception:
        pass
      self._h = None

  def load(self, params, assume_unchanged: bool = False) -> "FlowEngine":
    flat = flatten(self.cfg, params, self.device)
    key = (flat.data_ptr(), flat._version, _WRITE_EPOCH.get(flat.data_ptr(), 0))
    if assume_unchanged and self._flat is not None and key == self._flat_key:
      return self
    with _OnDevice(self.device):
      _capi.check(self.lib.cnf_model_set_params(self._h, flat.data_ptr(), _stream_ptr(self.device)),
                  "cnf_model_set_params")
    self._flat = flat
    self._flat_key = key
    return self

  def reserve(self, n_slices: int, sets_per_slice: int = 1) -> int:
    if not self._tables_ok:
      return 0
    stream = _stream_ptr(self.device)
    have = self._reserved.get(stream, 0)
    want = min(int(n_slices), 2048) * int(sets_per_slice)
    if want <= have or torch.cuda.is_current_stream_capturing():
      return have
    want = max(16, 1 << (want - 1).bit_length())
    with _OnDevice(self.device):
      _capi.check(self.lib.cnf_model_reserve(self._h, stream, want), "cnf_model_reserve")
    self._reserved[stream] = want
    return want

  def term_on_tables(self, slice_len: int, n_points: int, with_grad: bool) -> bool:
    return bool(self.lib.cnf_model_term_on_tables(self._h, int(slice_len), int(n_points), 1 if with_grad else 0))

  def grad_ready(self, grad: torch.Tensor) -> None:
    if self._flat is None:
      raise RuntimeError("load(params) before asking for gradients")
    if not self._grad_enabled:
      with _OnDevice(self.device):
        _capi.check(self.lib.cnf_grad_enable(self._h, 0), "cnf_grad_enable")
      self._grad_enabled = True
    self._check_out(grad, (self.cfg.param_count(),), "grad")

  def last_path(self) -> str:
    return _capi.PATH_NAMES.get(self.lib.cnf_model_last_path(self._h), "?")

  def set_profiling(self, on: bool) -> None:
    _capi.check(self.lib.cnf_model_set_profiling(self._h, 1 if on else 0), "cnf_model_set_profiling")

  def read_profile(self):
    f, b = _capi.ctypes.c_double(), _capi.ctypes.c_double()
    n, smp = _capi.ctypes.c_int64(), _capi.ctypes.c_int64()
    _capi.check(self.lib.cnf_model_read_profile(self._h, _capi.ctypes.byref(f), _capi.ctypes.byref(b),
                                                _capi.ctypes.byref(n), _capi.ctypes.byref(smp)),
                "cnf_model_read_profile")
    return f.value, b.value, n.value, smp.value

  def set_fast_math(self, on: bool) -> None:
    _capi.check(self.lib.cnf_model_set_fast_math(self._h, 1 if on else 0), "cnf_model_set_fast_math")

  def set_mfma(self, mode) -> None:
    _capi.check(self.lib.cnf_model_set_mfma(self._h, int(mode)), "cnf_model_set_mfma")

  def set_pwl(self, mode: int) -> None:
    _capi.check(self.lib.cnf_model_set_pwl(self._h, int(mode)), "cnf_model_set_pwl")
    self._pwl_mode = int(mode)

  def set_pwl_builder(self, mode: int) -> None:
    _capi.check(self.lib.cnf_model_set_pwl_builder(self._h, int(mode)), "cnf_model_set_pwl_builder")

  def last_pwl_builder(self) -> int:
    return self.lib.cnf_model_last_pwl_builder(self._h)

  def build_tables(self, c: torch.Tensor, c_offset: float = 0.0, out: torch.Tensor = None) -> torch.Tensor:
    c = c.to(self.device, torch.float32).contiguous().reshape(-1)
    per = self.lib.cnf_model_table_bytes(self._h) // (4 * self.cfg.num_layers)
    shape = (c.numel(), self.cfg.num_layers, per)
    if out is None:
      out = torch.empty(shape, dtype=torch.float32, device=self.device)
    if tuple(out.shape) != shape or out.dtype != torch.float32 or out.device != self.device or not out.is_contiguous():
      raise ValueError(f"out must be a contiguous float32 tensor of shape {shape} on {self.device}")
    _capi.check(self.lib.cnf_internal_build_tables_into(self._h, _stream_ptr(self.device), c.data_ptr(), float(c_offset),
                                                        c.numel(), out.data_ptr()), "cnf_internal_build_tables_into")
    return out

  def set_dpar(self, mode: int) -> None:
    _capi.check(self.lib.cnf_model_set_dpar(self._h, int(mode)), "cnf_model_set_dpar")

  def set_precise(self, on: bool) -> None:
    _capi.check(self.lib.cnf_model_set_precise(self._h, 1 if on else 0), "cnf_model_set_precise")
    self._precise = bool(on)

  def set_samples_per_lane(self, spl: int) -> None:
    _capi.check(self.lib.cnf_model_set_samples_per_lane(self._h, int(spl)), "cnf_model_set_samples_per_lane")

  def _points(self, t, what, keep_f64=False) -> torch.Tensor:
    if torch.is_tensor(t) and t.device == self.device and t.dim() == 2 and t.shape[1] == self.cfg.dim and \
        t.is_contiguous() and (t.dtype == torch.float32 or (keep_f64 and t.dtype == torch.float64)):
      return t
    if not torch.is_tensor(t):
      t = torch.as_tensor(np.asarray(t))
    if t.dim() != 2 or t.shape[1] != self.cfg.dim:
      raise ValueError(f"{what}: expected shape [B, {self.cfg.dim}], got {tuple(t.shape)}")
    dtype = torch.float64 if (keep_f64 and t.dtype == torch.float64) else torch.float32
    return t.to(device=self.device, dtype=dtype).contiguous()

  def cond(self, cond, B: int, dtype=torch.float32) -> Tuple[torch.Tensor, int]:
    if torch.is_tensor(cond) and cond.device == self.device and cond.dtype == dtype and cond.is_contiguous():
      c = cond if cond.dim() == 1 else cond.reshape(-1)
    else:
      if not torch.is_tensor(cond):
        cond = torch.as_tensor(np.asarray(cond, dtype=np.float64))
      c = cond.to(device=self.device, dtype=dtype).reshape(-1).contiguous()
    n = c.numel()
    if n == 0:
      raise ValueError("cond is empty")
    if n == 1:
      return c, max(B, 1)
    if n == B:
      return c, 1
    if B % n == 0:
      return c, B // n
    raise ValueError(f"cond with {n} values does not tile a batch of {B}")

  def _check_out(self, t, shape, what, dtype=torch.float32):
    if (t.dtype != dtype or t.device != self.device or not t.is_contiguous()
        or tuple(t.shape) != tuple(shape)):
      raise ValueError(f"{what}: need a contiguous {dtype} {tuple(shape)} tensor on {self.device}")
    return t

  def _run(self, fn, name, pts, cond, want_pts, want_aux, out=None, aux=None):
    B = pts.shape[0]
    if pts.dtype == torch.float64:
      fn, name = getattr(self.lib, name + "_f64"), name + "_f64"
    c, c_block = self.cond(cond, B, pts.dtype)
    if self._pwl_mode and B > 0 and pts.dtype == torch.float32:
      self.reserve(-(-B // c_block) if c_block > 1 else 1)
    if out is not None:
      self._check_out(out, pts.shape, name + " out", pts.dtype)
    elif want_pts:
      out = torch.empty_like(pts)
    if aux is not None:
      self._check_out(aux, (B,), name + " aux", pts.dtype)
    elif want_aux:
      aux = torch.empty(B, dtype=pts.dtype, device=self.device)
    if B > 0:
      with _OnDevice(self.device):
        _capi.check(fn(self._h, pts.data_ptr(), c.data_ptr(), c_block,
                       out.data_ptr() if out is not None else None,
                       aux.data_ptr() if aux is not None else None, B,
                       _stream_ptr(self.device)), name)
    return out, aux

  def forward_logdet(self, x, cond, want_logdet=True):
    x = self._points(x, "forward", keep_f64=True)
    return self._run(self.lib.cnf_forward_logdet, "cnf_forward_logdet", x, cond, True, want_logdet)

  def inverse_logdet(self, y, cond, want_logdet=True):
    y = self._points(y, "inverse", keep_f64=True)
    return self._run(self.lib.cnf_inverse_logdet, "cnf_inverse_logdet", y, cond, True, want_logdet)

  def log_prob(self, value, cond) -> torch.Tensor:
    value = self._points(value, "log_prob", keep_f64=True)
    B = value.shape[0]
    f64 = value.dtype == torch.float64
    c, c_block = self.cond(cond, B, value.dtype)
    if self._pwl_mode and B > 0 and not f64:
      self.reserve(-(-B // c_block) if c_block > 1 else 1)
    lp = torch.empty(B, dtype=value.dtype, device=self.device)
    if B > 0:
      fn = self.lib.cnf_log_prob_f64 if f64 else self.lib.cnf_log_prob
      with _OnDevice(self.device):
        _capi.check(fn(self._h, value.data_ptr(), c.data_ptr(), c_block, lp.data_ptr(), B,
                       _stream_ptr(self.device)), "cnf_log_prob")
    return lp

  def sample_logprob(self, noise, cond, want_logp=True, out=None, logp_out=None):
    noise = self._points(noise, "sample", keep_f64=True)
    return self._run(self.lib.cnf_sample_logprob, "cnf_sample_logprob", noise, cond, True, want_logp,
                     out=out, aux=logp_out)

  def sample_logprob_seeded(self, seed, n_samples: int, cond, want_logp=True, first_sample: int = 0,
                            slice_stride: Optional[int] = None, out=None, logp_out=None):
    seed, off = seed_to_u64(seed)
    B = int(n_samples)
    c, c_block = self.cond(cond, B)
    if slice_stride is None:
      slice_stride = min(c_block, B) if c_block > 1 else 1
    if self._pwl_mode and B > 0:
      self.reserve(-(-B // c_block) if c_block > 1 else 1)
    D = self.cfg.dim
    if out is not None:
      self._check_out(out, (B, D), "sample_logprob_seeded out")
    else:
      out = torch.empty(B, D, dtype=torch.float32, device=self.device)
    if logp_out is not None:
      self._check_out(logp_out, (B,), "sample_logprob_seeded logp")
    elif want_logp:
      logp_out = torch.empty(B, dtype=torch.float32, device=self.device)
    if B > 0:
      with _OnDevice(self.device):
        _capi.check(self.lib.cnf_sample_logprob_seeded(self._h, seed, off + int(first_sample), int(slice_stride),
                                                       c.data_ptr(), c_block, out.data_ptr(),
                                                       logp_out.data_ptr() if logp_out is not None else None, B,
                                                       _stream_ptr(self.device)), "cnf_sample_logprob_seeded")
    return out, logp_out

  def slice_conds(self, t) -> torch.Tensor:
    if torch.is_tensor(t):
      if t.device == self.device and t.dtype == torch.float32 and t.is_contiguous():
        return t if t.dim() == 1 else t.reshape(-1)
      return t.to(device=self.device, dtype=torch.float32).reshape(-1).contiguous()
    a = np.ascontiguousarray(np.asarray(t, dtype=np.float32).reshape(-1))
    key = a.tobytes()
    cache = self.__dict__.setdefault("_cond_cache", {})
    d = cache.get(key)
    if d is None:
      if len(cache) >= 32:
        cache.clear()
      d = cache[key] = torch.from_numpy(a.copy()).to(self.device)
    return d

# ... 667 lines not shown
```

include/cnf_ot_amd_debug.h:

```cpp
#ifndef CNF_OT_AMD_DEBUG_H
#define CNF_OT_AMD_DEBUG_H

#include "cnf_ot_amd.h"

#ifdef __cplusplus
extern "C" {
#endif

int cnf_model_set_fast_math(CnfModel *m, int on);

int cnf_model_set_samples_per_lane(CnfModel *m, int spl);

int cnf_model_set_mfma(CnfModel *m, int mode);

int cnf_model_set_pwl(CnfModel *m, int mode);

int cnf_model_set_pwl_builder(CnfModel *m, int mode);
int cnf_model_last_pwl_builder(const CnfModel *m);

int cnf_internal_build_tables_into(CnfModel *m, void *stream, const float *c, float c_offset, int64_t n, float *out);

int cnf_model_set_dpar(CnfModel *m, int mode);

int cnf_model_set_profiling(CnfModel *m, int on);
int cnf_model_read_profile(CnfModel *m, double *flow_ms, double *build_ms,
                           int64_t *launches, int64_t *samples);

#ifdef __cplusplus
}
#endif
#endif
```

Baseline: 96.77 billion samples/s.

## Replace first-layer inverse spline with certified degree-5 piecewise polynomial table

Adds a kernel that, once per parameter set, fits degree-5 Chebyshev-node polynomials for the first (condition-independent) layer's inverse spline output and log-derivative over a 1024-cell grid split at the knots. It checks each piece against probe points and only marks the table certified if every error stays within budget. The flow kernel stages this table into LDS and, when certified, evaluates the first layer with a cell lookup plus Horner steps instead of bin search and closed-form sqrt/log. This targets per-sample transcendental and search cost in the first layer, at the price of extra LDS use, a one-time build kernel, and approximation error kept near f32 precision.

```diff
diff --git a/cnf_ot_amd/_capi.py b/cnf_ot_amd/_capi.py
--- a/cnf_ot_amd/_capi.py
+++ b/cnf_ot_amd/_capi.py
@@ -233,6 +233,9 @@
   "cnf_model_set_dpar": (ctypes.c_int, [_P, ctypes.c_int]),
   "cnf_model_set_pwl_builder": (ctypes.c_int, [_P, ctypes.c_int]),
   "cnf_model_last_pwl_builder": (ctypes.c_int, [_P]),
+  "cnf_model_set_first_table": (ctypes.c_int, [_P, ctypes.c_int]),
+  "cnf_internal_first_table_floats": (_I64, []),
+  "cnf_internal_first_table": (ctypes.c_int, [_P, _P, _P]),
   "cnf_internal_build_tables_into": (ctypes.c_int, [_P, _P, _P, ctypes.c_float, _I64, _P]),
   "cnf_model_set_profiling": (ctypes.c_int, [_P, ctypes.c_int]),
   "cnf_model_read_profile": (ctypes.c_int, [_P, ctypes.POINTER(ctypes.c_double), ctypes.POINTER(ctypes.c_double),
diff --git a/cnf_ot_amd/build.py b/cnf_ot_amd/build.py
--- a/cnf_ot_amd/build.py
+++ b/cnf_ot_amd/build.py
@@ -12,7 +12,7 @@
 SOURCES = ["cnf_flow.hip", "cnf_grad.hip", "cnf_grad_pwl.hip", "cnf_importance.hip", "cnf_mmd.hip", "cnf_knn.hip", "cnf_interaction.hip", "cnf_interaction_vjp.hip", "cnf_stein.hip", "cnf_kde.hip", "cnf_hopf_cole.hip", "cnf_fp_particles.hip",
            "cnf_mv_particles.hip", "cnf_sinkhorn.hip", "cnf_sliced.hip", "cnf_step.hip", "cnf_model.hip", "cnf_rng.hip"]
 HEADERS = ["cnf_device.h", "cnf_terms.h", "cnf_common.h", "cnf_host.h", "cnf_flow_tile.h", "cnf_backward.h", "cnf_pwl.h",
-           "cnf_pwl_build.h", "cnf_fp_stats.h", "cnf_pairs.h", "cnf_interaction_pairs.h", os.path.join("..", "..", "include", "cnf_ot_amd.h")]
+           "cnf_pwl_build.h", "cnf_first_table.h", "cnf_fp_stats.h", "cnf_pairs.h", "cnf_interaction_pairs.h", os.path.join("..", "..", "include", "cnf_ot_amd.h")]
 VARIANT_PATH = os.path.join(LIB_DIR, "BUILD_VARIANT")
 ARCH = "gfx950"
 
diff --git a/cnf_ot_amd/csrc/cnf_common.h b/cnf_ot_amd/csrc/cnf_common.h
--- a/cnf_ot_amd/csrc/cnf_common.h
+++ b/cnf_ot_amd/csrc/cnf_common.h
@@ -42,6 +42,10 @@
   int64_t tabd_off;
   int64_t e2_off;
   int precise;
+  int64_t ft_off;
+  int ft_built;
+  int ft_wanted;
+  int first_table_mode;
   float* prep;
   int64_t n_params;
   int64_t per_layer;
diff --git a/cnf_ot_amd/csrc/cnf_device.h b/cnf_ot_amd/csrc/cnf_device.h
--- a/cnf_ot_amd/csrc/cnf_device.h
+++ b/cnf_ot_amd/csrc/cnf_device.h
@@ -287,11 +287,27 @@
   template <int K> __device__ __forceinline__ v2f get(int f) const { return v2f{px[tab_off(f, K)], py[tab_off(f, K)]}; }
 };
 
+template <int K, bool INV, bool ARG, class T>
+__device__ __forceinline__ void table_spline_tails(const typename Lanes<T>::real* tab, T v,
+                                                   const SplineConstsT<typename Lanes<T>::real> sc, T& out, T& ld) {
+  typedef typename Lanes<T>::real R;
+  const auto below = vle(v, sc.lo);
+  const auto above = vge(v, sc.hi);
+  const R* tl = tab + tab_off(F_TAIL, K);
+  const T lo_out = INV ? vfma(v - sc.lo, splat<T>(tl[T_INV_DLO]), splat<T>(sc.lo))
+                       : vfma(v - sc.lo, splat<T>(tl[T_DLO]), splat<T>(sc.lo));
+  const T hi_out = INV ? vfma(v - sc.hi, splat<T>(tl[T_INV_DHI]), splat<T>(sc.hi))
+                       : vfma(v - sc.hi, splat<T>(tl[T_DHI]), splat<T>(sc.hi));
+  out = vsel(below, lo_out, out);
+  ld = vsel(below, ARG ? splat<T>(tl[T_DLO]) : splat<T>(INV ? -tl[T_LOG_DLO] : tl[T_LOG_DLO]), ld);
+  out = vsel(above, hi_out, out);
+  ld = vsel(above, ARG ? splat<T>(tl[T_DHI]) : splat<T>(INV ? -tl[T_LOG_DHI] : tl[T_LOG_DHI]), ld);
+}
+
 template <int K, bool INV, bool FAST, class T, bool ARG = false, bool LEAN = false>
 __device__ __forceinline__ void table_spline(const typename Lanes<T>::real* tab, T v,
                                              const SplineConstsT<typename Lanes<T>::real> sc, T& out, T& ld,
                                              bool tails = true) {
-  typedef typename Lanes<T>::real R;
   typename Lanes<T>::index k;
   if constexpr (std::is_same<T, v2f>::value) k = bin_of_pairs<K>(tab + tab_off(INV ? F_YKB : F_XKB, K), v);
   else k = bin_of<K>(tab + tab_off(INV ? F_YK : F_XK, K), v);
@@ -314,19 +330,8 @@
                                row.template get<K>(F_BH), ibw,
                                row.template get<K>(F_S), row.template get<K>(F_ST), row.template get<K>(F_D0),
                                row.template get<K>(F_D1), row.template get<K>(F_L2S), out, ld);
-  if (LEAN ? tails : maybe_outside(v, sc.lo, sc.hi)) {
-    const auto below = vle(v, sc.lo);
-    const auto above = vge(v, sc.hi);
-    const R* tl = tab + tab_off(F_TAIL, K);
-    const T lo_out = INV ? vfma(v - sc.lo, splat<T>(tl[T_INV_DLO]), splat<T>(sc.lo))
-                         : vfma(v - sc.lo, splat<T>(tl[T_DLO]), splat<T>(sc.lo));
-    const T hi_out = INV ? vfma(v - sc.hi, splat<T>(tl[T_INV_DHI]), splat<T>(sc.hi))
-                         : vfma(v - sc.hi, splat<T>(tl[T_DHI]), splat<T>(sc.hi));
-    out = vsel(below, lo_out, out);
-    ld = vsel(below, ARG ? splat<T>(tl[T_DLO]) : splat<T>(INV ? -tl[T_LOG_DLO] : tl[T_LOG_DLO]), ld);
-    out = vsel(above, hi_out, out);
-    ld = vsel(above, ARG ? splat<T>(tl[T_DHI]) : splat<T>(INV ? -tl[T_LOG_DHI] : tl[T_LOG_DHI]), ld);
-  }
+  if (LEAN ? tails : maybe_outside(v, sc.lo, sc.hi))
+    table_spline_tails<K, INV, ARG, T>(tab, v, sc, out, ld);
 }
 
 __device__ __forceinline__ v2f step_mask(v2f d, v2f big) {
diff --git a/cnf_ot_amd/csrc/cnf_first_table.h b/cnf_ot_amd/csrc/cnf_first_table.h
--- /dev/null
+++ b/cnf_ot_amd/csrc/cnf_first_table.h
@@ -0,0 +1,218 @@
+#pragma once
+#include "cnf_device.h"
+
+namespace cnf {
+
+constexpr int FT_K = 5;
+constexpr int FT_CELLS = 1024;
+constexpr int FT_DEG = 5;
+constexpr int FT_ROW = 2 * (FT_DEG + 1);
+constexpr int FT_ROWS = FT_CELLS + FT_K - 1;
+constexpr int FT_PROBES = 17;
+constexpr double FT_BUDGET = 2.4e-7;
+__host__ __device__ inline double ft_edge_guard(double lo, double hi) {
+  const double m = fabs(lo) > fabs(hi) ? fabs(lo) : fabs(hi);
+  return 1.1920928955078125e-7 * (2.0 * m + (hi - lo));
+}
+constexpr int FT_WORDS = 4;
+enum { FT_W_CERT = 0, FT_W_FAILS = 1, FT_W_DONE = 2 };
+constexpr uint32_t FT_CERTIFIED = 0x31305446u;
+constexpr int FT_GRID_FLOATS = 4 * FT_CELLS;
+constexpr int FT_LDS_FLOATS = FT_GRID_FLOATS + FT_ROWS * FT_ROW;
+constexpr int FT_FLOATS = FT_WORDS + FT_LDS_FLOATS;
+static_assert(FT_ROW % 4 == 0 && FT_WORDS % 4 == 0, "grid entries and rows are read with 16-byte loads");
+
+constexpr int FT_PPB = 8;
+constexpr int FT_BLOCKS = (FT_ROWS + FT_PPB - 1) / FT_PPB;
+static_assert(FT_BLOCKS * FT_PPB >= FT_CELLS, "block b also writes the grid entries of cells 8 b .. 8 b + 7");
+
+__device__ __forceinline__ void ft_closed(const double* xk, const double* yk, const double* d, int k, double v,
+                                          double& out, double& ld) {
+  const double x0 = xk[k], y0 = yk[k];
+  const double bw = xk[k + 1] - x0, bh = yk[k + 1] - y0, s = bh / bw;
+  const double d0 = d[k], d1 = d[k + 1], st = d1 + d0 - 2.0 * s;
+  const double dy = v - y0, c2 = 2.0 * s * dy;
+  const double b = d0 * bh - st * dy, a = s * bh - b;
+  const double z = c2 / (b + sqrt(b * b + a * (c2 + c2))), omz = 1.0 - z;
+  const double num2 = d1 * z * z + 2.0 * s * z * omz + d0 * omz * omz;
+  const double den = s + st * z * omz;
+  out = x0 + bw * z;
+  ld = -log(s * s * num2 / (den * den));
+}
+
+template <int K>
+__global__ __launch_bounds__(32 * FT_PPB) void first_table_kernel(const double* __restrict__ tabd, float* __restrict__ ft,
+                                                                 double lo, double hi) {
+  static_assert(K == FT_K, "FT_ROWS counts the K - 1 knot splits");
+  constexpr int N = FT_DEG + 1;
+  __shared__ double xk[K + 1], yk[K + 1], dk[K + 1];
+  __shared__ double fo[FT_PPB][N], fl[FT_PPB][N];
+  __shared__ float cf[FT_PPB][FT_ROW];
+  if (threadIdx.x <= K) {
+    xk[threadIdx.x] = tabd[tab_off(F_XK, K) + threadIdx.x];
+    yk[threadIdx.x] = tabd[tab_off(F_YK, K) + threadIdx.x];
+    dk[threadIdx.x] = threadIdx.x < K ? tabd[tab_off(F_D0, K) + threadIdx.x] : tabd[tab_off(F_D1, K) + K - 1];
+  }
+  __syncthreads();
+  const double cw = (hi - lo) / FT_CELLS, guard = ft_edge_guard(lo, hi);
+  int kc[K - 1];
+  bool fail = false;
+#pragma unroll
+  for (int j = 0; j < K - 1; ++j) {
+    const double q = floor((yk[j + 1] - lo) / cw);
+    const int c = q >= 0.0 && q < (double)FT_CELLS ? (int)q : 0;
+    fail |= !(q >= 0.0 && q < (double)FT_CELLS);
+    kc[j] = c;
+    if (j > 0 && kc[j - 1] == c) fail = true;
+    const double e0 = lo + c * cw, e1 = c + 1 < FT_CELLS ? lo + (c + 1) * cw : hi;
+    if (!(yk[j + 1] - e0 >= guard) || !(e1 - yk[j + 1] >= guard)) fail = true;
+  }
+  const int lp = threadIdx.x >> 5, ln = threadIdx.x & 31;
+  const int p = blockIdx.x * FT_PPB + lp;
+  float* grid = ft + FT_WORDS;
+  float* rows = grid + FT_GRID_FLOATS;
+
+  int m = 0, half = 0, knot = 0;
+#pragma unroll
+  for (int j = 0; j < K - 1; ++j) {
+    const int q = kc[j] + j;
+    if (q + 1 <= p) ++m;
+    if (p == q + 1) { half = 2; knot = j + 1; }
+    else if (p == q && half == 0) { half = 1; knot = j + 1; }
+  }
+  int c = p - m;
+  c = c < 0 ? 0 : (c > FT_CELLS - 1 ? FT_CELLS - 1 : c);
+  double a = lo + c * cw, b = c + 1 < FT_CELLS ? lo + (c + 1) * cw : hi;
+  int bin = 0;
+#pragma unroll
+  for (int j = 0; j < K - 1; ++j) bin += kc[j] < c ? 1 : 0;
+  double refd = 0.5 * (a + b);
+  if (half == 1) { b = yk[knot]; refd = yk[knot]; bin = knot - 1; }
+  if (half == 2) { a = yk[knot]; refd = yk[knot]; bin = knot; }
+  if (bin > K - 1) bin = K - 1;
+  const float ref32 = (float)refd;
+  const double ref = (double)ref32;
+  const double mid = 0.5 * (a + b), rad = 0.5 * (b - a);
+
+  const double nodes[N] = {-1.0, -0.8090169943749475, -0.30901699437494745, 0.30901699437494745, 0.8090169943749475, 1.0};
+  double xs[N];
+  double x = mid + rad * ((2.0 * (double)(ln - N) + 1.0) / (double)FT_PROBES - 1.0);
+#pragma unroll
+  for (int i = 0; i < N; ++i) {
+    const double xn = i == 0 ? a : (i == N - 1 ? b : mid + rad * nodes[i]);
+    xs[i] = xn - ref;
+    if (ln == i) x = xn;
+  }
+  double vo, vl;
+  ft_closed(xk, yk, dk, bin, x, vo, vl);
+  if (ln < N) { fo[lp][ln] = vo; fl[lp][ln] = vl; }
+  __syncthreads();
+  if (ln < 2) {
+    double cc[N], mm[N];
+#pragma unroll
+    for (int i = 0; i < N; ++i) { cc[i] = ln == 0 ? fo[lp][i] : fl[lp][i]; mm[i] = 0.0; }
+#pragma unroll
+    for (int j = 1; j < N; ++j)
+#pragma unroll
+      for (int i = N - 1; i >= j; --i) cc[i] = (cc[i] - cc[i - 1]) / (xs[i] - xs[i - j]);
+    mm[0] = cc[N - 1];
+#pragma unroll
+    for (int i = N - 2; i >= 0; --i) {
+#pragma unroll
+      for (int q = N - 1 - i; q >= 1; --q) mm[q] = mm[q - 1] - xs[i] * mm[q];
+      mm[0] = cc[i] - xs[i] * mm[0];
+    }
+#pragma unroll
+    for (int q = 0; q < N; ++q) {
+      const float v = (float)mm[q];
+      if (!(fabsf(v) <= 3.0e38f)) fail = true;
+      cf[lp][2 * q + ln] = v;
+      if (p < FT_ROWS) rows[(int64_t)p * FT_ROW + 2 * q + ln] = v;
+    }
+  }
+  __syncthreads();
+  if (ln >= N && ln < N + FT_PROBES && p < FT_ROWS) {
+    const double dv = x - ref;
+    double po = (double)cf[lp][2 * FT_DEG], pl = (double)cf[lp][2 * FT_DEG + 1];
+#pragma unroll
+    for (int q = FT_DEG - 1; q >= 0; --q) { po = po * dv + (double)cf[lp][2 * q]; pl = pl * dv + (double)cf[lp][2 * q + 1]; }
+    if (!(fabs(po - vo) <= FT_BUDGET * fmax(1.0, fabs(vo)))) fail = true;
+    if (!(fabs(pl - vl) <= FT_BUDGET * fmax(1.0, fabs(vl)))) fail = true;
+  }
+  if (ln == 31) {
+    const int cell = blockIdx.x * FT_PPB + lp;
+    if (cell < FT_CELLS) {
+      int base = cell;
+      bool split = false;
+      double r = 0.5 * ((lo + cell * cw) + (cell + 1 < FT_CELLS ? lo + (cell + 1) * cw : hi));
+#pragma unroll
+      for (int j = 0; j < K - 1; ++j) {
+        base += kc[j] < cell ? 1 : 0;
+        if (kc[j] == cell && !split) { split = true; r = yk[j + 1]; }
+      }
+      f4 e;
+      e.x = (float)r;
+      e.y = split ? (float)r : __builtin_inff();
+      e.z = __uint_as_float((uint32_t)(base * FT_ROW * 4));
+      e.w = 0.0f;
+      reinterpret_cast<f4*>(grid)[cell] = e;
+    }
+  }
+  const int any = __syncthreads_or(p < FT_ROWS && fail ? 1 : 0);
+  if (threadIdx.x == 0) {
+    uint32_t* words = reinterpret_cast<uint32_t*>(ft);
+    if (any) atomicAdd(&words[FT_W_FAILS], 1u);
+    __threadfence();
+    if (atomicAdd(&words[FT_W_DONE], 1u) == gridDim.x - 1) {
+      __threadfence();
+      words[FT_W_CERT] = atomicAdd(&words[FT_W_FAILS], 0u) == 0u ? FT_CERTIFIED : 0u;
+    }
+  }
+}
+
+__device__ __forceinline__ void ft_stage(float* dst, const float* __restrict__ ft, int tid, int nthreads) {
+  const f4* src = reinterpret_cast<const f4*>(ft + FT_WORDS);
+  f4* d = reinterpret_cast<f4*>(dst);
+  for (int i = tid; i < FT_LDS_FLOATS / 4; i += nthreads) d[i] = src[i];
+}
+
+struct FtConsts { float cs, c0; uint32_t grid, rows; };
+__device__ __forceinline__ FtConsts ft_consts(const float* ftl, const SplineConsts sc) {
+  FtConsts f;
+  f.cs = (float)FT_CELLS / (sc.hi - sc.lo);
+  f.c0 = -sc.lo * f.cs;
+  f.grid = (uint32_t)(uintptr_t)ftl;
+  f.rows = f.grid + FT_GRID_FLOATS * 4;
+  return f;
+}
+
+typedef const f4 __attribute__((address_space(3))) * ft_f4_ptr;
+
+__device__ __forceinline__ f4 ft_cell(const FtConsts f, float v) {
+  uint32_t cell;
+  asm("v_cvt_u32_f32 %0, %1" : "=v"(cell) : "v"(fmaf(v, f.cs, f.c0)));
+  cell = cell > (uint32_t)(FT_CELLS - 1) ? (uint32_t)(FT_CELLS - 1) : cell;
+  return *(ft_f4_ptr)(uintptr_t)(f.grid + (cell << 4));
+}
+__device__ __forceinline__ uint32_t ft_row(const FtConsts f, float v, f4 g) {
+  return f.rows + __float_as_uint(g.z) + (v >= g.y ? (uint32_t)(FT_ROW * 4) : 0u);
+}
+__device__ __forceinline__ v2f ft_horner(uint32_t ra, float dv) {
+  const ft_f4_ptr row = (ft_f4_ptr)(uintptr_t)ra;
+  const f4 r0 = row[0], r1 = row[1], r2 = row[2];
+  const v2f d2 = v2f{dv, dv};
+  v2f acc = __builtin_elementwise_fma(v2f{r2.z, r2.w}, d2, v2f{r2.x, r2.y});
+  acc = __builtin_elementwise_fma(acc, d2, v2f{r1.z, r1.w});
+  acc = __builtin_elementwise_fma(acc, d2, v2f{r1.x, r1.y});
+  acc = __builtin_elementwise_fma(acc, d2, v2f{r0.z, r0.w});
+  return __builtin_elementwise_fma(acc, d2, v2f{r0.x, r0.y});
+}
+__device__ __forceinline__ void ft_eval(const FtConsts f, v2f v, v2f& out, v2f& ld) {
+  const f4 gx = ft_cell(f, v.x), gy = ft_cell(f, v.y);
+  const v2f px = ft_horner(ft_row(f, v.x, gx), v.x - gx.x);
+  const v2f py = ft_horner(ft_row(f, v.y, gy), v.y - gy.x);
+  out = v2f{px.x, py.x};
+  ld = v2f{px.y, py.y};
+}
+
+}
diff --git a/cnf_ot_amd/csrc/cnf_flow.hip b/cnf_ot_amd/csrc/cnf_flow.hip
--- a/cnf_ot_amd/csrc/cnf_flow.hip
+++ b/cnf_ot_amd/csrc/cnf_flow.hip
@@ -24,7 +24,8 @@
 __global__ void prepare_kernel(const float* __restrict__ params, float* __restrict__ prep,
                                int K, int64_t n_params, double lo, double hi, double min_bin,
                                double min_slope, int D, int L, int M, int64_t per_layer,
-                               int64_t per_layer_q, int64_t mfma_off, int64_t tabd_off, int H, int periodic) {
+                               int64_t per_layer_q, int64_t mfma_off, int64_t tabd_off, int H, int periodic,
+                               int64_t ft_off) {
   const int P = 3 * K + 1;
   const int hdr = hdr_floats(K);
   constexpr int MAXK = 64;
@@ -62,6 +63,7 @@
   }
 
   __shared__ double ex[2][MAXK], dl[MAXK + 1], mxs[2];
+  if (ft_off > 0 && threadIdx.x < FT_WORDS) reinterpret_cast<uint32_t*>(prep + ft_off)[threadIdx.x] = 0u;
   if (threadIdx.x < 2) {
     const float* u = params + threadIdx.x * K;
     double mx = u[0];
@@ -286,6 +288,7 @@
   uint64_t seed;
   int64_t first_sample, slice_stride;
   int32_t in_shared;
+  const float* ft;
 };
 
 __global__ void cond_uniform_kernel(const float* __restrict__ c, int64_t B, uint32_t* flag, uint32_t epoch) {
@@ -317,6 +320,18 @@
     tabd = e2tab + EXP2_N;
     for (int i = tid; i < EXP2_N; i += PWL_THREADS) e2tab[i] = a.m.e2tab[i];
     for (int i = tid; i < hdr_floats(K); i += PWL_THREADS) tabd[i] = a.m.tabd[i];
+  }
+  constexpr bool FTAB = !TO_BASE && FAST && !PRECISE && LFIX == 2 && LROWS >= PWL_NPIECE && K == FT_K;
+  [[maybe_unused]] bool use_ft = false;
+  [[maybe_unused]] FtConsts fc{};
+  if constexpr (FTAB) {
+    if (a.ft)
+      use_ft = __builtin_amdgcn_readfirstlane((int)reinterpret_cast<const uint32_t*>(a.ft)[FT_W_CERT]) == (int)FT_CERTIFIED;
+    if (use_ft) {
+      float* ftl = lds_raw + pwl_flow_lds_floats(K, LFIX, LROWS, false);
+      ft_stage(ftl, a.ft, tid, PWL_THREADS);
+      fc = ft_consts(ftl, sc);
+    }
   }
 
   const int total = a.n_slices * a.tiles_per_slice;
@@ -390,7 +405,9 @@
     const int slice = tl.slice;
     if (slice != cur) {
       __syncthreads();
-      pwl_stage<LROWS>(tbl, a.tables + (int64_t)slice * L * PWL_TBL, L, tid, PWL_THREADS);
+      int stid = tid;
+      if constexpr (FTAB) asm volatile("" : "+v"(stid));
+      pwl_stage<LROWS>(tbl, a.tables + (int64_t)slice * L * PWL_TBL, L, stid, PWL_THREADS);
       cur = slice;
       __syncthreads();
     }
@@ -405,8 +422,13 @@
     if (!TO_BASE && lp && a.aux) base = (u0 * u0 + u1 * u1) * -0.5f - (float)(2 * HALF_LOG_2PI);
     if (!TO_BASE) asm volatile("" : "+v"(base));
     BaseAcc<v2f> bacc;
-    const v2f acc = flow2_tables<K, TO_BASE, FAST, PRECISE, true, LROWS, LFIX, true>(tab, tbl, a.tables + (int64_t)slice * L * PWL_TBL, L, sc,
-                                                            u0, u1, &a.m.scd, e2tab, tabd, &bacc);
+    v2f acc;
+    if (FTAB && use_ft)
+      acc = flow2_tables<K, TO_BASE, FAST, PRECISE, true, LROWS, LFIX, true, FTAB>(tab, tbl, a.tables + (int64_t)slice * L * PWL_TBL, L, sc,
+                                                              u0, u1, &a.m.scd, e2tab, tabd, &bacc, fc);
+    else
+      acc = flow2_tables<K, TO_BASE, FAST, PRECISE, true, LROWS, LFIX, true>(tab, tbl, a.tables + (int64_t)slice * L * PWL_TBL, L, sc,
+                                                              u0, u1, &a.m.scd, e2tab, tabd, &bacc);
     asm volatile("" : "+v"(xn));
     __builtin_amdgcn_sched_barrier(0);
     auto emit = [&](bool has_aux, bool is_lp, bool has_out, bool whole) {
@@ -829,6 +851,14 @@
 
 using namespace cnf;
 
+void first_table_enqueue(CnfModel* m, hipStream_t stream) {
+  hipLaunchKernelGGL(first_table_kernel<FT_K>, dim3(FT_BLOCKS), dim3(32 * FT_PPB), 0, stream,
+                     reinterpret_cast<const double*>(m->prep + m->tabd_off), m->prep + m->ft_off,
+                     (double)m->cfg.range_min, (double)m->cfg.range_max);
+  m->ft_built = 1;
+  m->ft_wanted = 1;
+}
+
 extern "C" int cnf_model_set_params(CnfModel* m, const float* params, void* stream) {
   if (!m || !params) return CNF_ERR_INVALID;
   const int K = m->cfg.num_bins;
@@ -841,11 +871,15 @@
                      m->n_params, (double)m->cfg.range_min, (double)m->cfg.range_max,
                      (double)m->cfg.min_bin_size, (double)m->cfg.min_knot_slope, m->cfg.dim,
                      m->cfg.num_layers, m->cfg.mlp_num_layers, m->per_layer, m->per_layer_q, m->mfma_off,
-                     m->tabd_off, m->cfg.hidden_size, m->cfg.periodized);
+                     m->tabd_off, m->cfg.hidden_size, m->cfg.periodized, m->ft_off);
   if (m->cfg.periodized && m->cfg.dim > 1)
     hipLaunchKernelGGL(circular_slopes_kernel, dim3((unsigned)(m->cfg.num_layers * (m->cfg.dim - 1))), dim3(64), 0,
                        (hipStream_t)stream, params, m->prep, K, m->cfg.hidden_size, m->cfg.dim, m->cfg.num_layers,
                        m->cfg.mlp_num_layers, m->per_layer);
+  if (m->ft_off > 0) {
+    m->ft_built = 0;
+    if (m->ft_wanted && pwl_config_ok(m)) first_table_enqueue(m, (hipStream_t)stream);
+  }
   if (hipGetLastError() != hipSuccess) return CNF_ERR_HIP;
   hipStreamCaptureStatus cap = hipStreamCaptureStatusNone;
   if (hipStreamIsCapturing((hipStream_t)stream, &cap) != hipSuccess) cap = hipStreamCaptureStatusNone;
@@ -997,12 +1031,13 @@
   if (!pwl_config_ok(m)) return CNF_ERR_UNSUPPORTED;
   const int L = m->cfg.num_layers;
   const bool precise = to_base && m->precise;
-  auto lds_for = [&](int lrows) {
-    return (size_t)(((cnf::hdr_floats(5) + 3) & ~3) + L * cnf::pwl_ltbl(lrows)) * sizeof(float) +
-           (precise ? precise_lds_bytes(5) : 0);
+  auto lds_for = [&](int lrows, bool first_table) {
+    return (size_t)cnf::pwl_flow_lds_floats(5, L, lrows, first_table) * sizeof(float) + (precise ? precise_lds_bytes(5) : 0);
   };
-  const bool full = lds_for(cnf::PWL_NPIECE) <= 160 * 1024;
-  size_t lds = lds_for(full ? cnf::PWL_NPIECE : cnf::PWL_LROWS);
+  const bool full = lds_for(cnf::PWL_NPIECE, false) <= 160 * 1024;
+  const float* ft = !to_base && full && L == 2 && m->ft_off > 0 && m->first_table_mode == 0 ? m->prep + m->ft_off : nullptr;
+  if (ft && !m->ft_built) first_table_enqueue(m, stream);
+  size_t lds = lds_for(full ? cnf::PWL_NPIECE : cnf::PWL_LROWS, ft != nullptr);
   if (lds > 160 * 1024) return CNF_ERR_UNSUPPORTED;
   const int64_t slice_len = c_block < B ? c_block : B;
   const int64_t n_slices = (B + slice_len - 1) / slice_len;
@@ -1043,7 +1078,7 @@
     a.in = in ? in + (in_shared ? 0 : first * 2) : nullptr; a.out = out ? out + first * 2 : nullptr; a.aux = aux ? aux + first : nullptr;
     a.seed = noise ? noise->seed : 0; a.slice_stride = noise ? noise->slice_stride : 0;
     a.first_sample = noise ? noise->first_sample + s0 * noise->slice_stride : 0;
-    a.tables = tables;
+    a.tables = tables; a.ft = ft;
     a.B = (B - first) < ns * slice_len ? (B - first) : ns * slice_len;
     a.slice_len = slice_len;
     a.n_slices = (int32_t)ns; a.tiles_per_slice = (int32_t)tps; a.aux_mode = aux_mode;
diff --git a/cnf_ot_amd/csrc/cnf_flow_tile.h b/cnf_ot_amd/csrc/cnf_flow_tile.h
--- a/cnf_ot_amd/csrc/cnf_flow_tile.h
+++ b/cnf_ot_amd/csrc/cnf_flow_tile.h
@@ -1,6 +1,7 @@
 #pragma once
 #include "cnf_common.h"
 #include "cnf_pwl.h"
+#include "cnf_first_table.h"
 
 namespace cnf {
 
@@ -259,14 +260,22 @@
 
 constexpr int PWL_MAX_THREADS = 1024;
 
+constexpr int pwl_flow_lds_floats(int K, int L, int lrows, bool first_table) {
+  return ((hdr_floats(K) + 3) & ~3) + L * pwl_ltbl(lrows) + (first_table ? FT_LDS_FLOATS : 0);
+}
+static_assert(pwl_flow_lds_floats(FT_K, 2, PWL_NPIECE, true) * sizeof(float) <= 160 * 1024,
+              "the L = 2 kernel holds both conditioner tables and the inverse table");
+
 template <int K, bool TO_BASE, bool FAST, bool PRECISE = false, bool SHIFT_FREE_OK = false, int LROWS = PWL_LROWS, int LFIX = 0,
-          bool LEAN_OK = false>
+          bool LEAN_OK = false, bool FTAB = false>
 __device__ __forceinline__ v2f flow2_tables(const float* tab, const float* tbl, const float* __restrict__ gtbl,
                                             int L, const SplineConsts sc, v2f& u0, v2f& u1,
                                             const PreciseConsts* pc = nullptr, const double* e2tab = nullptr,
-                                            const double* tabd = nullptr, BaseAcc<v2f>* bacc = nullptr) {
+                                            const double* tabd = nullptr, BaseAcc<v2f>* bacc = nullptr,
+                                            const FtConsts ft = FtConsts{}) {
   constexpr bool INV = !TO_BASE;
   constexpr bool LEAN = LEAN_OK && INV && FAST;
+  static_assert(!FTAB || LEAN, "the inverse table: the lean sampling direction");
   static_assert(!PRECISE || TO_BASE, "precise path: data -> base");
   v2f acc = splat<v2f>(0.0f);
   [[maybe_unused]] v2f lo0 = splat<v2f>(0.0f), lo1 = lo0;
@@ -293,6 +302,7 @@
     } else {
       PwlRows rr;
       v2f qa[K], qb[K];
+      if constexpr (FTAB) ft_eval(ft, uf, of, ld);
       if (!TO_BASE) {
         pwl_find<LROWS>(tl, uf, rr, general);
         rr.dua = pwl_logit_pairs<LROWS>(rr.ra, gl, rr.pa, uf.x, qa);
@@ -302,7 +312,10 @@
       bool tails = true;
       if constexpr (LEAN) tails = __builtin_amdgcn_ballot_w64(maybe_outside(uf, uo, sc.lo, sc.hi)) != 0;
       v2f larg = splat<v2f>(1.0f);
-      if constexpr (LOGPROD) {
+      if constexpr (FTAB) {
+        if (tails) table_spline_tails<K, INV, false, v2f>(tab, uf, sc, of, ld);
+        acc += ld;
+      } else if constexpr (LOGPROD) {
         table_spline<K, INV, FAST, v2f, true, LEAN>(tab, uf, sc, of, larg, tails);
       } else {
         table_spline<K, INV, FAST, v2f, false, LEAN>(tab, uf, sc, of, ld, tails);
@@ -320,10 +333,10 @@
       if (!SHIFT_FREE_OK || __builtin_amdgcn_ballot_w64(general) != 0)
       {
         cond_spline_rows<K, INV, FAST, false, false, LEAN>(qa, qb, slopes, uo, sc, oo, ld, tails);
-        if constexpr (LOGPROD) { const v2f lg = Math<FAST>::log(larg); ld += INV ? -lg : lg; }
+        if constexpr (LOGPROD && !FTAB) { const v2f lg = Math<FAST>::log(larg); ld += INV ? -lg : lg; }
       } else {
         cond_spline_rows<K, INV, FAST, true, LOGPROD, LEAN>(qa, qb, slopes, uo, sc, oo, ld, tails);
-        if constexpr (LOGPROD) { const v2f lg = Math<FAST>::log(larg * ld); ld = INV ? -lg : lg; }
+        if constexpr (LOGPROD) { const v2f lg = Math<FAST>::log(FTAB ? ld : larg * ld); ld = INV ? -lg : lg; }
       }
     }
     acc += ld;
diff --git a/cnf_ot_amd/csrc/cnf_host.h b/cnf_ot_amd/csrc/cnf_host.h
--- a/cnf_ot_amd/csrc/cnf_host.h
+++ b/cnf_ot_amd/csrc/cnf_host.h
@@ -19,6 +19,8 @@
 int cnf_internal_flow_shared(CnfModel* m, hipStream_t stream, const float* in, const float* c, int64_t slice_len,
                              int64_t n_slices, const float* tables, float* out);
 
+void first_table_enqueue(CnfModel* m, hipStream_t stream);
+
 
 
 
diff --git a/cnf_ot_amd/csrc/cnf_model.hip b/cnf_ot_amd/csrc/cnf_model.hip
--- a/cnf_ot_amd/csrc/cnf_model.hip
+++ b/cnf_ot_amd/csrc/cnf_model.hip
@@ -1,5 +1,6 @@
 #include "cnf_host.h"
 #include "cnf_pwl.h"
+#include "cnf_first_table.h"
 
 #include <math.h>
 #include <new>
@@ -90,7 +91,12 @@
   m->tabd_off = (hdr_floats(K) + (m->n_params - P) + 4 + (int64_t)q_floats + 1) & ~(int64_t)1;
   m->e2_off = m->tabd_off + 2 * hdr_floats(K);
   m->precise = 1;
-  const size_t bytes = (size_t)(m->e2_off + 2 * cnf::EXP2_N) * sizeof(float) + 64;
+  int64_t n_floats = m->e2_off + 2 * cnf::EXP2_N;
+  if (pwl_network(*cfg) && cfg->num_layers == 2 && K == cnf::FT_K) {
+    m->ft_off = (n_floats + 3) & ~(int64_t)3;
+    n_floats = m->ft_off + cnf::FT_FLOATS;
+  }
+  const size_t bytes = (size_t)n_floats * sizeof(float) + 64;
   m->scd.lo = (double)cfg->range_min; m->scd.hi = (double)cfg->range_max;
   m->scd.min_bin = (double)cfg->min_bin_size; m->scd.min_slope = (double)cfg->min_knot_slope;
   m->scd.span_eff = (m->scd.hi - m->scd.lo) - (double)K * m->scd.min_bin;
@@ -180,6 +186,24 @@
   return CNF_OK;
 }
 
+extern "C" int cnf_model_set_first_table(CnfModel* m, int mode) {
+  if (!m || mode < 0 || mode > 1) return CNF_ERR_INVALID;
+  m->first_table_mode = mode;
+  return CNF_OK;
+}
+
+extern "C" int64_t cnf_internal_first_table_floats(void) { return cnf::FT_FLOATS; }
+
+extern "C" int cnf_internal_first_table(CnfModel* m, void* stream, float* out) {
+  if (!m || !out || !m->params_set) return CNF_ERR_INVALID;
+  if (m->ft_off <= 0 || !pwl_config_ok(m)) return CNF_ERR_UNSUPPORTED;
+  if (wait_for_params(m, (hipStream_t)stream) != CNF_OK) return CNF_ERR_HIP;
+  if (!m->ft_built) first_table_enqueue(m, (hipStream_t)stream);
+  if (hipMemcpyAsync(out, m->prep + m->ft_off, sizeof(float) * (size_t)cnf::FT_FLOATS, hipMemcpyDeviceToHost,
+                     (hipStream_t)stream) != hipSuccess) return CNF_ERR_HIP;
+  return hipStreamSynchronize((hipStream_t)stream) == hipSuccess ? CNF_OK : CNF_ERR_HIP;
+}
+
 extern "C" int cnf_model_set_pwl_builder(CnfModel* m, int mode) {
   if (!m || mode < 0 || mode > 2) return CNF_ERR_INVALID;
   m->pwl_builder = mode;
diff --git a/cnf_ot_amd/first_table.py b/cnf_ot_amd/first_table.py
--- /dev/null
+++ b/cnf_ot_amd/first_table.py
@@ -0,0 +1,169 @@
+import numpy as np
+
+FT_CELLS = 1024
+FT_DEG = 5
+FT_ROW = 2 * (FT_DEG + 1)
+FT_PROBES = 17
+FT_BUDGET = 2.4e-7
+FT_WORDS = 4
+FT_CERTIFIED = 0x31305446
+FT_K = 5
+
+
+def edge_guard(lo, hi):
+  return 2.0 ** -23 * (2.0 * max(abs(lo), abs(hi)) + (hi - lo))
+
+
+def first_header(params, K=5, lo=-10.0, hi=10.0, min_bin=1e-4, min_slope=1e-4):
+  p = np.asarray(params, dtype=np.float32).astype(np.float64)
+  offset = np.log(np.exp(1.0 - min_slope) - 1.0)
+  total = (hi - lo) - K * min_bin
+
+  def knots(u):
+    e = np.exp(u - u.max())
+    s = 0.0
+    for k in range(K):
+      s += e[k]
+    pos = [lo]
+    run = 0.0
+    for k in range(K - 1):
+      run += e[k] / s * total + min_bin
+      pos.append(lo + run)
+    pos.append(hi)
+    return np.array(pos)
+
+  xk, yk = knots(p[:K]), knots(p[K:2 * K])
+  v = p[2 * K:3 * K + 1] + offset
+  d = np.maximum(v, 0.0) + np.log1p(np.exp(-np.abs(v))) + min_slope
+  return dict(K=K, lo=lo, hi=hi, xk=xk, yk=yk, d=d)
+
+
+def inverse_closed(h, k, v):
+  v = np.asarray(v, dtype=np.float64)
+  k = np.asarray(k)
+  x0, y0 = h["xk"][k], h["yk"][k]
+  bw, bh = h["xk"][k + 1] - x0, h["yk"][k + 1] - y0
+  s = bh / bw
+  d0, d1 = h["d"][k], h["d"][k + 1]
+  st = d1 + d0 - 2.0 * s
+  dy = v - y0
+  c2 = 2.0 * s * dy
+  b = d0 * bh - st * dy
+  a = s * bh - b
+  z = c2 / (b + np.sqrt(b * b + a * (c2 + c2)))
+  omz = 1.0 - z
+  num2 = d1 * z * z + 2.0 * s * z * omz + d0 * omz * omz
+  den = s + st * z * omz
+  return x0 + bw * z, -np.log(s * s * num2 / (den * den))
+
+
+def pieces(h):
+  lo, hi, K = h["lo"], h["hi"], h["K"]
+  cw = (hi - lo) / FT_CELLS
+  yk = h["yk"]
+  kc = [int(np.floor((yk[j] - lo) / cw)) for j in range(1, K)]
+  ok = True
+  guard = edge_guard(lo, hi)
+  for j in range(K - 1):
+    c = kc[j]
+    if j > 0 and kc[j - 1] == c:
+      ok = False
+    e0, e1 = lo + c * cw, (lo + (c + 1) * cw if c + 1 < FT_CELLS else hi)
+    if yk[j + 1] - e0 < guard or e1 - yk[j + 1] < guard:
+      ok = False
+  out = []
+  for p in range(FT_CELLS + K - 1):
+    m, half, knot = 0, 0, 0
+    for j in range(K - 1):
+      q = kc[j] + j
+      if q + 1 <= p:
+        m += 1
+      if p == q + 1:
+        half, knot = 2, j + 1
+      elif p == q and half == 0:
+        half, knot = 1, j + 1
+    c = min(max(p - m, 0), FT_CELLS - 1)
+    a, b = lo + c * cw, (lo + (c + 1) * cw if c + 1 < FT_CELLS else hi)
+    nb = sum(1 for j in range(K - 1) if kc[j] < c)
+    if half == 0:
+      ref, k = 0.5 * (a + b), nb
+    elif half == 1:
+      b, ref, k = yk[knot], yk[knot], knot - 1
+    else:
+      a, ref, k = yk[knot], yk[knot], knot
+    out.append((a, b, float(np.float32(ref)), min(k, K - 1), c, half))
+  return out, ok, kc
+
+
+_NODES = np.array([-1.0, -0.8090169943749475, -0.30901699437494745, 0.30901699437494745, 0.8090169943749475, 1.0])
+_PROBES = (2.0 * np.arange(FT_PROBES) + 1.0) / FT_PROBES - 1.0
+
+
+def _monomial(x, f):
+  n = x.shape[1]
+  c = np.array(f, dtype=np.float64)
+  for j in range(1, n):
+    for i in range(n - 1, j - 1, -1):
+      c[:, i] = (c[:, i] - c[:, i - 1]) / (x[:, i] - x[:, i - j])
+  m = np.zeros_like(c)
+  m[:, 0] = c[:, n - 1]
+  for i in range(n - 2, -1, -1):
+    for q in range(n - 1 - i, 0, -1):
+      m[:, q] = m[:, q - 1] - x[:, i] * m[:, q]
+    m[:, 0] = c[:, i] - x[:, i] * m[:, 0]
+  return m
+
+
+def _horner(co, dv):
+  r = np.zeros_like(dv) + co[:, -1:]
+  for q in range(co.shape[1] - 2, -1, -1):
+    r = r * dv + co[:, q:q + 1]
+  return r
+
+
+def build(params, probes=_PROBES, **kw):
+  h = first_header(params, **kw)
+  ps, ok, kc = pieces(h)
+  a, b, ref = (np.array([q[i] for q in ps], dtype=np.float64) for i in range(3))
+  k = np.array([q[3] for q in ps])
+  mid, rad = 0.5 * (a + b), 0.5 * (b - a)
+  rows = np.zeros((len(ps), FT_ROW), dtype=np.float32)
+  with np.errstate(all="ignore"):
+    xn = mid[:, None] + rad[:, None] * _NODES[None, :]
+    xn[:, 0], xn[:, -1] = a, b
+    o, l = inverse_closed(h, k[:, None], xn)
+    rows[:, 0::2] = _monomial(xn - ref[:, None], o)
+    rows[:, 1::2] = _monomial(xn - ref[:, None], l)
+    xp = mid[:, None] + rad[:, None] * np.asarray(probes)[None, :]
+    o, l = inverse_closed(h, k[:, None], xp)
+    eo = np.abs(_horner(rows[:, 0::2].astype(np.float64), xp - ref[:, None]) - o) / np.maximum(1.0, np.abs(o))
+    el = np.abs(_horner(rows[:, 1::2].astype(np.float64), xp - ref[:, None]) - l) / np.maximum(1.0, np.abs(l))
+    e = np.maximum(eo.max(axis=1), el.max(axis=1))
+    e[~(np.isfinite(eo).all(axis=1) & np.isfinite(el).all(axis=1) & np.isfinite(rows).all(axis=1))] = np.inf
+  worst = float(e.max())
+  grid = np.zeros((FT_CELLS, 4), dtype=np.float64)
+  K = h["K"]
+  for c in range(FT_CELLS):
+    base = c + sum(1 for j in range(K - 1) if kc[j] < c)
+    split = any(kc[j] == c for j in range(K - 1))
+    grid[c, 0] = ps[base][2]
+    grid[c, 1] = ps[base][2] if split else np.inf
+    grid[c, 2] = base * FT_ROW * 4
+  return dict(rows=rows, grid=grid, certified=bool(ok and worst <= FT_BUDGET), err=worst, piece_err=e, geom=ps,
+              geom_ok=ok, header=h)
+
+
+def evaluate(tab, v):
+  h = tab["header"]
+  v = np.asarray(v, dtype=np.float64)
+  c = np.clip(np.floor((v - h["lo"]) * (FT_CELLS / (h["hi"] - h["lo"]))).astype(np.int64), 0, FT_CELLS - 1)
+  g = tab["grid"][c]
+  row = (g[:, 2] / (FT_ROW * 4)).astype(np.int64) + (v >= g[:, 1])
+  dv = v - g[:, 0]
+  co = tab["rows"][row].astype(np.float64)
+  o = co[:, 2 * FT_DEG].copy()
+  l = co[:, 2 * FT_DEG + 1].copy()
+  for q in range(FT_DEG - 1, -1, -1):
+    o = o * dv + co[:, 2 * q]
+    l = l * dv + co[:, 2 * q + 1]
+  return o, l
diff --git a/cnf_ot_amd/flows.py b/cnf_ot_amd/flows.py
--- a/cnf_ot_amd/flows.py
+++ b/cnf_ot_amd/flows.py
@@ -199,6 +199,22 @@
 
   def set_pwl_builder(self, mode: int) -> None:
     _capi.check(self.lib.cnf_model_set_pwl_builder(self._h, int(mode)), "cnf_model_set_pwl_builder")
+
+  def set_first_table(self, mode: int) -> None:
+    _capi.check(self.lib.cnf_model_set_first_table(self._h, int(mode)), "cnf_model_set_first_table")
+
+  def first_table(self):
+    from . import first_table as ft
+    n_grid, n_rows = 4 * ft.FT_CELLS, (ft.FT_CELLS + ft.FT_K - 1) * ft.FT_ROW
+    n = int(self.lib.cnf_internal_first_table_floats())
+    if n != ft.FT_WORDS + n_grid + n_rows:
+      raise RuntimeError(f"the library's inverse table has {n} floats, first_table.py describes {ft.FT_WORDS + n_grid + n_rows}")
+    buf = np.empty(n, dtype=np.float32)
+    with _OnDevice(self.device):
+      _capi.check(self.lib.cnf_internal_first_table(self._h, _stream_ptr(self.device), buf.ctypes.data), "cnf_internal_first_table")
+    words = buf[:ft.FT_WORDS].view(np.uint32)
+    grid = buf[ft.FT_WORDS:ft.FT_WORDS + n_grid].reshape(ft.FT_CELLS, 4)
+    return bool(words[0] == ft.FT_CERTIFIED), grid, buf[ft.FT_WORDS + n_grid:].reshape(-1, ft.FT_ROW)
 
   def last_pwl_builder(self) -> int:
     return self.lib.cnf_model_last_pwl_builder(self._h)
diff --git a/include/cnf_ot_amd_debug.h b/include/cnf_ot_amd_debug.h
--- a/include/cnf_ot_amd_debug.h
+++ b/include/cnf_ot_amd_debug.h
@@ -20,6 +20,11 @@
 
 int cnf_internal_build_tables_into(CnfModel *m, void *stream, const float *c, float c_offset, int64_t n, float *out);
 
+int cnf_model_set_first_table(CnfModel *m, int mode);
+
+int64_t cnf_internal_first_table_floats(void);
+int cnf_internal_first_table(CnfModel *m, void *stream, float *out);
+
 int cnf_model_set_dpar(CnfModel *m, int mode);
 
 int cnf_model_set_profiling(CnfModel *m, int on);
```

Measured after the change: 102.5 billion samples/s, median of 6. 5.9% higher.
